# Fahad021/DER-VET

Measured on AMD Instinct MI355X. Metric: dispatch LP windows/sec (whole node, 8760h monthly windows); % HBM roofline, higher is better.
Workload: dtype f64

## Files before the change

der-vet_amd/csrc/dvh_band.hip:

```cpp
#include <stdio.h>
#include <stdlib.h>

#include <algorithm>
#include <type_traits>

#include "dvh_device.h"

namespace dvh {
namespace {

constexpr int kBandSteps = 768;
constexpr int kJMax = kBandJMax;
constexpr int kNeedsEll = -2;

__host__ __device__ constexpr size_t band_lds_doubles(int B, int S, bool ice, bool lc) {
  const int NW = B / kWave, NC = ice ? 5 : 3, NR = ice ? 4 : 2;
  const size_t SB = (size_t)S * B;
  return 2 * (size_t)(B + 1) + kJMax + (size_t)kNRed * (NW + 1) + 4 + (size_t)kJMax * B + (NC + NR) * SB +
         (lc ? 5 * SB : 0) + (ice ? 6 * SB : 0);
}
__host__ __device__ constexpr size_t band_ints_bytes(int B, int S) { return sizeof(int32_t) * (4 * (size_t)S * B + 4); }
__host__ __device__ constexpr size_t band_drow_bytes(int B, int S) { return align16(sizeof(int32_t) * (size_t)S * B); }
__host__ __device__ constexpr size_t band_lds_bytes(int B, int S, bool ice, bool lc) {
  const size_t d = align16(sizeof(double) * band_lds_doubles(B, S, ice, lc));
// ... 1152 lines not shown
    acc[2] = mv2;
    acc[3] = mv3;
#pragma unroll
    for (int u = 4; u < NRED; ++u) acc[u] = 0.0;
    double r = 0.0;
    if constexpr (GATE) {
      double acc4[4] = {acc[0], acc[1], acc[2], acc[3]};
      block_sum1<B, 4, true>(acc4, red);
#pragma unroll
      for (int u = 0; u < 4; ++u) acc[u] = acc4[u];
      r = usc<USC>(sqrt(pw * acc[0] + acc[2] / pw));
      if (kkt && !last && kkt_gate_skip(o, gate, r)) {
        kkt = false;
        ++gate.skip;
      }
    }
    if (kkt) {
      float fcl[S][NC], frl[S][NR], fspl = 1.0f;
      if constexpr (Tune::kkt_prefetch) {
        const int to = S * opaque(tid);
        const float* fcw = w.fc + W.wn;
        const float* frw = w.fr + W.wm;
#pragma unroll
        for (int s = 0; s < S; ++s) {
          const bool vs = to + s < T;
#pragma unroll
          for (int v = 0; v < NC; ++v) {
            const int j = v < 3 ? v * T + to + s : (v == 3 ? CE : CO) + to + s;
            const float f = fcw[vs ? j : 0];
            fcl[s][v] = vs ? f : 1.0f;
          }
#pragma unroll
          for (int r = 0; r < NR; ++r) {
            const int i = r == 0 ? (vs ? to + s + 1 : -1) : r == 1 ? DRL[s * B + tid] : (vs ? (r == 2 ? ra[s] : rb[s]) : -1);
            const float f = frw[i >= 0 ? i : 0];
            frl[s][r] = i >= 0 ? f : 1.0f;
          }
        }
        const int lo_ = (to / S) & (kWave - 1);
        const float ft = fcw[tlane ? 3 * T + lo_ : 0], fi = frw[0];
        fspl = tlane ? ft : ilane ? fi : 1.0f;
      }
      double xp[S][NC], yp[S][NR];
      load_images(xp, yp);
      XE[tid] = xp[0][2];
      YS[tid + 1] = yp[S - 1][0];
      if (ilane) YS[0] = sp[2];
      if (tlane) XT[lane] = sp[5];
      if (J > 0) tau_parts_of(yp);
      lds_barrier();
      auto col_kkt = [&](int j, double kt, double cj, double loj, double hij, double xj, float fpre) {
        const float fd = Tune::kkt_prefetch ? fpre : w.fc[W.wn + opaque(j)];
        static_assert(Tune::gate_rdx == Tune::kkt_inline, "col_kkt_x_i is inlined only, col_kkt_o out of line only");
        if constexpr (Tune::gate_rdx) {
          const ColKktX r = col_kkt_x_i(kt, cj, loj, hij, xj, fd);
          acc[5] += r.rd2;
          acc[6] += r.cx;
          acc[8] += r.bt;
          acc[kRdx] += r.rdx;
        } else {
          const ColKkt r = col_kkt_o(kt, cj, loj, hij, xj, fd);
          acc[5] += r.rd2;
          acc[6] += r.cx;
          acc[8] += r.bt;
        }
      };
      auto row_kkt = [&](int i, double kv, double qi, double yi, bool ge, float fpre) {
        const float fd = Tune::kkt_prefetch ? fpre : w.fr[W.wm + opaque(i)];
        const RowKkt r = row_kkt_fn<Tune::kkt_inline>(kv, qi, yi, fd, ge);
        acc[4] += r.rp2;
        acc[7] += qi * yi;
        acc[9] += r.y2;
      };
      const double ysp = YS[tid];
#pragma unroll
      for (int s = 0; s < S; ++s) {
        double kt[NC];
        ktr(s, yp[s], s == 0 ? ysp : yp[s > 0 ? s - 1 : 0][0], kt);
        if (val[s]) {
#pragma unroll
          for (int v = 0; v < NC; ++v) {
            if constexpr (BOX)
              col_kkt(col(s, v), kt[v], cof(s, v), 0.0, 1.0, xp[s][v], fcl[s][v]);
            else
              col_kkt(col(s, v), kt[v], cof(s, v), v == 2 ? loe[s] : 0.0, hib(s, v), xp[s][v], fcl[s][v]);
          }
        }
      }
      if (wid == 0 && J > 0) {
        const double ktt = tau_kt();
        if (tlane) col_kkt(3 * T + lane, ktt, sp[2], sp[3], sp[4], sp[5], fspl);
      }
      const double xen = XE[tid + 1];
#pragma unroll
      for (int s = 0; s < S; ++s) {
        double kv[NR];
        kown(s, xp[s], kv);
        kfin_next(s, kv, s == S - 1 ? xen : xp[s < S - 1 ? s + 1 : s][2]);
        kfin_tau(s, kv);
        const int t = t0 + s;
        if (val[s]) row_kkt(t + 1, kv[0], qv(s, 0), yp[s][0], false, frl[s][0]);
        const int dr_ = DRL[s * B + tid];
        if (dr_ >= 0) row_kkt(dr_, kv[1], qv(s, 1), yp[s][1], true, frl[s][1]);
        if (ICE && val[s]) {
          row_kkt(ra[s], kv[2], rhs(s, 2), yp[s][2], true, frl[s][NR > 2 ? 2 : 0]);
          row_kkt(rb[s], kv[3], rhs(s, 3), yp[s][3], true, frl[s][NR > 3 ? 3 : 0]);
        }
      }
      if (ilane) row_kkt(0, sp[4] * XE[0], sp[3], sp[2], false, fspl);
    }
    if constexpr (GATE) {
      if (kkt) {
        double acc6[NRED - 4];
#pragma unroll
        for (int u = 4; u < NRED; ++u) acc6[u - 4] = acc[u];
        block_sum1<B, NRED - 4, true>(acc6, red + 4 * NW);
#pragma unroll
        for (int u = 4; u < NRED; ++u) acc[u] = acc6[u - 4];
      }
    } else if (kkt) {
      block_sum1<B, NRED, true>(acc, red);
    } else {
      double acc4[4] = {acc[0], acc[1], acc[2], acc[3]};
      block_sum1<B, 4, true>(acc4, red);
#pragma unroll
      for (int u = 0; u < 4; ++u) acc[u] = acc4[u];
    }
    if constexpr (!GATE) r = usc<USC>(sqrt(pw * acc[0] + acc[2] / pw));
    if (kkt) {
      const double pobj = usc<USC>(acc[6] + c0), dobj = usc<USC>(acc[7] + acc[8] + c0);
      const double pres = usc<USC>(sqrt(acc[4]) / (1.0 + sgpr_fresh<USC>(qnorm)));
      const double dres = usc<USC>(sqrt(acc[5]) / (1.0 + sgpr_fresh<USC>(cnorm)));
      const double gap = usc<USC>(fabs(pobj - dobj) / (1.0 + fabs(pobj) + fabs(dobj)));
      if (tid == 0) {
        fin[0] = pobj;
        fin[1] = pres;
        fin[2] = dres;
        fin[3] = gap;
      }
      if (kkt_done(o, pres, dres, gap, pobj, dobj, acc[4], acc[9], Tune::gate_rdx ? acc[kRdx] : 0.0)) {
        status = kOptimal;
        break;
      }
      if constexpr (GATE) {
        gate.note(pres, dres, gap, o.eps, r);
        gate.q = usc<USC>(gate.q);
      }
      if (!(isfinite(pobj) && isfinite(dobj))) {
        status = kNumerical;
        break;
      }
    }
    if (r0 < 0.0) r0 = r;
    const bool restart = (r <= o.b_suff * r0) || (r <= o.b_nec * r0 && rprev >= 0.0 && r > rprev) ||
                         ((double)kin >= o.b_art * (double)it);
    if (restart) {
      const double ddx = sqrt(acc[1]), ddy = sqrt(acc[3]);
      if (ddx > 1e-10 && ddy > 1e-10) pw = uniform(pw_update<!ICE>(ddy / ddx, pw, o.theta));
      tau = uniform(eta / pw);
      sigma = uniform(eta * pw);
      sigma2n = uniform(-2.0 * sigma);
      box_steps_rescale();
      double xp[S][NC], yp[S][NR];
      load_images(xp, yp);
#pragma unroll
      for (int s = 0; s < S; ++s) {
#pragma unroll
        for (int v = 0; v < NC; ++v) {
          x[s][v] = xa[s][v] = xp[s][v];
        }
#pragma unroll
        for (int rr = 0; rr < NR; ++rr) {
          y[s][rr] = ya[s][rr] = yp[s][rr];
        }
      }
      if (ilane) sp[0] = sp[1] = sp[2];
      if (tlane) sp[0] = sp[1] = sp[5];
      kin = 0;
      kbase = 0;
      hw = hload(0);
      r0 = r;
      rprev = -1.0;
    } else {
      rprev = r;
    }
    if (restart || kkt) {
      YS[tid + 1] = y[S - 1][0];
      if (ilane) YS[0] = sp[0];
      if (J > 0) tau_parts_of(y);
      lds_barrier();
    }
  }
#pragma unroll
  for (int s = 0; s < S; ++s) {
    if (!val[s]) continue;
    const int t = t0 + s;
#pragma unroll
    for (int v = 0; v < NC; ++v) {
      const int j = col(s, v);
      if constexpr (BOX) {
        const double d = dcf(j), lo = lraw[j] / d, hv = uraw[j] / d;
        double wv = hv - (v == 2 ? lo : 0.0);
        if (!(wv >= 0x1p-500)) wv = 0.0;
        xo_g[j] = unscale_x(fmin(fmax(fma(wv, xpi(v, s), lo), lo), hv), d, lraw[j], uraw[j]);
      } else {
        xo_g[j] = unscale_x(xpi(v, s), dcf(j), lraw[j], uraw[j]);
      }
    }
    yo_g[t + 1] = ypi(0, s) * drf(t + 1);
    const int dr_ = DRL[s * B + tid];
    if (dr_ >= 0) yo_g[dr_] = ypi(1, s) * drf(dr_);
    if (ICE) {
      yo_g[ra[s]] = ypi(2, s) * drf(ra[s]);
      yo_g[rb[s]] = ypi(3, s) * drf(rb[s]);
    }
  }
  if (tlane) xo_g[3 * T + lane] = unscale_x(sp[5], dcf(3 * T + lane), lraw[3 * T + lane], uraw[3 * T + lane]);
  if (ilane) yo_g[0] = sp[2] * drf(0);
  if constexpr (DVH_BAND_PROBE) {
    pstamp(kProbeSegs - 1);
    pacc[kProbeSegs - 1] += (unsigned)(pt1 - pt2);
    unsigned hw = 0;
    asm volatile("s_getreg_b32 %0, hwreg(HW_REG_HW_ID)" : "=s"(hw));
    __syncthreads();
    if (lane == 0) {
      for (int u = 0; u < kProbeSegs; ++u) xo_g[(kProbeSegs + 1) * wid + u] = (double)pacc[u];
      xo_g[(kProbeSegs + 1) * wid + kProbeSegs] = (double)hw;
    }
  }
  if (tid == 0) {
    b.istats[2 * k] = status;
    b.istats[2 * k + 1] = it;
    for (int u = 0; u < 4; ++u) b.stats[4 * k + u] = fin[u];
  }
}

struct BandArgs {
  Batch b;
  Work w;
  Chunk ch;
  Opts o;
  const int32_t* list;
  int count;
  int32_t* queue;
};
template <int B, int S, bool ICE, bool LC, int WPS, bool GATE, bool BOX, bool PERSIST>
__global__ __launch_bounds__(B, WPS) void pdhg_band_kernel(const BandArgs args) {
  if constexpr (!PERSIST) {
    const int i = blockIdx.x;
    band_window<B, S, ICE, LC, WPS, GATE, BOX>(args.b, args.w, args.ch, args.o,
                                               args.list ? args.list[i] : args.ch.first + i, threadIdx.x);
  } else {
    __shared__ int32_t next;
    for (;;) {
#if defined(__HIP_DEVICE_COMPILE__)
      using KArgs = const __attribute__((address_space(4))) BandArgs*;
      KArgs kp = (KArgs)__builtin_amdgcn_kernarg_segment_ptr();
      asm volatile("" : "+s"(kp));
      const BandArgs& args = *(const BandArgs*)kp;
#endif
      if (__builtin_amdgcn_readfirstlane(threadIdx.x) < kWave)
        next = __builtin_amdgcn_readfirstlane(atomicAdd(args.queue, (threadIdx.x & (kWave - 1)) == 0 ? 1 : 0));
      __syncthreads();
      const int i = __builtin_amdgcn_readfirstlane(next);
      __syncthreads();
      if (i >= args.count) return;
      int tid = threadIdx.x;
#if defined(__HIP_DEVICE_COMPILE__)
      asm volatile("" : "+v"(tid));
#endif
      band_window<B, S, ICE, LC, WPS, GATE, BOX>(args.b, args.w, args.ch, args.o,
                                                 args.list ? args.list[i] : args.ch.first + i, tid);
    }
  }
}

template <int B, int S, bool ICE, bool LC, int WPS, bool GATE, bool BOX>
__global__ __launch_bounds__(B, WPS) void pdhg_band_kernel_j1(const BandArgs args) {
  __shared__ int32_t next;
  for (;;) {
#if defined(__HIP_DEVICE_COMPILE__)
    using KArgs = const __attribute__((address_space(4))) BandArgs*;
    KArgs kp = (KArgs)__builtin_amdgcn_kernarg_segment_ptr();
    asm volatile("" : "+s"(kp));
    const BandArgs& args = *(const BandArgs*)kp;
#endif
    if (__builtin_amdgcn_readfirstlane(threadIdx.x) < kWave)
      next = __builtin_amdgcn_readfirstlane(atomicAdd(args.queue, (threadIdx.x & (kWave - 1)) == 0 ? 1 : 0));
    __syncthreads();
    const int i = __builtin_amdgcn_readfirstlane(next);
    __syncthreads();
    if (i >= args.count) return;
    int tid = threadIdx.x;
#if defined(__HIP_DEVICE_COMPILE__)
    asm volatile("" : "+v"(tid));
#endif
    band_window<B, S, ICE, LC, WPS, GATE, BOX, true>(args.b, args.w, args.ch, args.o,
                                                     args.list ? args.list[i] : args.ch.first + i, tid);
  }
}

template <int B, int S, bool ICE, bool LC, int WPS, bool GATE, bool BOX, bool PERSIST>
hipError_t launch_band_one_q(const Batch& b, const Work& w, const Chunk& ch, const Opts& o, hipStream_t s,
                             const int32_t* list, int nlist, int* variant_out) {
  static_assert(B * S == kBandSteps, "every form covers T <= kBandSteps");
  const size_t lds = band_lds_bytes(B, S, ICE, LC);
  auto kern = pdhg_band_kernel<B, S, ICE, LC, WPS, GATE, BOX, PERSIST>;
  hipError_t e = hipFuncSetAttribute((const void*)kern, hipFuncAttributeMaxDynamicSharedMemorySize, (int)lds);
  if (e != hipSuccess) return e;
  if (getenv("DVH_BAND_OCC")) {
    int nb = -1, dev = 0;
    hipGetDevice(&dev);
    hipDeviceProp_t pr;
    hipGetDeviceProperties(&pr, dev);
    hipOccupancyMaxActiveBlocksPerMultiprocessor(&nb, (const void*)kern, B, lds);
    hipFuncAttributes fa;
    hipFuncGetAttributes(&fa, (const void*)kern);
    fprintf(stderr, "band<%d,%d,%d,%d,gate %d,box %d,persist %d>: lds %zu B, blocks/CU %d, lds/CU %zu, regs %d, local %zu\n",
            B, S, (int)ICE, (int)LC, (int)GATE, (int)BOX, (int)PERSIST, lds, nb, (size_t)pr.maxSharedMemoryPerMultiProcessor,
            fa.numRegs, (size_t)fa.localSizeBytes);
  }
  const int count = list ? nlist : ch.count;
  if (count <= 0) return hipSuccess;
  int grid = count;
  if (PERSIST) {
    int& slots = w.slots[(ICE ? 4 : 0) + (GATE ? 2 : 0) + (BOX ? 1 : 0)];
    if (slots <= 0) {
      int nb = 0, cus = 0, dev = 0;
      if ((e = hipGetDevice(&dev)) != hipSuccess) return e;
      if ((e = hipOccupancyMaxActiveBlocksPerMultiprocessor(&nb, (const void*)kern, B, lds)) != hipSuccess) return e;
      if ((e = hipDeviceGetAttribute(&cus, hipDeviceAttributeMultiprocessorCount, dev)) != hipSuccess) return e;
      slots = std::max(1, nb) * std::max(1, cus);
    }
    static const int reserve = [] { const char* e = getenv("DVH_BAND_RESERVE"); return e ? std::max(0, atoi(e)) : 0; }();
    grid = std::min(count, std::max(1, slots - 2 * reserve));
    if ((e = hipMemsetAsync(w.queue, 0, sizeof(int32_t), s)) != hipSuccess) return e;
  }
  const BandArgs args{b, w, ch, o, list, count, w.queue};
  hipLaunchKernelGGL(kern, dim3(grid), dim3(B), lds, s, args);
  if (variant_out) *variant_out = 9000000 + 1000 * (S - 1) + (ICE ? 100 : 0) + B / kWave;
  return hipGetLastError();
}
template <int B, int S, bool ICE, bool LC, int WPS, bool GATE, bool BOX>
hipError_t launch_band_one_g(const Batch& b, const Work& w, const Chunk& ch, const Opts& o, hipStream_t s,
                             const int32_t* list, int nlist, bool j1, int* variant_out) {
  if constexpr (S == 3 && !ICE) {
    static_assert(B == kBandSteps / 3 && LC && WPS == 2, "dvh_band_persist.hip instantiates this form");
    const char* q = getenv("DVH_BAND_QUEUE");
    if (!(q && atoi(q) == 0)) return launch_band_persist(GATE, BOX, j1, b, w, ch, o, s, list, nlist, variant_out);
  }
  if constexpr (ICE) {
    static_assert(B == kBandSteps && S == 1 && !LC && WPS == 3, "dvh_band_persist_ice.hip instantiates this form");
    const char* q = getenv("DVH_BAND_QUEUE");
    const char* qi = getenv("DVH_BAND_QUEUE_ICE");
    if (!(q && atoi(q) == 0) && !(qi && atoi(qi) == 0))
      return launch_band_persist_ice(GATE, BOX, b, w, ch, o, s, list, nlist, variant_out);
  }
  return launch_band_one_q<B, S, ICE, LC, WPS, GATE, BOX, false>(b, w, ch, o, s, list, nlist, variant_out);
}
template <int B, int S, bool ICE, bool LC, int WPS, bool BOX = false>
hipError_t launch_band_one(const Batch& b, const Work& w, const Chunk& ch, const Opts& o, hipStream_t s,
                           const int32_t* list, int nlist, bool j1, int* variant_out) {
  if (o.kkt_predict > 0)
    return launch_band_one_g<B, S, ICE, LC, WPS, true, BOX>(b, w, ch, o, s, list, nlist, j1, variant_out);
  return launch_band_one_g<B, S, ICE, LC, WPS, false, BOX>(b, w, ch, o, s, list, nlist, j1, variant_out);
}

}

#if DVH_BAND_PERSIST_TU == 1
namespace {
template <bool GATE, bool BOX>
hipError_t launch_band_persist_j1(const Batch& b, const Work& w, const Chunk& ch, const Opts& o, hipStream_t s,
                                  const int32_t* list, int nlist, int* variant_out) {
  constexpr int B = kBandSteps / 3, S = 3;
  const size_t lds = band_lds_bytes(B, S, false, true);
  auto kern = pdhg_band_kernel_j1<B, S, false, true, 2, GATE, BOX>;
  hipError_t e = hipFuncSetAttribute((const void*)kern, hipFuncAttributeMaxDynamicSharedMemorySize, (int)lds);
  if (e != hipSuccess) return e;
  const int count = list ? nlist : ch.count;
  if (count <= 0) return hipSuccess;
  int& slots = w.slots[8 + (GATE ? 2 : 0) + (BOX ? 1 : 0)];
  if (slots <= 0) {
    int nb = 0, cus = 0, dev = 0;
    if ((e = hipGetDevice(&dev)) != hipSuccess) return e;
    if ((e = hipOccupancyMaxActiveBlocksPerMultiprocessor(&nb, (const void*)kern, B, lds)) != hipSuccess) return e;
    if ((e = hipDeviceGetAttribute(&cus, hipDeviceAttributeMultiprocessorCount, dev)) != hipSuccess) return e;
    slots = std::max(1, nb) * std::max(1, cus);
  }
  static const int reserve = [] { const char* e = getenv("DVH_BAND_RESERVE"); return e ? std::max(0, atoi(e)) : 0; }();
  const int grid = std::min(count, std::max(1, slots - 2 * reserve));
  if ((e = hipMemsetAsync(w.queue, 0, sizeof(int32_t), s)) != hipSuccess) return e;
  const BandArgs args{b, w, ch, o, list, count, w.queue};
  hipLaunchKernelGGL(kern, dim3(grid), dim3(B), lds, s, args);
  if (variant_out) *variant_out = 9000000 + 1000 * (S - 1) + kBandJ1 + B / kWave;
  return hipGetLastError();
}
}
hipError_t launch_band_persist(bool gate, bool box, bool j1, const Batch& b, const Work& w, const Chunk& ch,
                               const Opts& o, hipStream_t s, const int32_t* list, int nlist, int* variant_out) {
  constexpr int B = kBandSteps / 3;
  if (j1) {
    const char* e = getenv("DVH_BAND_J1");
    if (e && atoi(e) == 0) j1 = false;
  }
  if (j1) {
    if (gate) {
      if (box) return launch_band_persist_j1<true, true>(b, w, ch, o, s, list, nlist, variant_out);
      return launch_band_persist_j1<true, false>(b, w, ch, o, s, list, nlist, variant_out);
    }
    if (box) return launch_band_persist_j1<false, true>(b, w, ch, o, s, list, nlist, variant_out);
    return launch_band_persist_j1<false, false>(b, w, ch, o, s, list, nlist, variant_out);
  }
  if (gate) {
    if (box) return launch_band_one_q<B, 3, false, true, 2, true, true, true>(b, w, ch, o, s, list, nlist, variant_out);
    return launch_band_one_q<B, 3, false, true, 2, true, false, true>(b, w, ch, o, s, list, nlist, variant_out);
  }
  if (box) return launch_band_one_q<B, 3, false, true, 2, false, true, true>(b, w, ch, o, s, list, nlist, variant_out);
  return launch_band_one_q<B, 3, false, true, 2, false, false, true>(b, w, ch, o, s, list, nlist, variant_out);
}
#elif DVH_BAND_PERSIST_TU == 2
hipError_t launch_band_persist_ice(bool gate, bool box, const Batch& b, const Work& w, const Chunk& ch, const Opts& o,
                                   hipStream_t s, const int32_t* list, int nlist, int* variant_out) {
  constexpr int B = kBandSteps;
  if (gate) {
    if (box) return launch_band_one_q<B, 1, true, false, 3, true, true, true>(b, w, ch, o, s, list, nlist, variant_out);
    return launch_band_one_q<B, 1, true, false, 3, true, false, true>(b, w, ch, o, s, list, nlist, variant_out);
  }
  if (box) return launch_band_one_q<B, 1, true, false, 3, false, true, true>(b, w, ch, o, s, list, nlist, variant_out);
  return launch_band_one_q<B, 1, true, false, 3, false, false, true>(b, w, ch, o, s, list, nlist, variant_out);
}
#else
hipError_t launch_pdhg_band(const Batch& b, const Work& w, const Chunk& ch, const Opts& o, hipStream_t s, bool ice,
                            int form, bool box, const int32_t* list, int nlist, bool j1, int* variant_out) {
  if (ice) {
    if (box) return launch_band_one<kBandSteps, 1, true, false, 3, true>(b, w, ch, o, s, list, nlist, false, variant_out);
    return launch_band_one<kBandSteps, 1, true, false, 3>(b, w, ch, o, s, list, nlist, false, variant_out);
  }
  if (form == 1) {
    if (box) return launch_band_one<kBandSteps, 1, false, false, 3, true>(b, w, ch, o, s, list, nlist, false, variant_out);
    return launch_band_one<kBandSteps, 1, false, false, 3>(b, w, ch, o, s, list, nlist, false, variant_out);
  }
  if (box) return launch_band_one<kBandSteps / 3, 3, false, true, 2, true>(b, w, ch, o, s, list, nlist, j1, variant_out);
  return launch_band_one<kBandSteps / 3, 3, false, true, 2>(b, w, ch, o, s, list, nlist, j1, variant_out);
}
#endif

}
```

der-vet_amd/csrc/dvh_cascade.cpp:

```cpp
#include <cstdio>
#include <cstdlib>

#include "dvh_handle.h"

namespace dvh {

int chain_pass(dvh_handle* h, const dvh::Batch& b, const dvh::Work& w, const dvh::Chunk& ch, const dvh::Opts& o,
               const std::vector<int32_t>& med, int max_T, const std::vector<int64_t>& desc,
               std::vector<char>& med_done, hipStream_t s) {
  const int nm = (int)med.size();
  if (nm == 0) return DVH_OK;
  const size_t I = sizeof(int32_t);
  DVH_HIP(h, h->m_list.ensure(I * (size_t)nm));
  DVH_HIP(h, hipMemcpyAsync(h->m_list.p, med.data(), I * nm, hipMemcpyHostToDevice, s));
  DVH_HIP(h, h->m_plan.ensure(I * (size_t)nm * dvh::kPlanInts));
  hipError_t e = dvh::launch_chain_plan(b, w, ch, h->m_list.as<int32_t>(), nm, max_T, h->m_plan.as<int32_t>(), s);
  if (e != hipSuccess) return hip_fail(h, e, "launch_chain_plan");
  std::vector<int32_t> head((size_t)nm * 4);
  DVH_HIP(h, hipMemcpy2DAsync(head.data(), 4 * I, h->m_plan.p, I * dvh::kPlanInts, 4 * I, nm, hipMemcpyDeviceToHost, s));
  DVH_HIP(h, sync_stream(h, s));
  std::vector<int32_t> small_setup, accepted;
  for (int i = 0; i < nm; ++i) {
    const int P = head[4 * (size_t)i];
    if (P < 0) med_done[med[i]] = 1;
    if (P <= 0) continue;
    accepted.push_back(i);
    if (desc[8 * (size_t)med[i]] < dvh::kMedSetupNMax) small_setup.push_back(med[i]);
  }
  if (accepted.empty()) return DVH_OK;
  if (!small_setup.empty()) {
    int mn = 0;
    for (int k : small_setup) mn = std::max<int>(mn, (int)desc[8 * (size_t)k]);
    DVH_HIP(h, h->m_pos.ensure(I * small_setup.size()));
    DVH_HIP(h, hipMemcpyAsync(h->m_pos.p, small_setup.data(), I * small_setup.size(), hipMemcpyHostToDevice, s));
    e = dvh::launch_setup_medium(b, w, ch, o, mn, h->m_pos.as<int32_t>(), (int)small_setup.size(), s);
    if (e != hipSuccess) return hip_fail(h, e, "launch_setup_medium");
  }
  for (int i : accepted) {
    const int k = med[i];
    if (desc[8 * (size_t)k] < dvh::kMedSetupNMax) continue;
    e = dvh::launch_setup_long(b, w, ch, o, k, &desc[8 * (size_t)k], s);
    if (e != hipSuccess) return hip_fail(h, e, "launch_setup_long");
  }
  std::vector<double> flag6(accepted.size(), 0.0);
  for (size_t a = 0; a < accepted.size(); ++a)
    DVH_HIP(h, hipMemcpyAsync(&flag6[a], w.scal + (int64_t)(med[accepted[a]] - ch.first) * dvh::kScal + 6,
                              sizeof(double), hipMemcpyDeviceToHost, s));
  DVH_HIP(h, sync_stream(h, s));
  std::vector<int32_t> groups[2];
  int PTg[2] = {0, 0};
  for (size_t a = 0; a < accepted.size(); ++a) {
    if (flag6[a] != 0.0) continue;
    const int i = accepted[a], P = head[4 * (size_t)i];
    const int g = P > dvh::kChainMedMax ? 1 : 0;
    groups[g].push_back(i);
    PTg[g] = std::max(PTg[g], P);
  }
  if (h->chain_cap < 0) {
    int cap = 0;
    if (dvh::chain_capacity(h->device, &cap) != hipSuccess) cap = 0;
    (void)hipGetLastError();
    h->chain_cap = cap;
  }
  if (h->spin_ticks <= 0) {
    int khz = 0;
    if (hipDeviceGetAttribute(&khz, hipDeviceAttributeWallClockRate, h->device) != hipSuccess || khz <= 0) khz = 100000;
    h->spin_ticks = (long long)khz * 1000 * 2;
    if (const char* v = getenv("DVH_CHAIN_SPIN_TICKS")) {
      const long long t = atoll(v);
      if (t != 0) h->spin_ticks = t;
    }
  }
  const int S = h->chain_cap / 8;
  for (int g = 0; g < 2; ++g) {
    const int PT = PTg[g];
    if (groups[g].empty()) continue;
    const int NT = S >= 1 && PT <= 8 * S ? dvh::chain_team_count(S, PT) : 0;
    if (NT < 1) continue;
    constexpr int kMaxPerLaunch = 0x3FFF - 2;
    for (size_t a0 = 0; a0 < groups[g].size(); a0 += kMaxPerLaunch) {
      const int np = (int)std::min<size_t>(kMaxPerLaunch, groups[g].size() - a0);
      const int32_t* pos = groups[g].data() + a0;
      std::vector<int32_t> ks(np);
      for (int q = 0; q < np; ++q) ks[q] = med[pos[q]];
      DVH_HIP(h, h->m_pos.ensure(I * 2 * (size_t)np));
      int32_t* dpos = h->m_pos.as<int32_t>();
      DVH_HIP(h, hipMemcpyAsync(dpos, pos, I * np, hipMemcpyHostToDevice, s));
      DVH_HIP(h, hipMemcpyAsync(dpos + np, ks.data(), I * np, hipMemcpyHostToDevice, s));
      e = dvh::launch_chain_mark(b, dpos + np, np, s);
      if (e != hipSuccess) return hip_fail(h, e, "launch_chain_mark");
      DVH_HIP(h, h->m_xbuf.ensure(dvh::chain_xbuf_bytes(NT, PT)));
      DVH_HIP(h, h->m_abort.ensure(dvh::chain_abort_bytes(S)));
      e = dvh::launch_chain(b, w, ch, o, dpos, np, h->m_plan.as<int32_t>(), PT, S, h->m_xbuf.p,
                            h->m_abort.as<int32_t>(), h->spin_ticks, s);
      if (e == hipErrorCooperativeLaunchTooLarge) {
        (void)hipGetLastError();
        h->chain_cap = 0;
        return DVH_OK;
      }
      if (e != hipSuccess) return hip_fail(h, e, "launch_chain");
      std::vector<int32_t> ab(dvh::chain_abort_bytes(S) / I);
      DVH_HIP(h, hipMemcpyAsync(ab.data(), h->m_abort.p, I * ab.size(), hipMemcpyDeviceToHost, s));
      DVH_HIP(h, sync_stream(h, s));
      if (getenv("DVH_CHAIN_PROBE_DUMP")) {
        for (int gb = 0; gb < 8 * S; ++gb)
          if (ab[16 + 8 * (size_t)gb + 6] || ab[16 + 8 * (size_t)gb + 7])
            fprintf(stderr, "PROBE block %d tauwait %d hopwait %d\n", gb, ab[16 + 8 * (size_t)gb + 6],
                    ab[16 + 8 * (size_t)gb + 7]);
      }
      if (ab[0] != 0) {
        std::string msg = "medium tier: a segment exchange timed out (PT " + std::to_string(PT) + ", NT " +
                          std::to_string(NT) + "); unfinished windows moved to the grid-wide path; workgroups "
                          "{block: state list round entry tag seen}:";
        for (int gb = 0; gb < 8 * S; ++gb) {
          const int32_t* d = &ab[16 + 8 * (size_t)gb];
          if (d[0] == 0) continue;
          char buf[128];
          snprintf(buf, sizeof buf, " %d: %d %d %d 0x%x 0x%x 0x%x;", gb, d[0], d[1], d[2], d[3], d[4], d[5]);
          msg += buf;
        }
        h->st.warn += msg;
        ++h->st.n_chain_aborts;
        std::vector<int32_t> st(2);
        for (int q = 0; q < np; ++q) {
          DVH_HIP(h, hipMemcpy(st.data(), b.istats + 2 * (int64_t)ks[q], 2 * I, hipMemcpyDeviceToHost));
          if (st[0] != dvh::kChainPending) {
            med_done[ks[q]] = 1;
            ++h->st.n_chain;
          }
        }
        continue;
      }
      for (int q = 0; q < np; ++q) med_done[ks[q]] = 1;
      h->st.n_chain += np;
    }
  }
  return DVH_OK;
}

int device_cascade(dvh_handle* h, const dvh::Batch& b, const dvh::Work& w, const dvh::Chunk& ch, const dvh::Opts& o,
                   int nsmall, int nj, int wc, int mn, int mm, hipStream_t s, const int32_t* order) {
  const size_t I = sizeof(int32_t);
  int32_t* L[5];
  for (int r = 0; r < 5; ++r) L[r] = h->d_list.as<int32_t>() + (size_t)r * wc;
  int32_t* info = h->d_route.as<int32_t>();
  int32_t* rh = h->route_host.as<int32_t>();
  if (h->cus <= 0 && hipDeviceGetAttribute(&h->cus, hipDeviceAttributeMultiprocessorCount, h->device) != hipSuccess)
    h->cus = 256;
  const int forced_form = h->kernel_path == 3 ? 1 : h->kernel_path == 4 ? 3 : 0;
  auto form_for = [&](int nl) { return forced_form ? forced_form : (nl <= h->cus ? 1 : 3); };
  auto route = [&](int slot, const int32_t* in, int n_in, int want, int cls, int out) -> hipError_t {
    return dvh::launch_route(b.desc, b.istats, w.scal, ch.first, n_in, in, want, dvh::kSmallMax, cls, 512, 768,
                             L[out], info + 8 * slot, s);
  };
  auto readback = [&](int slot0, int nslots) -> hipError_t {
    hipError_t e = hipMemcpyAsync(rh + 8 * slot0, info + 8 * slot0, 8 * I * nslots, hipMemcpyDeviceToHost, s);
    return e != hipSuccess ? e : sync_stream(h, s);
  };
  const bool j1 = nj == 0;
  int variant = -1, bvar = -1;
  h->last_band_variant = -1;
  auto form_code = [](int v) { return v >= 0 && v % 100 >= dvh::kBandJ1 ? v - dvh::kBandJ1 : v; };
  const char* box_env = getenv("DVH_BAND_BOX");
  const int box_mode = box_env ? atoi(box_env) : 1;
  const bool box = box_mode >= 1, box_ice = box_mode >= 2;
  DVH_HIP(h, dvh::launch_pdhg_band(b, w, ch, o, s, false, form_for(ch.count), box, order, order ? ch.count : 0, j1, &bvar));
  DVH_HIP(h, route(0, nullptr, ch.count, -2, 0, 0));
  if (box) DVH_HIP(h, route(1, nullptr, ch.count, -3, 0, 1));
  DVH_HIP(h, readback(0, box ? 2 : 1));
  if (box && rh[8] > 0) {
    DVH_HIP(h, dvh::launch_pdhg_band(b, w, ch, o, s, false, form_for(rh[8]), false, L[1], rh[8], j1, nullptr));
    DVH_HIP(h, route(0, nullptr, ch.count, -2, 0, 0));
    DVH_HIP(h, readback(0, 1));
  }
  int cur = rh[0];
  h->st.n_band += nsmall - cur;
  if (nsmall - cur > 0) {
    variant = form_code(bvar);
    h->last_band_variant = bvar;
  }
  if (cur > 0) {
    DVH_HIP(h, dvh::launch_pdhg_band(b, w, ch, o, s, true, form_for(cur), box_ice, L[0], cur, false, &bvar));
    if (h->kernel_path == 5) DVH_HIP(h, dvh::launch_pdhg_band_grid(b, w, ch, o, s, L[0], cur, &bvar));
    DVH_HIP(h, route(1, L[0], cur, -2, 0, 4));
    if (box_ice) DVH_HIP(h, route(2, L[0], cur, -3, 0, 1));
    DVH_HIP(h, readback(1, box_ice ? 2 : 1));
    if (box_ice && rh[16] > 0) {
      DVH_HIP(h, dvh::launch_pdhg_band(b, w, ch, o, s, true, form_for(rh[16]), false, L[1], rh[16], false, nullptr));
      DVH_HIP(h, route(1, L[0], cur, -2, 0, 4));
      DVH_HIP(h, readback(1, 1));
    }
    const int left = rh[8];
    h->st.n_band += cur - left;
    if (cur - left > 0 && variant < 0) variant = bvar;
    cur = left;
    if (cur > 0) {
      DVH_HIP(h, dvh::launch_setup(b, w, ch, o, mn, mm, s, L[4], cur));
      DVH_HIP(h, route(1, L[4], cur, -2, 1, 2));
      DVH_HIP(h, route(2, L[4], cur, -2, 2, 3));
      DVH_HIP(h, readback(1, 2));
    }
  }
  if (cur == 0) {
    h->last_variant = variant;
    return DVH_OK;
  }
  int ran[2] = {0, 0};
  for (int c = 0; c < 2; ++c) {
    const int32_t* in = rh + 8 * (1 + c);
    if (in[0] == 0) continue;
    int ev = -1;
    hipError_t e = dvh::launch_pdhg_ell(b, w, ch, o, in[3], in[4], in[1], in[2], s, &ev, L[2 + c], in[0],
                                        in[0] <= 2 * h->cus);
    if (e == hipSuccess) {
      if (variant < 0) variant = ev;
      DVH_HIP(h, route(3 + c, L[2 + c], in[0], -1, 0, c));
      ran[c] = 1;
    } else if (e == hipErrorInvalidValue) {
      (void)hipGetLastError();
    } else {
      return hip_fail(h, e, "launch_pdhg_ell");
    }
  }
  if (ran[0] || ran[1]) DVH_HIP(h, readback(3, 2));
  int gn = 0, gm[3] = {0, 0, 0};
  int32_t* gl = nullptr;
  for (int c = 0; c < 2; ++c) {
    const int32_t* in = rh + 8 * (1 + c);
    if (in[0] == 0) continue;
    const int32_t* g = ran[c] ? rh + 8 * (3 + c) : in;
    int32_t* l = ran[c] ? L[c] : L[2 + c];
    if (ran[c]) h->st.n_ell += in[0] - g[0];
    if (g[0] == 0) continue;
    if (!gl) {
      gl = l;
    } else {
      DVH_HIP(h, hipMemcpyAsync(gl + gn, l, I * g[0], hipMemcpyDeviceToDevice, s));
    }
    gn += g[0];
    for (int u = 0; u < 3; ++u) gm[u] = std::max(gm[u], (int)g[3 + u]);
  }
  if (gn > 0) {
    DVH_HIP(h, dvh::launch_power(b, w, ch, o, gl, gn, s));
    int gv = -1;
    hipError_t e = dvh::launch_pdhg(b, w, ch, o, gm[0], gm[1], gm[2], s, &gv, gl, gn);
    if (e == hipErrorInvalidValue)
      return fail(h, DVH_ERR_UNSUPPORTED, "window too large for the on-chip PDHG kernels (n or m > 4096)");
    if (e != hipSuccess) return hip_fail(h, e, "launch_pdhg");
    h->st.n_generic += gn;
    if (variant < 0) variant = gv;
  }
  h->last_variant = variant;
  return DVH_OK;
}

}
```

der-vet_amd/csrc/dvh_handle.h:

```cpp
#pragma once
#include <array>
#include <string>

#include "dvh_host.h"

struct SolveStats {
  int n_ell = 0, n_generic = 0, n_large = 0, n_band = 0, n_chain = 0;
  int n_chain_aborts = 0;
  std::string warn;
  float large_ms[2] = {0, 0};
  size_t chunk_used = 0;
  int32_t cert[5] = {0, 0, 0, 0, 0};
  double cert_ms = 0.0;
  double timing[3] = {0, 0, 0};
  void reset() {
    n_ell = n_generic = n_large = n_band = n_chain = 0;
    n_chain_aborts = 0;
    warn.clear();
    large_ms[0] = large_ms[1] = 0.0f;
    chunk_used = 0;
  }
  void add(const SolveStats& p) {
    n_ell += p.n_ell;
    n_generic += p.n_generic;
    n_large += p.n_large;
    n_band += p.n_band;
    n_chain += p.n_chain;
    n_chain_aborts += p.n_chain_aborts;
    warn += p.warn;
    for (int u = 0; u < 4; ++u) cert[u] += p.cert[u];
    cert[4] = std::max(cert[4], p.cert[4]);
    cert_ms = std::max(cert_ms, p.cert_ms);
    for (int u = 1; u < 3; ++u) timing[u] = std::max(timing[u], p.timing[u]);
  }
};

struct dvh_handle_core {
  int device = 0;
  hipStream_t stream = nullptr;
  ~dvh_handle_core() {
    if (stream) (void)hipStreamDestroy(stream);
  }
};

struct SizingSlot {
  dvh::SizingState* p = nullptr;
  SizingSlot() = default;
  SizingSlot(const SizingSlot&) = delete;
  SizingSlot& operator=(const SizingSlot&) = delete;
  ~SizingSlot() {
    if (p) dvh::sizing_destroy(p);
  }
};

struct dvh_handle : dvh_handle_core {
  SizingSlot sizing;
  dvh::CommOwner comm;
  dvh::LargeOwner large;
  DevEvent ev[4];
  DevEvent cert_ev[2];
  std::vector<std::array<DevEvent, 3>> chunk_events;
  DevEvent val_ev[2][2];
  bool val_ran[2] = {false, false};
  dvh_options opts{};
  std::string err;
  DevBuf d_desc, d_indptr, d_indices, d_data, d_c, d_c0, d_q, d_l, d_u, d_x, d_y, d_stats, d_istats;
  DevBuf w_queue;
  int band_slots[dvh::kPersistForms] = {};
  DevBuf w_tptr, w_tind, w_tval, w_kval, w_rowof, w_perm, w_dr, w_dc, w_cs, w_ls, w_us, w_qs, w_vbuf, w_wbuf,
      w_tmpc, w_tmpr, w_longk, w_longt, w_scal, w_fc, w_fr;
  DevBuf d_list, d_hinv;
  DevBuf m_list, m_plan, m_pos, m_xbuf, m_abort;
  int chain_cap = -1;
  long long spin_ticks = 0;
  SolveStats st;
  DevBuf o_data, o_cases, o_len, o_hist, o_soe;
  DevBuf s_pairs, s_wts, s_bad;
  DevBuf g_seeds, g_word;
  DevBuf d_route;
  DevBuf c_tptr, c_tind, c_tval, c_tau, c_gx, c_sig, c_gy, c_counts;
  bool cert_pending = false;
  DevBuf v_zwork;
  int n_syncs = 0;
  double outage_ms = 0.0;
  int last_variant = -1;
  int last_band_variant = -1;
  int kernel_path = 0;
  int cus = 0;
  std::vector<int32_t> order;
  std::vector<int32_t> order_used;
  DevBuf d_order;
  std::vector<dvh_handle*> peers;
  PinnedBuf route_host, cert_host;
};

inline hipError_t sync_stream(dvh_handle* h, hipStream_t s) {
  ++h->n_syncs;
  return hipStreamSynchronize(s);
}

inline int fail(dvh_handle* h, int code, const std::string& msg) {
  if (h) h->err = msg;
  return code;
}

inline int hip_fail(dvh_handle* h, hipError_t e, const char* where) {
  return fail(h, DVH_ERR_HIP, std::string(where) + ": " + hipGetErrorString(e));
}

#define DVH_HIP(h, call)                                 \
  do {                                                   \
    hipError_t e_ = (call);                              \
    if (e_ != hipSuccess) return hip_fail(h, e_, #call); \
  } while (0)

namespace dvh {

int device_cascade(dvh_handle* h, const Batch& b, const Work& w, const Chunk& ch, const Opts& o, int nsmall, int nj, int wc,
                   int mn, int mm, hipStream_t s, const int32_t* order);
int chain_pass(dvh_handle* h, const Batch& b, const Work& w, const Chunk& ch, const Opts& o,
               const std::vector<int32_t>& med, int max_T, const std::vector<int64_t>& desc,
               std::vector<char>& med_done, hipStream_t s);

}
```

der-vet_amd/csrc/dvh_internal.h:

```cpp
#pragma once
#include <hip/hip_runtime.h>
#include <stdint.h>

#include <memory>
#include <string>

struct dvh_window_series;
struct dvh_battery_group;
struct dvh_packed;
struct dvh_options;
struct dvh_handle;

namespace dvh {

constexpr int kWave = 64;
constexpr int kLongRow = 32;
constexpr int kLMax = 64;
constexpr int kScal = 16;
constexpr int kHalpernTab = 65536;
constexpr int kSmallMax = 4096;
constexpr int kChainB = 768;
constexpr int kPMax = 192;
constexpr int kChainMedMax = 16;
constexpr int kChainJMax = 256;
constexpr int kChainJSeg = 4;
constexpr int kPlanStart = 4;
constexpr int kPlanSlot = kPlanStart + kPMax + 4;
constexpr int kPlanLo = kPlanSlot + kChainJSeg * kPMax;
constexpr int kPlanHi = kPlanLo + kChainJSeg * kPMax;
constexpr int kPlanInts = kPlanHi + kChainJSeg * kPMax;
constexpr int kMedSetupNMax = 40000;

__host__ __device__ inline double unscale_x(double xs, double d, double l, double u) {
  const double v = xs * d;
  return v != v ? v : fmin(fmax(v, l), u);
}

struct Opts {
  double eps, step_safety, rho, b_suff, b_nec, b_art, theta;
  double eps_obj;
  int max_iters, check_every, kkt_every, ruiz_iters, power_iters;
  int setup_segments;
  int small_max;
  int warm;
  int kkt_predict;
};

struct Batch {
  const int64_t* desc;
  const int32_t* indptr;
  const int32_t* indices;
  const double* data;
  const double* c;
  const double* c0;
  const double* q;
  const double* l;
  const double* u;
  double* x;
  double* y;
  double* stats;
  int32_t* istats;
};

struct Work {
  int32_t* tptr;
  int32_t* tind;
  double* tval;
  double* kval;
  int32_t* rowof;
  int32_t* perm;
  double* dr;
  double* dc;
  double* cs;
  double* ls;
  double* us;
  double* qs;
  double* vbuf;
  double* wbuf;
  double* tmpc;
  double* tmpr;
  int32_t* longk;
  int32_t* longt;
  const double* hinv;
  double* scal;
  float* fc;
  float* fr;
  int32_t* queue;
  int* slots;
};
constexpr int kPersistForms = 12;

struct Chunk {
  int first;
  int count;
  int64_t base_n, base_m, base_nz;
};

hipError_t launch_setup(const Batch& b, const Work& w, const Chunk& ch, const Opts& o, int max_n, int max_m,
                        hipStream_t s, const int32_t* list = nullptr, int nlist = 0);
hipError_t launch_pdhg(const Batch& b, const Work& w, const Chunk& ch, const Opts& o, int max_n, int max_m,
                       int64_t max_nnz, hipStream_t s, int* variant_out, const int32_t* list, int nlist);
hipError_t launch_pdhg_ell(const Batch& b, const Work& w, const Chunk& ch, const Opts& o, int max_n, int max_m,
                           int wx, int wy, hipStream_t s, int* variant_out, const int32_t* list, int nlist,
                           bool latency = false);
hipError_t launch_pdhg_band(const Batch& b, const Work& w, const Chunk& ch, const Opts& o, hipStream_t s, bool ice,
                            int form, bool box, const int32_t* list, int nlist, bool j1, int* variant_out);
constexpr int kBandJ1 = 50;
constexpr int kBandJMax = 4;
hipError_t launch_band_persist(bool gate, bool box, bool j1, const Batch& b, const Work& w, const Chunk& ch,
                               const Opts& o, hipStream_t s, const int32_t* list, int nlist, int* variant_out);
hipError_t launch_band_persist_ice(bool gate, bool box, const Batch& b, const Work& w, const Chunk& ch, const Opts& o,
                                   hipStream_t s, const int32_t* list, int nlist, int* variant_out);
size_t setup_lds_bytes(int max_n, int max_m);
hipError_t launch_setup_medium(const Batch& b, const Work& w, const Chunk& ch, const Opts& o, int max_n,
                               const int32_t* list, int nlist, hipStream_t s);
hipError_t launch_chain_plan(const Batch& b, const Work& w, const Chunk& ch, const int32_t* list, int nlist,
                             int max_T, int32_t* plan, hipStream_t s);
hipError_t launch_setup_long(const Batch& b, const Work& w, const Chunk& ch, const Opts& o, int k, const int64_t* d,
                             hipStream_t s);
constexpr int kChainPending = -7;
hipError_t launch_chain_mark(const Batch& b, const int32_t* list, int nlist, hipStream_t s);
hipError_t chain_capacity(int device, int* blocks);
size_t chain_xbuf_bytes(int NT, int PT);
size_t chain_abort_bytes(int S);
int chain_team_count(int S, int PT);
hipError_t launch_chain(const Batch& b, const Work& w, const Chunk& ch, const Opts& o, const int32_t* pos, int npos,
                        const int32_t* plan, int PT, int S, void* xbuf, int32_t* abort_word, long long spin_ticks,
                        hipStream_t s);
constexpr int kMaxBlend = 8;
hipError_t launch_warm_transfer(const int64_t* desc, const double* c, const double* u, double* x, double* y,
                                const int32_t* rows, const double* wts, int q, int count, int32_t* bad, hipStream_t s);
hipError_t launch_series_draws(const uint64_t* seeds, int count, int steps, int n_unif, double a1, double innov,
                               double* z0, double* ar, double* unif, int32_t* ambiguous, int32_t* amb_rows,
                               hipStream_t s);
hipError_t launch_series_windows(const ::dvh_window_series& w, int32_t* bad, hipStream_t s);
hipError_t launch_build_battery(const ::dvh_battery_group& g, const ::dvh_packed& b, int first, hipStream_t s);
hipError_t launch_route(const int64_t* desc, const int32_t* istats, const double* scal, int first, int count,
                        const int32_t* in_list, int want, int small_max, int cls, int lim_n, int lim_m,
                        int32_t* out_list, int32_t* out_info, hipStream_t s);
hipError_t launch_power(const Batch& b, const Work& w, const Chunk& ch, const Opts& o, const int32_t* list, int nlist,
                        hipStream_t s);

struct OutageCase {
  int n_steps, max_steps, outage_len, pad;
  int64_t len_off, hist_off;
  double dt, soe0, dg_gen, gamma, soe_min, soe_max, charge_max, discharge_max, rte;
  const double *critical_load, *pv_max, *pv_vari, *init_soe, *load_shed;
};
hipError_t launch_outage(const OutageCase* d_cases, int ncase, int max_steps_n, int max_bins, int32_t* d_lengths,
                         int32_t* d_hist, hipStream_t s);
hipError_t launch_outage_min_soe(const OutageCase* d_cases, int ncase, int max_steps_n, double* d_soe_used,
                                 hipStream_t s);

hipError_t launch_outage_first_uncovered(const OutageCase* d_cases, int ncase, int max_steps_n, int32_t* d_first,
                                         int32_t* d_count, hipStream_t s);

struct SizingLP {
  const double *cl, *pv_vari, *shed;
  int32_t* starts;
  int n_steps, K, L, new_start;
  double dt, dg_gen, rte, llsoc, ulsoc, a0;
  double lE, uE, lP, uP, cE, cP, c0;
};
hipError_t launch_build_sizing(const SizingLP* d_lps, int nlp, const int64_t* desc, int32_t* indptr, int32_t* indices,
                               double* data, double* c, double* c0, double* q, double* l, double* u, hipStream_t s);
hipError_t launch_gather_sizes(const int64_t* desc, const double* x, const int32_t* istats, int nlp, double* sizes,
                               hipStream_t s);

struct SizingState;
void sizing_destroy(SizingState* s);
struct LargeSolver;
LargeSolver* large_create();
void large_destroy(LargeSolver* ls);
struct Comm;
void comm_destroy(Comm* c);
template <auto Destroy>
struct DestroyWith {
  template <class T>
  void operator()(T* p) const { Destroy(p); }
};
using LargeOwner = std::unique_ptr<LargeSolver, DestroyWith<large_destroy>>;
using CommOwner = std::unique_ptr<Comm, DestroyWith<comm_destroy>>;

struct HandleView {
  int device;
  hipStream_t stream;
  dvh_options* opts;
  std::string* err;
  SizingState** sizing;
};
HandleView handle_view(dvh_handle* h);
inline int fail(const HandleView& v, int code, const std::string& msg) {
  *v.err = msg;
  return code;
}
#define DVH_VIEW_HIP(v, call)                                                                                  \
  do {                                                                                                         \
    hipError_t e_ = (call);                                                                                    \
    if (e_ != hipSuccess) return dvh::fail(v, DVH_ERR_HIP, std::string(#call) + ": " + hipGetErrorString(e_)); \
  } while (0)


constexpr int kCommIdBytes = 128;
int comm_unique_id(unsigned char* id, std::string* err);
int comm_init(int device, int rank, int world, const unsigned char* id, CommOwner* out, std::string* err);
int comm_all_gather(Comm* c, const void* send, void* recv, size_t bytes, hipStream_t s, std::string* err);
void comm_info(const Comm* c, int* rank, int* world);
hipError_t large_solve(LargeSolver* ls, const Batch& b, int k, const int64_t* d, const Opts& o, const double* hinv,
                       hipStream_t s, std::string* err, float* setup_ms, float* pdhg_ms);

hipError_t launch_pdhg_band_grid(const Batch& b, const Work& w, const Chunk& ch, const Opts& o, hipStream_t s,
                                 const int32_t* list, int nlist, int* variant_out);

constexpr int kCertifyDefaultCap = 65536;
struct CertWork {
  int32_t* tptr;
  int32_t* tind;
  double* tval;
  double* tau;
  double* gx;
  double* sig;
  double* gy;
  int32_t* counts;
  int64_t base_n, base_m, base_nz;
};
size_t certify_lds_bytes(int max_n, int max_m);
hipError_t launch_certify(const Batch& b, const CertWork& cw, int count, int max_n, int max_m, int cap, int gate,
                          hipStream_t s);

}
```

der-vet_amd/csrc/dvh_solve.cpp:

```cpp
#include <chrono>
#include <thread>

#include "dvh_handle.h"
#include "dvh_validate.h"

namespace {

constexpr int kChunkWindows = 262144;

dvh::Opts make_opts(const dvh_options& p) {
  dvh::Opts o;
  o.eps = p.eps;
  o.eps_obj = p.eps_obj;
  o.step_safety = p.step_safety;
  o.rho = p.reflection;
  o.b_suff = p.restart_sufficient;
  o.b_nec = p.restart_necessary;
  o.b_art = p.restart_artificial;
  o.theta = p.primal_weight_theta;
  o.max_iters = p.max_iters;
  o.check_every = std::max(1, std::min(p.check_every, p.max_iters));
  o.kkt_every = p.kkt_every;
  o.ruiz_iters = p.ruiz_iters;
  o.power_iters = p.power_iters;
  o.warm = p.warm_start != 0;
  o.kkt_predict = p.kkt_predict;
  o.small_max = dvh::kSmallMax;
  return o;
}

dvh::Batch make_batch(const dvh_packed& bt) {
  return dvh::Batch{bt.desc, bt.indptr, bt.indices, bt.data, bt.c, bt.c0, bt.q, bt.l, bt.u,
                    bt.x, bt.y, bt.stats, bt.istats};
}

int certify_pass(dvh_handle* h, const dvh_packed* bt, const std::vector<int64_t>& desc, int gate, hipStream_t s) {
  const int count = bt->count;
  const int64_t bn = desc[6], bm = desc[7], bz = desc[5];
  int64_t sn = 0, sm = 0, snz = 0;
  int mn = 1, mm = 1;
  for (int k = 0; k < count; ++k) {
    const int64_t* d = &desc[8 * (size_t)k];
    sn = std::max(sn, d[6] + d[0] - bn);
    sm = std::max(sm, d[7] + d[1] - bm);
    snz = std::max(snz, d[5] + d[3] - bz);
    if (d[0] > dvh::kSmallMax || d[1] > dvh::kSmallMax) continue;
    mn = std::max<int>(mn, (int)d[0]);
    mm = std::max<int>(mm, (int)d[1]);
  }
  const size_t D = sizeof(double), I = sizeof(int32_t);
  DVH_HIP(h, h->c_tptr.ensure(I * (size_t)(sn + count)));
  DVH_HIP(h, h->c_tind.ensure(I * (size_t)snz));
  DVH_HIP(h, h->c_tval.ensure(D * (size_t)snz));
  DVH_HIP(h, h->c_tau.ensure(D * (size_t)sn));
  DVH_HIP(h, h->c_gx.ensure(D * (size_t)sn));
  DVH_HIP(h, h->c_sig.ensure(D * (size_t)sm));
  DVH_HIP(h, h->c_gy.ensure(D * (size_t)sm));
  DVH_HIP(h, h->c_counts.ensure(I * 5));
  DVH_HIP(h, h->cert_host.ensure(I * 5));
  for (DevEvent& e : h->cert_ev) DVH_HIP(h, e.ensure());
  dvh::CertWork cw{h->c_tptr.as<int32_t>(), h->c_tind.as<int32_t>(), h->c_tval.as<double>(), h->c_tau.as<double>(),
                   h->c_gx.as<double>(), h->c_sig.as<double>(), h->c_gy.as<double>(), h->c_counts.as<int32_t>(),
                   bn, bm, bz};
  const int cap = h->opts.certify_iters > 0 ? h->opts.certify_iters : dvh::kCertifyDefaultCap;
  DVH_HIP(h, hipMemsetAsync(h->c_counts.p, 0, I * 5, s));
  DVH_HIP(h, hipEventRecord(h->cert_ev[0], s));
  DVH_HIP(h, dvh::launch_certify(make_batch(*bt), cw, count, mn, mm, cap, gate, s));
  DVH_HIP(h, hipEventRecord(h->cert_ev[1], s));
  DVH_HIP(h, hipMemcpyAsync(h->cert_host.p, h->c_counts.p, I * 5, hipMemcpyDeviceToHost, s));
  h->cert_pending = true;
  return DVH_OK;
}

void certify_reset(dvh_handle* h) {
  for (int32_t& v : h->st.cert) v = 0;
  h->st.cert_ms = 0.0;
  h->cert_pending = false;
}

bool is_large(const int64_t* d) { return d[0] > dvh::kSmallMax || d[1] > dvh::kSmallMax; }

struct ChunkPlan {
  dvh::Chunk ch;
  int64_t sn, sm, snz;
  int mn, mm;
  int64_t mnz;
  int nsmall;
  int nj;
  std::vector<int32_t> med;
  int med_T = 0;
};
struct BatchPlan {
  std::vector<ChunkPlan> chunks;
  std::vector<int> large;
  int64_t wn = 0, wm = 0, wnz = 0;
  int wc = 0;
};

BatchPlan scan_chunks(const std::vector<int64_t>& desc, int count, bool chain_on) {
  auto is_medium = [&](const int64_t* d) {
    const int64_t T = d[2] - 1;
    return chain_on && T > dvh::kChainB && T <= (int64_t)dvh::kPMax * dvh::kChainB && d[0] >= 3 * T &&
           d[0] <= 3 * T + dvh::kChainJMax && d[1] <= 2 * T + 1;
  };
  BatchPlan p;
  for (int first = 0; first < count; first += kChunkWindows) {
    ChunkPlan c{};
    c.ch.first = first;
    c.ch.count = std::min(kChunkWindows, count - first);
    const int64_t* d0 = &desc[8 * (size_t)first];
    c.ch.base_n = d0[6];
    c.ch.base_m = d0[7];
    c.ch.base_nz = d0[5];
    for (int k = first; k < first + c.ch.count; ++k) {
      const int64_t* d = &desc[8 * (size_t)k];
      c.sn = std::max(c.sn, d[6] + d[0] - c.ch.base_n);
      c.sm = std::max(c.sm, d[7] + d[1] - c.ch.base_m);
      c.snz = std::max(c.snz, d[5] + d[3] - c.ch.base_nz);
      if (is_large(d)) {
        p.large.push_back(k);
        if (is_medium(d)) {
          c.med.push_back(k);
          c.med_T = std::max<int>(c.med_T, (int)d[2] - 1);
        }
        continue;
      }
      ++c.nsmall;
      const int64_t J = d[0] - 3 * (d[2] - 1);
      if (J == 0 || (J >= 2 && J <= dvh::kBandJMax)) ++c.nj;
      c.mn = std::max<int>(c.mn, (int)d[0]);
      c.mm = std::max<int>(c.mm, (int)d[1]);
      c.mnz = std::max(c.mnz, d[3]);
    }
    p.wn = std::max(p.wn, c.sn);
    p.wm = std::max(p.wm, c.sm);
    p.wnz = std::max(p.wnz, c.snz);
    p.wc = std::max(p.wc, c.ch.count);
    p.chunks.push_back(c);
  }
  return p;
}

int make_work(dvh_handle* h, const BatchPlan& p, dvh::Work& w) {
  const int64_t wn = p.wn, wm = p.wm, wnz = p.wnz;
  const int wc = p.wc;
  const size_t D = sizeof(double), I = sizeof(int32_t);
  DVH_HIP(h, h->w_tptr.ensure(I * (wn + wc)));
  DVH_HIP(h, h->w_tind.ensure(I * wnz));
  DVH_HIP(h, h->w_tval.ensure(D * wnz));
  DVH_HIP(h, h->w_kval.ensure(D * wnz));
  DVH_HIP(h, h->w_rowof.ensure(I * wnz));
  DVH_HIP(h, h->w_perm.ensure(I * wnz));
  DVH_HIP(h, h->w_dr.ensure(D * wm));
  DVH_HIP(h, h->w_dc.ensure(D * wn));
  DVH_HIP(h, h->w_cs.ensure(D * wn));
  DVH_HIP(h, h->w_ls.ensure(D * wn));
  DVH_HIP(h, h->w_us.ensure(D * wn));
  DVH_HIP(h, h->w_qs.ensure(D * wm));
  DVH_HIP(h, h->w_vbuf.ensure(D * wn));
  DVH_HIP(h, h->w_wbuf.ensure(D * wm));
  DVH_HIP(h, h->w_tmpc.ensure(D * wn));
  DVH_HIP(h, h->w_tmpr.ensure(D * wm));
  DVH_HIP(h, h->w_longk.ensure(I * (size_t)wc * dvh::kLMax));
  DVH_HIP(h, h->w_longt.ensure(I * (size_t)wc * dvh::kLMax));
  DVH_HIP(h, h->w_scal.ensure(D * (size_t)wc * dvh::kScal));
  DVH_HIP(h, h->w_fc.ensure(sizeof(float) * wn));
  DVH_HIP(h, h->w_fr.ensure(sizeof(float) * wm));
  DVH_HIP(h, h->w_queue.ensure(sizeof(int32_t)));
  w = dvh::Work{h->w_tptr.as<int32_t>(), h->w_tind.as<int32_t>(), h->w_tval.as<double>(), h->w_kval.as<double>(),
                h->w_rowof.as<int32_t>(), h->w_perm.as<int32_t>(), h->w_dr.as<double>(), h->w_dc.as<double>(),
                h->w_cs.as<double>(), h->w_ls.as<double>(), h->w_us.as<double>(), h->w_qs.as<double>(),
                h->w_vbuf.as<double>(), h->w_wbuf.as<double>(), h->w_tmpc.as<double>(), h->w_tmpr.as<double>(),
                h->w_longk.as<int32_t>(), h->w_longt.as<int32_t>(), h->d_hinv.as<double>(), h->w_scal.as<double>(),
                h->w_fc.as<float>(), h->w_fr.as<float>(), h->w_queue.as<int32_t>(), h->band_slots};
  DVH_HIP(h, h->d_list.ensure(I * 5 * (size_t)wc));
  DVH_HIP(h, h->d_route.ensure(I * 8 * 5));
  DVH_HIP(h, h->route_host.ensure(I * 8 * 5));
  return DVH_OK;
}

int next_chunk_events(dvh_handle* h, const DevEvent*& out) {
  if (h->st.chunk_used == h->chunk_events.size()) h->chunk_events.emplace_back();
  std::array<DevEvent, 3>& ce = h->chunk_events[h->st.chunk_used];
  for (DevEvent& e : ce) DVH_HIP(h, e.ensure());
  ++h->st.chunk_used;
  out = ce.data();
  return DVH_OK;
}

int host_list_tiers(dvh_handle* h, const dvh::Batch& b, const dvh::Work& w, const ChunkPlan& c, const dvh::Opts& o,
                    bool fast, const std::vector<int64_t>& desc, hipStream_t s) {
  const size_t I = sizeof(int32_t);
  auto large_at = [&](int k) { return is_large(&desc[8 * (size_t)k]); };
  std::vector<double> scal((size_t)c.ch.count * dvh::kScal);
  DVH_HIP(h, hipMemcpyAsync(scal.data(), w.scal, sizeof(double) * scal.size(), hipMemcpyDeviceToHost, s));
  DVH_HIP(h, sync_stream(h, s));
  int wx = 0, wy = 0;
  for (int k = 0; k < c.ch.count; ++k) {
    const double* sc = &scal[(size_t)k * dvh::kScal];
    if (sc[6] != 0.0) continue;
    wy = std::max(wy, (int)sc[8]);
    wx = std::max(wx, (int)sc[9]);
  }
  int variant = -1;
  hipError_t e = hipErrorInvalidValue;
  if (fast) {
    int ev = -1;
    e = dvh::launch_pdhg_ell(b, w, c.ch, o, c.mn, c.mm, wx, wy, s, &ev, nullptr, 0);
    if (e == hipSuccess) variant = ev;
  }
  std::vector<int32_t> generic;
  if (e == hipSuccess) {
    std::vector<int32_t> ist(2 * (size_t)c.ch.count);
    DVH_HIP(h, hipMemcpyAsync(ist.data(), b.istats + 2 * (size_t)c.ch.first, I * ist.size(),
                              hipMemcpyDeviceToHost, s));
    DVH_HIP(h, sync_stream(h, s));
    int nl = 0;
    for (int k = 0; k < c.ch.count; ++k) {
      if (large_at(c.ch.first + k)) {
        ++nl;
        continue;
      }
      if (ist[2 * (size_t)k] == -1) generic.push_back(c.ch.first + k);
    }
    h->st.n_ell += c.ch.count - (int)generic.size() - nl;
  } else if (e == hipErrorInvalidValue) {
    (void)hipGetLastError();
    for (int k = 0; k < c.ch.count; ++k)
      if (!large_at(c.ch.first + k)) generic.push_back(c.ch.first + k);
  } else {
    return hip_fail(h, e, "launch_pdhg_ell");
  }
  if (!generic.empty()) {
    DVH_HIP(h, hipMemcpyAsync(h->d_list.p, generic.data(), I * generic.size(), hipMemcpyHostToDevice, s));
    DVH_HIP(h, dvh::launch_power(b, w, c.ch, o, h->d_list.as<int32_t>(), (int)generic.size(), s));
    int gv = -1;
    e = dvh::launch_pdhg(b, w, c.ch, o, c.mn, c.mm, c.mnz, s, &gv, h->d_list.as<int32_t>(), (int)generic.size());
    if (e == hipErrorInvalidValue)
      return fail(h, DVH_ERR_UNSUPPORTED, "window too large for the on-chip PDHG kernels (n or m > 4096)");
    if (e != hipSuccess) return hip_fail(h, e, "launch_pdhg");
    h->st.n_generic += (int)generic.size();
    if (variant < 0) variant = gv;
    DVH_HIP(h, sync_stream(h, s));
  }
  h->last_variant = variant;
  return DVH_OK;
}

int solve_packed(dvh_handle* h, const dvh_packed* bt, const std::vector<int64_t>& desc, hipStream_t s) {
  const int count = bt->count;
  certify_reset(h);
  const dvh::Opts o = make_opts(h->opts);
  const dvh::Batch b = make_batch(*bt);
  const bool fast = h->kernel_path != 1 && o.rho == 1.0;
  const bool cascade = fast && (h->kernel_path == 0 || h->kernel_path >= 3);
  const bool chain_on = (h->kernel_path == 0 || h->kernel_path >= 3) && o.rho == 1.0 && o.max_iters + o.power_iters < (1 << 17);
  const BatchPlan plan = scan_chunks(desc, count, chain_on);
  dvh::Work w;
  if (int rc = make_work(h, plan, w)) return rc;
  h->st.reset();
  DVH_HIP(h, hipEventRecord(h->ev[0], s));
  const size_t I = sizeof(int32_t);
  const int32_t* order = nullptr;
  h->order_used.swap(h->order);
  h->order.clear();
  if (!h->order_used.empty() && (int)h->order_used.size() == count && plan.chunks.size() == 1 &&
      plan.chunks[0].nsmall == count) {
    DVH_HIP(h, h->d_order.ensure(I * count));
    DVH_HIP(h, hipMemcpyAsync(h->d_order.as<int32_t>(), h->order_used.data(), I * count, hipMemcpyHostToDevice, s));
    order = h->d_order.as<int32_t>();
  }
  std::vector<char> med_done(count, 0);
  for (const ChunkPlan& c : plan.chunks) {
    if (c.nsmall == 0 && c.med.empty()) continue;
    const DevEvent* ce = nullptr;
    if (int rc = next_chunk_events(h, ce)) return rc;
    DVH_HIP(h, hipEventRecord(ce[0], s));
    if (c.nsmall > 0 && !cascade) DVH_HIP(h, dvh::launch_setup(b, w, c.ch, o, c.mn, c.mm, s));
    DVH_HIP(h, hipEventRecord(ce[1], s));
    if (c.nsmall > 0)
      if (int rc = cascade ? dvh::device_cascade(h, b, w, c.ch, o, c.nsmall, c.nj, plan.wc, c.mn, c.mm, s, order)
                           : host_list_tiers(h, b, w, c, o, fast, desc, s))
        return rc;
    if (int rc = dvh::chain_pass(h, b, w, c.ch, o, c.med, c.med_T, desc, med_done, s)) return rc;
    DVH_HIP(h, hipEventRecord(ce[2], s));
  }
  for (int k : plan.large) {
    if (med_done[k]) continue;
    if (!h->large) h->large.reset(dvh::large_create());
    std::string msg;
    hipError_t e = dvh::large_solve(h->large.get(), b, k, &desc[8 * (size_t)k], o, h->d_hinv.as<double>(), s, &msg,
                                    &h->st.large_ms[0], &h->st.large_ms[1]);
    if (e != hipSuccess) return fail(h, DVH_ERR_HIP, "window " + std::to_string(k) + ": " + msg);
    ++h->st.n_large;
  }
  if (h->opts.certify != 0)
    if (int rc = certify_pass(h, bt, desc, 1, s)) return rc;
  DVH_HIP(h, hipEventRecord(h->ev[3], s));
  return DVH_OK;
}

int certify_packed(dvh_handle* h, const dvh_packed* bt, const std::vector<int64_t>& desc, hipStream_t s) {
  certify_reset(h);
  h->st.reset();
  DVH_HIP(h, hipEventRecord(h->ev[0], s));
  if (int rc = certify_pass(h, bt, desc, 0, s)) return rc;
  DVH_HIP(h, hipEventRecord(h->ev[3], s));
  return DVH_OK;
}

int finish_timing(dvh_handle* h, hipStream_t s) {
  DVH_HIP(h, sync_stream(h, s));
  SolveStats& st = h->st;
  float t = 0;
  st.timing[0] = st.timing[1] = st.timing[2] = 0;
  if (hipEventElapsedTime(&t, h->ev[0], h->ev[3]) == hipSuccess) st.timing[0] = t;
  if (h->cert_pending) {
    for (int i = 0; i < 5; ++i) st.cert[i] = h->cert_host.as<int32_t>()[i];
    if (hipEventElapsedTime(&t, h->cert_ev[0], h->cert_ev[1]) == hipSuccess) st.cert_ms = t;
    h->cert_pending = false;
  }
  for (size_t i = 0; i < st.chunk_used; ++i) {
    const auto& ce = h->chunk_events[i];
    if (hipEventElapsedTime(&t, ce[0], ce[1]) == hipSuccess) st.timing[1] += t;
    if (hipEventElapsedTime(&t, ce[1], ce[2]) == hipSuccess) st.timing[2] += t;
  }
  st.timing[1] += st.large_ms[0];
  st.timing[2] += st.large_ms[1];
  return DVH_OK;
}

std::vector<int> split_batch(const dvh_lp* lps, int32_t count, int parts) {
  std::vector<double> cum(count + 1, 0.0);
  for (int k = 0; k < count; ++k) {
    const dvh_lp& lp = lps[k];
    const bool big = lp.n > dvh::kSmallMax || lp.m_eq + lp.m_ineq > dvh::kSmallMax;
    cum[k + 1] = cum[k] + (big ? std::max(1.0, lp.nnz / 5208.0) : 1.0);
  }
  std::vector<int> b(parts + 1, count);
  b[0] = 0;
  for (int r = 1; r < parts; ++r) {
    const double target = cum[count] * r / parts;
    int k = b[r - 1];
    while (k < count && cum[k] + 0.5 * (cum[k + 1] - cum[k]) < target) ++k;
    b[r] = k;
  }
  return b;
}

int solve_batch_one(dvh_handle* h, const dvh_lp* lps, int32_t count, dvh_result* out, bool screen = false) {
  DVH_HIP(h, hipSetDevice(h->device));
  std::vector<int64_t> desc(8 * (size_t)count);
  int64_t tn = 0, tm = 0, tz = 0, tr = 0;
  for (int k = 0; k < count; ++k) {
    std::string msg = dvh::validate_lp(lps[k], k);
    if (!msg.empty()) return fail(h, DVH_ERR_ARG, msg);
    const dvh_lp& lp = lps[k];
    const int m = lp.m_eq + lp.m_ineq;
    int64_t* d = &desc[8 * (size_t)k];
    d[0] = lp.n;
    d[1] = m;
    d[2] = lp.m_eq;
    d[3] = lp.nnz;
    d[4] = tr;
    d[5] = tz;
    d[6] = tn;
    d[7] = tm;
    tr += m + 1;
    tz += lp.nnz;
    tn += lp.n;
    tm += m;
  }
  std::vector<int32_t> indptr(tr), indices(tz);
  std::vector<double> data(tz), c(tn), l(tn), u(tn), q(tm), c0(count);
  for (int k = 0; k < count; ++k) {
    const dvh_lp& lp = lps[k];
    const int64_t* d = &desc[8 * (size_t)k];
    const int m = (int)d[1];
    std::memcpy(&indptr[d[4]], lp.indptr, sizeof(int32_t) * (m + 1));
    if (lp.nnz) {
      std::memcpy(&indices[d[5]], lp.indices, sizeof(int32_t) * lp.nnz);
      std::memcpy(&data[d[5]], lp.data, sizeof(double) * lp.nnz);
    }
    std::memcpy(&c[d[6]], lp.c, sizeof(double) * lp.n);
    std::memcpy(&l[d[6]], lp.l, sizeof(double) * lp.n);
    std::memcpy(&u[d[6]], lp.u, sizeof(double) * lp.n);
    if (m) std::memcpy(&q[d[7]], lp.q, sizeof(double) * m);
    c0[k] = lp.c0;
  }
  const size_t D = sizeof(double), I = sizeof(int32_t);
  DVH_HIP(h, h->d_desc.ensure(desc.size() * sizeof(int64_t)));
  DVH_HIP(h, h->d_indptr.ensure(I * tr));
  DVH_HIP(h, h->d_indices.ensure(I * std::max<int64_t>(tz, 1)));
  DVH_HIP(h, h->d_data.ensure(D * std::max<int64_t>(tz, 1)));
  DVH_HIP(h, h->d_c.ensure(D * tn));
  DVH_HIP(h, h->d_l.ensure(D * tn));
  DVH_HIP(h, h->d_u.ensure(D * tn));
  DVH_HIP(h, h->d_x.ensure(D * tn));
  DVH_HIP(h, h->d_q.ensure(D * std::max<int64_t>(tm, 1)));
  DVH_HIP(h, h->d_y.ensure(D * std::max<int64_t>(tm, 1)));
  DVH_HIP(h, h->d_c0.ensure(D * count));
  DVH_HIP(h, h->d_stats.ensure(D * 4 * count));
  DVH_HIP(h, h->d_istats.ensure(I * 2 * count));
  hipStream_t s = h->stream;
  DVH_HIP(h, hipMemcpyAsync(h->d_desc.p, desc.data(), desc.size() * sizeof(int64_t), hipMemcpyHostToDevice, s));
  DVH_HIP(h, hipMemcpyAsync(h->d_indptr.p, indptr.data(), I * tr, hipMemcpyHostToDevice, s));
  if (tz) {
    DVH_HIP(h, hipMemcpyAsync(h->d_indices.p, indices.data(), I * tz, hipMemcpyHostToDevice, s));
    DVH_HIP(h, hipMemcpyAsync(h->d_data.p, data.data(), D * tz, hipMemcpyHostToDevice, s));
  }
  DVH_HIP(h, hipMemcpyAsync(h->d_c.p, c.data(), D * tn, hipMemcpyHostToDevice, s));
  DVH_HIP(h, hipMemcpyAsync(h->d_l.p, l.data(), D * tn, hipMemcpyHostToDevice, s));
  DVH_HIP(h, hipMemcpyAsync(h->d_u.p, u.data(), D * tn, hipMemcpyHostToDevice, s));
  if (tm) DVH_HIP(h, hipMemcpyAsync(h->d_q.p, q.data(), D * tm, hipMemcpyHostToDevice, s));
  DVH_HIP(h, hipMemcpyAsync(h->d_c0.p, c0.data(), D * count, hipMemcpyHostToDevice, s));
  std::vector<double> x0, y0;
  if (h->opts.warm_start || screen) {
    x0.assign(tn, 0.0);
    y0.assign(std::max<int64_t>(tm, 1), 0.0);
    for (int k = 0; k < count; ++k) {
      const int64_t* d = &desc[8 * (size_t)k];
      if (out[k].x) std::memcpy(&x0[d[6]], out[k].x, D * d[0]);
      if (out[k].y && d[1]) std::memcpy(&y0[d[7]], out[k].y, D * d[1]);
    }
    DVH_HIP(h, hipMemcpyAsync(h->d_x.p, x0.data(), D * tn, hipMemcpyHostToDevice, s));
    DVH_HIP(h, hipMemcpyAsync(h->d_y.p, y0.data(), D * y0.size(), hipMemcpyHostToDevice, s));
  }
  const dvh_packed bt{count, 0, tn, tm, tz, tr, h->d_desc.as<int64_t>(), h->d_indptr.as<int32_t>(),
                      h->d_indices.as<int32_t>(), h->d_data.as<double>(), h->d_c.as<double>(), h->d_c0.as<double>(),
                      h->d_q.as<double>(), h->d_l.as<double>(), h->d_u.as<double>(), h->d_x.as<double>(),
                      h->d_y.as<double>(), h->d_stats.as<double>(), h->d_istats.as<int32_t>()};
  h->n_syncs = 0;
  int rc = screen ? certify_packed(h, &bt, desc, s) : solve_packed(h, &bt, desc, s);
  if (rc != DVH_OK) return rc;
  std::vector<double> x(tn), y(tm), stats(4 * (size_t)count);
  std::vector<int32_t> ist(2 * (size_t)count);
  DVH_HIP(h, hipMemcpyAsync(x.data(), h->d_x.p, D * tn, hipMemcpyDeviceToHost, s));
  if (tm) DVH_HIP(h, hipMemcpyAsync(y.data(), h->d_y.p, D * tm, hipMemcpyDeviceToHost, s));
  DVH_HIP(h, hipMemcpyAsync(stats.data(), h->d_stats.p, D * 4 * count, hipMemcpyDeviceToHost, s));
  DVH_HIP(h, hipMemcpyAsync(ist.data(), h->d_istats.p, I * 2 * count, hipMemcpyDeviceToHost, s));
  rc = finish_timing(h, s);
  if (rc != DVH_OK) return rc;
  for (int k = 0; k < count; ++k) {
    const int64_t* d = &desc[8 * (size_t)k];
    dvh_result& r = out[k];
    if (r.x) std::memcpy(r.x, &x[d[6]], D * d[0]);
    if (r.y && d[1]) std::memcpy(r.y, &y[d[7]], D * d[1]);
    r.obj = stats[4 * k];
    r.primal_res_rel = stats[4 * k + 1];
    r.dual_res_rel = stats[4 * k + 2];
    r.gap_rel = stats[4 * k + 3];
    r.status = ist[2 * k];
    r.iters = ist[2 * k + 1];
  }
  return DVH_OK;
}

}

extern "C" {

int dvh_solve_batch(dvh_handle* h, const dvh_lp* lps, int32_t count, dvh_result* out) {
  if (!h) return DVH_ERR_ARG;
  if (count < 0 || (count > 0 && (!lps || !out))) return fail(h, DVH_ERR_ARG, "null lps/out or negative count");
  if (count == 0) return DVH_OK;
  if (h->peers.empty()) return solve_batch_one(h, lps, count, out);
  const auto t0 = std::chrono::steady_clock::now();
  std::vector<dvh_handle*> hs = {h};
  hs.insert(hs.end(), h->peers.begin(), h->peers.end());
  const int P = (int)hs.size();
  const std::vector<int> b = split_batch(lps, count, P);
  std::vector<int> rc(P, DVH_OK);
  std::vector<std::thread> th;
  for (int i = 1; i < P; ++i)
    if (b[i + 1] > b[i]) th.emplace_back([&, i] { rc[i] = solve_batch_one(hs[i], lps + b[i], b[i + 1] - b[i], out + b[i]); });
  if (b[1] > b[0]) rc[0] = solve_batch_one(h, lps, b[1], out);
  for (auto& t : th) t.join();
  SolveStats total;
  for (int i = 0; i < P; ++i) {
    if (rc[i] != DVH_OK) {
      const std::string msg = hs[i]->err;
      return fail(h, rc[i], "device " + std::to_string(hs[i]->device) + " (part " + std::to_string(i) + "): " + msg);
    }
    if (b[i + 1] > b[i]) total.add(hs[i]->st);
  }
  total.timing[0] = std::chrono::duration<double, std::milli>(std::chrono::steady_clock::now() - t0).count();
  h->st = total;
  return DVH_OK;
}

int dvh_certify_batch(dvh_handle* h, const dvh_lp* lps, int32_t count, dvh_result* out) {
  if (!h) return DVH_ERR_ARG;
  if (count < 0 || (count > 0 && (!lps || !out))) return fail(h, DVH_ERR_ARG, "null lps/out or negative count");
  if (count == 0) {
    certify_reset(h);
    return DVH_OK;
  }
  return solve_batch_one(h, lps, count, out, true);
}

int dvh_solve_packed_device(dvh_handle* h, const dvh_packed* bt, void* stream) {
  if (!h) return DVH_ERR_ARG;
  if (!bt || bt->count < 0) return fail(h, DVH_ERR_ARG, "null or negative batch");
  if (bt->count == 0) return DVH_OK;
  if (!bt->desc || !bt->indptr || !bt->c || !bt->c0 || !bt->l || !bt->u || !bt->x || !bt->stats || !bt->istats)
    return fail(h, DVH_ERR_ARG, "null device array in packed batch");
  DVH_HIP(h, hipSetDevice(h->device));
  hipStream_t s = stream ? static_cast<hipStream_t>(stream) : h->stream;
  h->n_syncs = 0;
  std::vector<int64_t> desc(8 * (size_t)bt->count);
  DVH_HIP(h, hipMemcpyAsync(desc.data(), bt->desc, desc.size() * sizeof(int64_t), hipMemcpyDeviceToHost, s));
  DVH_HIP(h, sync_stream(h, s));
  for (int k = 0; k < bt->count; ++k) {
    const int64_t* d = &desc[8 * (size_t)k];
    if (d[0] <= 0 || d[1] < 0 || d[2] < 0 || d[2] > d[1] || d[3] < 0 || d[4] < 0 || d[5] < 0 || d[6] < 0 || d[7] < 0 ||
        d[4] + d[1] + 1 > bt->total_rows || d[5] + d[3] > bt->total_nnz || d[6] + d[0] > bt->total_n ||
        d[7] + d[1] > bt->total_m)
      return fail(h, DVH_ERR_ARG, "packed descriptor " + std::to_string(k) + " out of range");
    if (k > 0) {
      const int64_t* p = &desc[8 * (size_t)(k - 1)];
      if (d[5] < p[5] || d[6] < p[6] || d[7] < p[7])
        return fail(h, DVH_ERR_ARG, "packed descriptors must have non-decreasing offsets");
    }
  }
  int rc = solve_packed(h, bt, desc, s);
  if (rc != DVH_OK) return rc;
  return finish_timing(h, s);
}

}
```

der-vet_amd/csrc/dvh_sweep.hip:

```cpp
#include "dvh_internal.h"

namespace dvh {
namespace {

constexpr int kSwB = 256;

__global__ __launch_bounds__(kSwB) void warm_transfer_kernel(const int64_t* desc, const double* c, const double* u,
                                                             double* x, double* y, const int32_t* rows,
                                                             const double* wts, int Q, int32_t* bad) {
  __shared__ double red[(kMaxBlend + 1) * (kSwB / kWave)];
  __shared__ double cps[kMaxBlend], cds[kMaxBlend];
  const int32_t* row = rows + (int64_t)(Q + 2) * blockIdx.x;
  const int w = row[0], T = row[Q + 1];
  const int64_t* dw = desc + 8 * (int64_t)w;
  const int64_t n = dw[0], m = dw[1];
  bool ok_shape = !(T > 0 && (3 * (int64_t)T + 1 != n || T + 1 > m));
  for (int i = 0; i < Q; ++i) {
    const int64_t* dp = desc + 8 * (int64_t)row[1 + i];
    ok_shape &= n == dp[0] && m == dp[1];
  }
  if (!ok_shape) {
    if (threadIdx.x == 0) atomicAdd(bad, 1);
    return;
  }
  const double* wq = wts + (int64_t)Q * blockIdx.x;
  const int64_t onw = dw[6], omw = dw[7];
  const int tid = threadIdx.x;
  int64_t onp[kMaxBlend], omp[kMaxBlend];
  double wqv[kMaxBlend];
#pragma unroll
  for (int q = 0; q < kMaxBlend; ++q) {
    const int64_t* dp = desc + 8 * (int64_t)row[1 + (q < Q ? q : 0)];
    onp[q] = dp[6];
    omp[q] = dp[7];
    wqv[q] = q < Q ? wq[q] : 0.0;
  }
  constexpr int kU = 2;
  for (int64_t j0 = tid; j0 < n; j0 += kU * kSwB) {
    double ur[kU], uv[kMaxBlend][kU], xv[kMaxBlend][kU];
#pragma unroll
    for (int e = 0; e < kU; ++e) {
      const int64_t j = j0 + e * kSwB;
      ur[e] = j < n ? u[onw + j] : 0.0;
#pragma unroll
      for (int q = 0; q < kMaxBlend; ++q) {
        uv[q][e] = (q < Q && j < n) ? u[onp[q] + j] : 1.0;
        xv[q][e] = (q < Q && j < n) ? x[onp[q] + j] : 0.0;
      }
    }
#pragma unroll
    for (int e = 0; e < kU; ++e) {
      const int64_t j = j0 + e * kSwB;
      if (j >= n) break;
      double acc = 0.0;
#pragma unroll
      for (int q = 0; q < kMaxBlend; ++q) {
        if (q >= Q) break;
        const double us = uv[q][e];
        const bool ok = isfinite(ur[e]) && isfinite(us) && us > 0.0;
        acc += wqv[q] * (xv[q][e] * (ok ? ur[e] / us : 1.0));
      }
      x[onw + j] = acc;
    }
  }
  if (T <= 0) {
    for (int64_t i = tid; i < m; i += kSwB) {
      double acc = 0.0;
#pragma unroll
      for (int q = 0; q < kMaxBlend; ++q) {
        if (q >= Q) break;
        acc += wqv[q] * y[omp[q] + i];
      }
      y[omw + i] = acc;
    }
    return;
  }
  const int lane = tid & 63, wid = tid >> 6;
  double a = 0.0;
  double bq[kMaxBlend];
#pragma unroll
  for (int q = 0; q < kMaxBlend; ++q) bq[q] = 0.0;
  for (int j = tid; j < T; j += kSwB) {
    a += fabs(c[onw + j]);
#pragma unroll
    for (int q = 0; q < kMaxBlend; ++q)
      if (q < Q) bq[q] += fabs(c[onp[q] + j]);
  }
#pragma unroll
  for (int o = 32; o > 0; o >>= 1) {
    a += __shfl_xor(a, o, kWave);
#pragma unroll
    for (int q = 0; q < kMaxBlend; ++q)
      if (q < Q) bq[q] += __shfl_xor(bq[q], o, kWave);
  }
  if (lane == 0) {
    red[(kMaxBlend + 1) * wid] = a;
#pragma unroll
    for (int q = 0; q < kMaxBlend; ++q)
      if (q < Q) red[(kMaxBlend + 1) * wid + 1 + q] = bq[q];
  }
  __syncthreads();
  if (tid < Q) {
    double sa = 0.0, sb = 0.0;
    for (int v = 0; v < kSwB / kWave; ++v) {
      sa += red[(kMaxBlend + 1) * v];
      sb += red[(kMaxBlend + 1) * v + 1 + tid];
    }
    const int64_t onq = desc[8 * (int64_t)row[1 + tid] + 6];
    cps[tid] = (sa / T) / fmax(sb / T, 1e-12);
    cds[tid] = c[onw + 3 * (int64_t)T] / fmax(c[onq + 3 * (int64_t)T], 1e-12);
  }
  __syncthreads();
  double cp[kMaxBlend], cd[kMaxBlend];
#pragma unroll
  for (int q = 0; q < kMaxBlend; ++q) {
    cp[q] = q < Q ? cps[q] : 0.0;
    cd[q] = q < Q ? cds[q] : 0.0;
  }
  for (int64_t i0 = tid; i0 < m; i0 += kU * kSwB) {
    double yv[kMaxBlend][kU];
#pragma unroll
    for (int e = 0; e < kU; ++e) {
      const int64_t i = i0 + e * kSwB;
#pragma unroll
      for (int q = 0; q < kMaxBlend; ++q) yv[q][e] = (q < Q && i < m) ? y[omp[q] + i] : 0.0;
    }
#pragma unroll
    for (int e = 0; e < kU; ++e) {
      const int64_t i = i0 + e * kSwB;
      if (i >= m) break;
      double acc = 0.0;
#pragma unroll
      for (int q = 0; q < kMaxBlend; ++q) {
        if (q >= Q) break;
        acc += wqv[q] * (yv[q][e] * (i <= T ? cp[q] : cd[q]));
      }
      y[omw + i] = acc;
    }
  }
}

}

hipError_t launch_warm_transfer(const int64_t* desc, const double* c, const double* u, double* x, double* y,
                                const int32_t* rows, const double* wts, int q, int count, int32_t* bad, hipStream_t s) {
  if (count <= 0) return hipSuccess;
  if (q < 1 || q > kMaxBlend) return hipErrorInvalidValue;
  hipLaunchKernelGGL(warm_transfer_kernel, dim3(count), dim3(kSwB), 0, s, desc, c, u, x, y, rows, wts, q, bad);
  return hipGetLastError();
}

}
```

der-vet_amd/dervet_hip/_lib.py:

```python
import ctypes
import os

HERE = os.path.dirname(os.path.abspath(__file__))
LIB_PATH = os.environ.get("DVH_LIB") or os.path.join(HERE, "libdervet_hip.so")

DVH_OK, DVH_ERR_ARG, DVH_ERR_HIP, DVH_ERR_UNSUPPORTED = 0, -1, -2, -3
OPTIMAL, PRIMAL_INFEASIBLE, DUAL_INFEASIBLE, ITER_LIMIT, NUMERICAL, UNDECIDED = 0, 1, 2, 3, 4, 5
STATUS_NAMES = {OPTIMAL: "optimal", PRIMAL_INFEASIBLE: "infeasible", DUAL_INFEASIBLE: "unbounded",
                ITER_LIMIT: "optimal_inaccurate", NUMERICAL: "solver_error",
                UNDECIDED: "undecided"}

c_int32_p = ctypes.POINTER(ctypes.c_int32)
c_double_p = ctypes.POINTER(ctypes.c_double)
c_int64_p = ctypes.POINTER(ctypes.c_int64)


class Options(ctypes.Structure):
    _fields_ = [("eps", ctypes.c_double), ("max_iters", ctypes.c_int32), ("check_every", ctypes.c_int32),
                ("ruiz_iters", ctypes.c_int32), ("power_iters", ctypes.c_int32), ("step_safety", ctypes.c_double),
                ("reflection", ctypes.c_double), ("restart_sufficient", ctypes.c_double),
                ("restart_necessary", ctypes.c_double), ("restart_artificial", ctypes.c_double),
                ("primal_weight_theta", ctypes.c_double), ("verbose", ctypes.c_int32),
                ("kkt_every", ctypes.c_int32), ("warm_start", ctypes.c_int32), ("certify_iters", ctypes.c_int32),
                ("eps_obj", ctypes.c_double), ("kkt_predict", ctypes.c_int32),
                ("certify", ctypes.c_int32)]


class LP(ctypes.Structure):
    _fields_ = [("n", ctypes.c_int32), ("m_eq", ctypes.c_int32), ("m_ineq", ctypes.c_int32), ("nnz", ctypes.c_int32),
                ("indptr", c_int32_p), ("indices", c_int32_p), ("data", c_double_p), ("c", c_double_p),
                ("c0", ctypes.c_double), ("q", c_double_p), ("l", c_double_p), ("u", c_double_p),
                ("structure", ctypes.c_int32), ("reserved", ctypes.c_int32)]


class Result(ctypes.Structure):
    _fields_ = [("x", c_double_p), ("y", c_double_p), ("obj", ctypes.c_double), ("primal_res_rel", ctypes.c_double),
                ("dual_res_rel", ctypes.c_double), ("gap_rel", ctypes.c_double), ("status", ctypes.c_int32),
                ("iters", ctypes.c_int32)]


class Packed(ctypes.Structure):
    _fields_ = [("count", ctypes.c_int32), ("reserved", ctypes.c_int32), ("total_n", ctypes.c_int64),
                ("total_m", ctypes.c_int64), ("total_nnz", ctypes.c_int64), ("total_rows", ctypes.c_int64),
                ("desc", ctypes.c_void_p), ("indptr", ctypes.c_void_p), ("indices", ctypes.c_void_p),
                ("data", ctypes.c_void_p), ("c", ctypes.c_void_p), ("c0", ctypes.c_void_p), ("q", ctypes.c_void_p),
                ("l", ctypes.c_void_p), ("u", ctypes.c_void_p), ("x", ctypes.c_void_p), ("y", ctypes.c_void_p),
                ("stats", ctypes.c_void_p), ("istats", ctypes.c_void_p)]


class OutageCase(ctypes.Structure):
    _fields_ = [("n_steps", ctypes.c_int32), ("max_outage", ctypes.c_int32), ("dt", ctypes.c_double),
                ("critical_load", c_double_p), ("pv_max", c_double_p), ("pv_vari", c_double_p),
                ("init_soe", c_double_p), ("load_shed_pct", c_double_p), ("soe0", ctypes.c_double),
                ("dg_gen", ctypes.c_double), ("gamma", ctypes.c_double), ("soe_min", ctypes.c_double),
                ("soe_max", ctypes.c_double), ("charge_max", ctypes.c_double), ("discharge_max", ctypes.c_double),
                ("rte", ctypes.c_double)]


class SizingSpec(ctypes.Structure):
    _fields_ = [("target_hours", ctypes.c_double), ("size_energy", ctypes.c_int32), ("size_power", ctypes.c_int32),
                ("ccost", ctypes.c_double), ("ccost_kw", ctypes.c_double), ("ccost_kwh", ctypes.c_double),
                ("energy_min", ctypes.c_double), ("energy_max", ctypes.c_double), ("power_min", ctypes.c_double),
                ("power_max", ctypes.c_double), ("energy", ctypes.c_double), ("power", ctypes.c_double),
                ("llsoc", ctypes.c_double), ("ulsoc", ctypes.c_double), ("soc_init", ctypes.c_double),
                ("n_seed", ctypes.c_int32), ("max_rounds", ctypes.c_int32)]


class SizingResult(ctypes.Structure):
    _fields_ = [("energy", ctypes.c_double), ("power", ctypes.c_double), ("capex", ctypes.c_double),
                ("status", ctypes.c_int32), ("lp_status", ctypes.c_int32), ("rounds", ctypes.c_int32),
                ("n_starts", ctypes.c_int32), ("lp_iters", ctypes.c_int32), ("reserved", ctypes.c_int32),
                ("starts", c_int32_p)]


SIZING_STATUS_NAMES = {0: "SIZED", 1: "ROUND_LIMIT", 2: "STALLED", 3: "LP_FAILED"}


class BatteryGroup(ctypes.Structure):
    _fields_ = [("T", ctypes.c_int32), ("J", ctypes.c_int32), ("G", ctypes.c_int32), ("mI", ctypes.c_int32),
                ("dt", ctypes.c_double), ("has_retail", ctypes.c_int32), ("has_da", ctypes.c_int32),
                ("has_emin", ctypes.c_int32), ("has_emax", ctypes.c_int32)] + \
               [(f, ctypes.c_void_p) for f in ("dcm_t", "dcm_j", "base", "retail", "da", "demand", "emin", "emax", "E",
                                               "pch", "pdis", "rte", "sdr", "soc_target", "ulsoc", "llsoc", "om",
                                               "c0")] + \
               [("has_ice", ctypes.c_int32), ("pad_ice", ctypes.c_int32)] + \
               [(f, ctypes.c_void_p) for f in ("ice_cap", "ice_pmin", "ice_cost")]



class SweepDraws(ctypes.Structure):
    _fields_ = [("count", ctypes.c_int32), ("steps", ctypes.c_int32), ("n_uniform", ctypes.c_int32),
                ("seeds", ctypes.c_void_p), ("a1", ctypes.c_double), ("innov", ctypes.c_double),
                ("z0", ctypes.c_void_p), ("ar", ctypes.c_void_p), ("uniform", ctypes.c_void_p),
                ("ambiguous", ctypes.c_void_p)]


class WindowSeries(ctypes.Structure):
    _fields_ = [(f, ctypes.c_int32) for f in ("G", "T", "t0", "rep", "J", "count", "hours")] + \
               [("dt", ctypes.c_double)] + \
               [(f, ctypes.c_void_p) for f in ("rows", "ar", "site_load", "pv_profile", "price", "load_scale",
                                               "price_scale", "pv_rated", "hp", "c0_add", "base", "retail", "c0")]

class DegradationState(ctypes.Structure):
    _fields_ = [("incl_cycle_degrade", ctypes.c_int32), ("reserved", ctypes.c_int32)] + \
               [(f, ctypes.c_void_p) for f in ("e_rated", "yearly", "soh", "replaceable", "degrade_perc",
                                               "replacements", "skipped", "capacity", "degradation", "reached")]


RAINFLOW_MAX_T, RAINFLOW_MAX_TABLE = 20351, 64


class BillGroup(ctypes.Structure):
    _fields_ = [("T", ctypes.c_int32), ("J", ctypes.c_int32), ("G", ctypes.c_int32), ("mI", ctypes.c_int32),
                ("dt", ctypes.c_double), ("has_pv", ctypes.c_int32), ("has_ice", ctypes.c_int32)] + \
               [(f, ctypes.c_void_p) for f in ("dcm_t", "dcm_j", "base", "orig", "retail", "da", "demand", "om",
                                               "ice_cost")]


class ValuationArgs(ctypes.Structure):
    _fields_ = [("S", ctypes.c_int32), ("Y", ctypes.c_int32), ("n_opt", ctypes.c_int32), ("n_extra", ctypes.c_int32),
                ("n_win", ctypes.c_int64), ("n_bills", ctypes.c_int64), ("opt_years", c_int32_p),
                ("win_ptr_host", c_int64_p)] + \
               [(f, ctypes.c_void_p) for f in ("win_ptr", "win_idx", "win_year", "bills", "bad")] + \
               [("rate", ctypes.c_double), ("growth", ctypes.c_double * 5)] + \
               [(f, ctypes.c_void_p) for f in ("capex", "fixed_om", "extra")]


BILL_ROWS, BILL_MAX_J, CBA_MAX_YEARS, CBA_MAX_EXTRA, CBA_FIXED_COLS, VALUE_COLS = 8, 16, 64, 16, 7, 7

class ValueSpec(ctypes.Structure):
    _fields_ = [("size_energy", ctypes.c_int32), ("size_power", ctypes.c_int32), ("c_energy", ctypes.c_double),
                ("c_power", ctypes.c_double), ("c_fixed", ctypes.c_double), ("alpha", ctypes.c_double),
                ("energy_min", ctypes.c_double), ("energy_max", ctypes.c_double), ("power_min", ctypes.c_double),
                ("power_max", ctypes.c_double), ("gap_tol", ctypes.c_double), ("max_rounds", ctypes.c_int32),
                ("reserved", ctypes.c_int32)]


class ValueMasterArgs(ctypes.Structure):
    _fields_ = [(f, ctypes.c_int32) for f in ("count", "n_cases", "W", "n_cand", "n_next", "cut_cap")] + \
               [("spec_host", ctypes.POINTER(ValueSpec))] + \
               [(f, ctypes.c_void_p) for f in ("spec", "case_ids", "window_cuts", "E_in", "P_in", "cuts", "state",
                                               "flags", "E_out", "pch_out", "pdis_out")]


VALUE_CUT_COLS, VALUE_MAX_J, VALUE_MAX_CUTS, VALUE_MAX_CAND, VALUE_STATE_COLS, VALUE_FLAG_COLS = 10, 64, 256, 8, 8, 8
VALUE_STATUS_NAMES = {0: "SIZED", 1: "ROUND_LIMIT", 2: "LP_FAILED", 3: "MASTER_FAILED"}

SYMBOLS = {
    "dvh_version": (ctypes.c_char_p, []),
    "dvh_default_options": (None, [ctypes.POINTER(Options)]),
    "dvh_create": (ctypes.c_int, [ctypes.c_int, ctypes.POINTER(Options), ctypes.POINTER(ctypes.c_void_p)]),
    "dvh_create_devices": (ctypes.c_int, [c_int32_p, ctypes.c_int32, ctypes.POINTER(Options),
                                          ctypes.POINTER(ctypes.c_void_p)]),
    "dvh_device_count": (ctypes.c_int, [ctypes.c_void_p]),
    "dvh_destroy": (ctypes.c_int, [ctypes.c_void_p]),
    "dvh_last_error": (ctypes.c_char_p, [ctypes.c_void_p]),
    "dvh_set_options": (ctypes.c_int, [ctypes.c_void_p, ctypes.POINTER(Options)]),
    "dvh_solve_batch": (ctypes.c_int, [ctypes.c_void_p, ctypes.POINTER(LP), ctypes.c_int32, ctypes.POINTER(Result)]),
    "dvh_certify_batch": (ctypes.c_int, [ctypes.c_void_p, ctypes.POINTER(LP), ctypes.c_int32, ctypes.POINTER(Result)]),
    "dvh_last_certify": (ctypes.c_int, [ctypes.c_void_p, c_int32_p]),
    "dvh_last_certify_ms": (ctypes.c_int, [ctypes.c_void_p, c_double_p]),
    "dvh_solve_packed_device": (ctypes.c_int, [ctypes.c_void_p, ctypes.POINTER(Packed), ctypes.c_void_p]),
    "dvh_warm_transfer": (ctypes.c_int, [ctypes.c_void_p, ctypes.POINTER(Packed), ctypes.c_void_p, ctypes.c_int32]),
    "dvh_warm_transfer_blend": (ctypes.c_int, [ctypes.c_void_p, ctypes.POINTER(Packed), ctypes.c_void_p,
                                               ctypes.c_void_p, ctypes.c_int32, ctypes.c_int32]),
    "dvh_build_battery_group": (ctypes.c_int, [ctypes.c_void_p, ctypes.POINTER(BatteryGroup), ctypes.POINTER(Packed),
                                               ctypes.c_int32]),
    "dvh_synchronize": (ctypes.c_int, [ctypes.c_void_p]),
    "dvh_series_draws": (ctypes.c_int, [ctypes.c_void_p, ctypes.POINTER(SweepDraws)]),
    "dvh_series_windows": (ctypes.c_int, [ctypes.c_void_p, ctypes.POINTER(WindowSeries)]),
    "dvh_last_timing": (ctypes.c_int, [ctypes.c_void_p, c_double_p]),
    "dvh_last_stats": (ctypes.c_int, [ctypes.c_void_p, c_int32_p]),
    "dvh_last_host_syncs": (ctypes.c_int, [ctypes.c_void_p, c_int32_p]),
    "dvh_last_path_counts": (ctypes.c_int, [ctypes.c_void_p, c_int32_p]),
    "dvh_last_path_counts4": (ctypes.c_int, [ctypes.c_void_p, c_int32_p]),
    "dvh_last_path_counts5": (ctypes.c_int, [ctypes.c_void_p, c_int32_p]),
    "dvh_last_band_variant": (ctypes.c_int, [ctypes.c_void_p, c_int32_p]),
    "dvh_last_chain_aborts": (ctypes.c_int, [ctypes.c_void_p, c_int32_p]),
    "dvh_last_warning": (ctypes.c_char_p, [ctypes.c_void_p]),
    "dvh_set_kernel_path": (ctypes.c_int, [ctypes.c_void_p, ctypes.c_int]),
    "dvh_set_launch_order": (ctypes.c_int, [ctypes.c_void_p, ctypes.c_void_p, ctypes.c_int32]),
    "dvh_outage_coverage": (ctypes.c_int, [ctypes.c_void_p, ctypes.POINTER(OutageCase), ctypes.c_int32, c_int32_p,
                                           c_double_p]),
    "dvh_outage_min_soe": (ctypes.c_int, [ctypes.c_void_p, ctypes.POINTER(OutageCase), ctypes.c_int32, c_int32_p,
                                          c_double_p]),
    "dvh_last_outage_ms": (ctypes.c_int, [ctypes.c_void_p, c_double_p]),
    "dvh_outage_first_uncovered": (ctypes.c_int, [ctypes.c_void_p, ctypes.POINTER(OutageCase), ctypes.c_int32,
                                                  c_int32_p, c_int32_p, c_int32_p]),
    "dvh_sizing_windows": (ctypes.c_int, [ctypes.c_void_p, ctypes.POINTER(OutageCase), ctypes.POINTER(SizingSpec),
                                          ctypes.c_int32, c_int32_p, c_int32_p, ctypes.POINTER(Result)]),
    "dvh_size_reliability": (ctypes.c_int, [ctypes.c_void_p, ctypes.POINTER(OutageCase), ctypes.POINTER(SizingSpec),
                                            ctypes.c_int32, ctypes.POINTER(SizingResult)]),
    "dvh_last_sizing_ms": (ctypes.c_int, [ctypes.c_void_p, c_double_p, c_double_p]),
    "dvh_cycle_damage": (ctypes.c_int, [ctypes.c_void_p, ctypes.c_void_p, ctypes.c_int64, ctypes.c_int32, ctypes.c_int32,
                                        ctypes.c_void_p, ctypes.c_void_p, ctypes.c_void_p, ctypes.c_int32,
                                        ctypes.c_void_p, ctypes.c_void_p]),
    "dvh_degradation_update": (ctypes.c_int, [ctypes.c_void_p, ctypes.POINTER(Packed), ctypes.c_int32, ctypes.c_int32,
                                              ctypes.c_int32, ctypes.c_int32, ctypes.c_double, ctypes.c_double,
                                              ctypes.c_void_p, ctypes.c_void_p, ctypes.c_int32,
                                              ctypes.POINTER(DegradationState), ctypes.c_void_p]),
    "dvh_bill_windows": (ctypes.c_int, [ctypes.c_void_p, ctypes.POINTER(BillGroup), ctypes.POINTER(Packed), ctypes.c_int32,
                                        ctypes.c_void_p, ctypes.c_void_p, ctypes.c_void_p, ctypes.c_void_p]),
    "dvh_value_scenarios": (ctypes.c_int, [ctypes.c_void_p, ctypes.POINTER(ValuationArgs), ctypes.c_void_p,
                                           ctypes.c_void_p, ctypes.c_void_p, ctypes.c_void_p]),
    "dvh_last_valuation_ms": (ctypes.c_int, [ctypes.c_void_p, c_double_p]),
    "dvh_value_cuts": (ctypes.c_int, [ctypes.c_void_p, ctypes.POINTER(BatteryGroup), ctypes.POINTER(Packed),
                                      ctypes.c_int32, ctypes.c_void_p, ctypes.c_void_p]),
    "dvh_value_master": (ctypes.c_int, [ctypes.c_void_p, ctypes.POINTER(ValueMasterArgs), ctypes.c_void_p]),
    "dvh_comm_unique_id": (ctypes.c_int, [ctypes.c_void_p, ctypes.c_char_p]),
    "dvh_comm_init": (ctypes.c_int, [ctypes.c_void_p, ctypes.c_int32, ctypes.c_int32, ctypes.c_char_p]),
    "dvh_comm_info": (ctypes.c_int, [ctypes.c_void_p, c_int32_p]),
    "dvh_gather_results": (ctypes.c_int, [ctypes.c_void_p, ctypes.c_void_p, ctypes.c_uint64, ctypes.c_void_p,
                                          ctypes.c_void_p]),
}
COMM_ID_BYTES = 128

_lib = None


def load(path=None):
    global _lib
    if _lib is not None and path is None:
        return _lib
    p = path or LIB_PATH
    if not os.path.exists(p):
        raise RuntimeError(f"libdervet_hip.so not found at {p}: build it with `python -m dervet_hip.build` "
                           "(there is no CPU fallback)")
    lib = ctypes.CDLL(p)
    for name, (res, args) in SYMBOLS.items():
        if (path is not None or os.environ.get("DVH_LIB")) and not hasattr(lib, name):
            continue
        f = getattr(lib, name)
        f.restype = res
        f.argtypes = args
    if path is None:
        _lib = lib
    return lib


def default_options(**kw):
    o = Options()
    load().dvh_default_options(ctypes.byref(o))
    for k, v in kw.items():
        if not hasattr(o, k):
            raise KeyError(f"unknown option {k}")
        setattr(o, k, v)
    return o
```

der-vet_amd/dervet_hip/build.py:

```python
import json
import os
import subprocess
import sys
from concurrent.futures import ThreadPoolExecutor

HERE = os.path.dirname(os.path.abspath(__file__))
CSRC = os.path.join(HERE, "..", "csrc")
LIB = os.path.join(HERE, "libdervet_hip.so")
BUILDINFO = os.path.join(HERE, "libdervet_hip.buildinfo.json")
SOURCES = ["dvh_kernels.hip", "dvh_band.hip", "dvh_band_persist.hip", "dvh_band_persist_ice.hip", "dvh_band_grid.hip", "dvh_chain.hip", "dvh_build.hip", "dvh_sweep.hip", "dvh_series.hip", "dvh_route.hip", "dvh_large.hip", "dvh_outage.hip",
           "dvh_certify.hip", "dvh_sizing.hip", "dvh_degradation.hip", "dvh_valuation.hip", "dvh_value_sizing.hip", "dvh_api.cpp", "dvh_api_outage.cpp", "dvh_api_build.cpp",
           "dvh_api_valuation.cpp", "dvh_api_value_sizing.cpp", "dvh_solve.cpp",
           "dvh_cascade.cpp", "dvh_validate.cpp", "dvh_comm.cpp", "dvh_sizing.cpp", "dvh_sizing_validate.cpp"]
EXTRA_FLAGS = {"dvh_band_persist.hip": ["-mllvm", "-disable-machine-licm", "-mllvm", "-amdgpu-use-amdgpu-trackers=1"],
               "dvh_band_persist_ice.hip": ["-mllvm", "-disable-machine-licm"],
               "dvh_chain.hip": ["-mllvm", "-disable-machine-licm"],
               "dvh_kernels.hip": ["-mllvm", "-disable-machine-licm"],
               "dvh_valuation.hip": ["-ffp-contract=off"],
               "dvh_value_sizing.hip": ["-ffp-contract=off"]}
INCLUDES = {"dvh_band_persist.hip": "dvh_band.hip",
            "dvh_band_persist_ice.hip": "dvh_band.hip"}
FLAGS = ["--offload-arch=gfx950", "-O3", "-std=c++17", "-fPIC", "-Wall", "-Wno-unused-result", "-Wno-unused-value"]
HEADERS = ["dvh_internal.h", "dvh_handle.h", "dvh_host.h", "dvh_device.h", "dvh_validate.h", "dvh_sizing_validate.h", "dvh_rng.h", "dvh_ziggurat.h", "dvh_rainflow.h", "dvh_degradation_validate.h", "dvh_cba.h", "dvh_valuation.h", "dvh_valuation_validate.h", "dvh_value_cut.h", "dvh_value_sizing.h", "dvh_value_sizing_validate.h", os.path.join("..", "..", "include", "dervet_hip.h")]


def _stale():
    if not os.path.exists(LIB):
        return True
    t = os.path.getmtime(LIB)
    return os.path.getmtime(os.path.abspath(__file__)) > t or \
        any(os.path.getmtime(os.path.join(CSRC, f)) > t for f in SOURCES + HEADERS)


def build(force=False, verbose=False):
    if not force and not _stale():
        if not os.path.exists(BUILDINFO):
            _write_buildinfo()
        return LIB
    hipcc = os.environ.get("HIPCC", "/opt/rocm/bin/hipcc")
    flags = list(FLAGS)
    objdir = os.path.join(HERE, "build_obj")
    os.makedirs(objdir, exist_ok=True)
    order = sorted(SOURCES, key=lambda f: -os.path.getsize(os.path.join(CSRC, INCLUDES.get(f, f))))
    objs = {f: os.path.join(objdir, f + ".o") for f in SOURCES}

    def compile_one(f):
        cmd = [hipcc, *flags, *EXTRA_FLAGS.get(f, []), "-c", os.path.join(CSRC, f), "-o", objs[f]]
        if verbose:
            print(" ".join(cmd), flush=True)
        return f, subprocess.run(cmd, capture_output=True, text=True)

    jobs = int(os.environ.get("DVH_BUILD_JOBS", min(len(SOURCES), os.cpu_count() or 1, 16)))
    with ThreadPoolExecutor(max_workers=max(1, jobs)) as ex:
        results = list(ex.map(compile_one, order))
    failed = [(f, r) for f, r in results if r.returncode != 0]
    for f, r in failed:
        sys.stderr.write(f"--- {f}\n" + r.stdout + r.stderr)
    if failed:
        raise RuntimeError("hipcc failed building libdervet_hip.so: " + ", ".join(f for f, _ in failed))
    cmd = [hipcc, "--offload-arch=gfx950", "-fPIC", "-shared", "-o", LIB + ".tmp"] + [objs[f] for f in SOURCES]
    r = subprocess.run(cmd, capture_output=True, text=True)
    if r.returncode != 0:
        sys.stderr.write(r.stdout + r.stderr)
        raise RuntimeError("hipcc failed linking libdervet_hip.so")
    os.replace(LIB + ".tmp", LIB)
    _write_buildinfo()
    return LIB


def _write_buildinfo():
    cfg = _current_config(compiler_version())
    with open(BUILDINFO + ".tmp", "w") as f:
        json.dump(cfg, f, sort_keys=True)
    os.replace(BUILDINFO + ".tmp", BUILDINFO)


def build_variant(out, defines, recompile=("dvh_band.hip", "dvh_band_persist.hip", "dvh_band_persist_ice.hip"),
                  verbose=False):
    build()
    hipcc = os.environ.get("HIPCC", "/opt/rocm/bin/hipcc")
    flags = [*FLAGS, *defines]
    name = os.path.splitext(os.path.basename(out))[0]
    objdir = os.path.join(HERE, "build_obj", name)
    os.makedirs(objdir, exist_ok=True)
    objs = {f: os.path.join(HERE, "build_obj", f + ".o") for f in SOURCES}

    def compile_one(f):
        objs[f] = os.path.join(objdir, f + ".o")
        cmd = [hipcc, *flags, *EXTRA_FLAGS.get(f, []), "-c", os.path.join(CSRC, f), "-o", objs[f]]
        if verbose:
            print(" ".join(cmd), flush=True)
        return f, subprocess.run(cmd, capture_output=True, text=True)

    with ThreadPoolExecutor(max_workers=max(1, len(recompile))) as ex:
        results = list(ex.map(compile_one, recompile))
    failed = [(f, r) for f, r in results if r.returncode != 0]
    for f, r in failed:
        sys.stderr.write(f"--- {f}\n" + r.stdout + r.stderr)
    if failed:
        raise RuntimeError("hipcc failed building variant " + name)
    os.makedirs(os.path.dirname(os.path.abspath(out)), exist_ok=True)
    cmd = [hipcc, "--offload-arch=gfx950", "-fPIC", "-shared", "-o", out] + [objs[f] for f in SOURCES]
    r = subprocess.run(cmd, capture_output=True, text=True)
    if r.returncode != 0:
        sys.stderr.write(r.stdout + r.stderr)
        raise RuntimeError("hipcc failed linking variant " + name)
    return out


def compiler_version():
    hipcc = os.environ.get("HIPCC", "/opt/rocm/bin/hipcc")
    try:
        r = subprocess.run([hipcc, "--version"], capture_output=True, text=True, timeout=60)
        lines = [ln.strip() for ln in r.stdout.splitlines() if ln.strip()]
        return " | ".join(ln for ln in lines if not ln.startswith("InstalledDir")) or "unknown"
    except (OSError, subprocess.SubprocessError):
        return "unknown"


def _current_config(compiler):
    return {"flags": FLAGS, "extra_flags": {k: EXTRA_FLAGS[k] for k in sorted(EXTRA_FLAGS)}, "compiler": compiler}


def build_config():
    try:
        with open(BUILDINFO) as f:
            rec = json.load(f)
        if rec == _current_config(rec.get("compiler")) and rec.get("compiler"):
            return rec
    except (OSError, ValueError):
        pass
    return _current_config(compiler_version())


if __name__ == "__main__":
    print(build(force="--force" in sys.argv, verbose=True))
```

der-vet_amd/dervet_hip/solver.py:

```python
import ctypes
from dataclasses import dataclass, field

import numpy as np

from . import _lib


@dataclass
class WindowLP:
    indptr: np.ndarray
    indices: np.ndarray
    data: np.ndarray
    c: np.ndarray
    q: np.ndarray
    l: np.ndarray
    u: np.ndarray
    m_eq: int
    c0: float = 0.0
    structure: int = 0
    meta: dict = field(default_factory=dict)

    @property
    def n(self):
        return len(self.c)

    @property
    def m(self):
        return len(self.q)

    @classmethod
    def from_csr(cls, K, q, c, l, u, m_eq, c0=0.0, **kw):
        K = K.tocsr()
        K.sort_indices()
        return cls(np.ascontiguousarray(K.indptr, np.int32), np.ascontiguousarray(K.indices, np.int32),
                   np.ascontiguousarray(K.data, np.float64), np.ascontiguousarray(c, np.float64),
                   np.ascontiguousarray(q, np.float64), np.ascontiguousarray(l, np.float64),
                   np.ascontiguousarray(u, np.float64), int(m_eq), float(c0), **kw)


@dataclass
class WindowResult:
    x: np.ndarray
    y: np.ndarray
    obj: float
    status: int
    iters: int
    primal_res_rel: float
    dual_res_rel: float
    gap_rel: float

    @property
    def status_name(self):
        return _lib.STATUS_NAMES.get(self.status, "solver_error")


class SolverError(RuntimeError):
    pass


def _init_torch_first():
    try:
        import torch
    except ImportError:
        return
    if torch.cuda.is_available():
        torch.cuda.init()


class BatchSolver:

    def __init__(self, device=0, devices=None, **options):
        _init_torch_first()
        self._lib = _lib.load()
        self._opts = _lib.default_options(**options)
        h = ctypes.c_void_p()
        if devices is None:
            rc = self._lib.dvh_create(1 << int(device), ctypes.byref(self._opts), ctypes.byref(h))
        else:
            arr = (ctypes.c_int32 * len(devices))(*[int(d) for d in devices])
            rc = self._lib.dvh_create_devices(arr, len(devices), ctypes.byref(self._opts), ctypes.byref(h))
        if rc != 0:
            raise SolverError(f"dvh_create failed ({rc}): no usable GPU device {devices or device} or invalid options")
        self._h = h

    @property
    def device_count(self):
        return int(self._lib.dvh_device_count(self._h))

    def close(self):
        if getattr(self, "_h", None):
            self._lib.dvh_destroy(self._h)
            self._h = None

    def __del__(self):
        try:
            self.close()
        except Exception:
            pass

    def __enter__(self):
        return self

    def __exit__(self, *a):
        self.close()

    def _check(self, rc, what):
        if rc != 0:
            msg = self._lib.dvh_last_error(self._h)
            raise SolverError(f"{what} failed ({rc}): {msg.decode() if msg else ''}")

    def options(self):
        o = type(self._opts)()
        ctypes.pointer(o)[0] = self._opts
        return o

    def set_options(self, **options):
        for k, v in options.items():
            setattr(self._opts, k, v)
        self._check(self._lib.dvh_set_options(self._h, ctypes.byref(self._opts)), "dvh_set_options")

    def timing(self):
        t = (ctypes.c_double * 3)()
        self._check(self._lib.dvh_last_timing(self._h, t), "dvh_last_timing")
        return {"total_ms": t[0], "setup_ms": t[1], "pdhg_ms": t[2]}

    def kernel_stats(self):
        v = (ctypes.c_int32 * 4)()
        self._check(self._lib.dvh_last_stats(self._h, v), "dvh_last_stats")
        c = (ctypes.c_int32 * 5)()
        self._check(self._lib.dvh_last_path_counts5(self._h, c), "dvh_last_path_counts5")
        a = ctypes.c_int32()
        self._check(self._lib.dvh_last_chain_aborts(self._h, ctypes.byref(a)), "dvh_last_chain_aborts")
        out = {"band_windows": c[3], "ell_windows": v[0], "generic_windows": v[1], "variant": v[2],
               "generic_only": bool(v[3]), "large_windows": c[2], "chain_windows": c[4],
               "chain_aborts": int(a.value)}
        if hasattr(self._lib, "dvh_last_band_variant"):
            bv = ctypes.c_int32()
            self._check(self._lib.dvh_last_band_variant(self._h, ctypes.byref(bv)), "dvh_last_band_variant")
            out["band_variant"] = int(bv.value)
        return out

    def last_warning(self):
        return (self._lib.dvh_last_warning(self._h) or b"").decode()

    def host_syncs(self):
        v = ctypes.c_int32()
        self._check(self._lib.dvh_last_host_syncs(self._h, ctypes.byref(v)), "dvh_last_host_syncs")
        return int(v.value)

    _PATHS = {"default": 0, "generic": 1, "ell": 2, "band1": 3, "band3": 4, "interconnect": 5}

    def set_kernel_path(self, path):
        mode = (1 if path else 0) if isinstance(path, bool) else self._PATHS[path]
        self._check(self._lib.dvh_set_kernel_path(self._h, mode), "dvh_set_kernel_path")

    def set_launch_order(self, order):
        o = np.ascontiguousarray(np.zeros(0, np.int32) if order is None else order, np.int32)
        self._check(self._lib.dvh_set_launch_order(self._h, o.ctypes.data_as(ctypes.c_void_p), len(o)),
                    "dvh_set_launch_order")

    def solve(self, lps, start=None):
        return self._batch_call("dvh_solve_batch", lps, start)

    def certify(self, lps):
        return self._batch_call("dvh_certify_batch", lps, None)

    def certify_stats(self):
        v = (ctypes.c_int32 * 5)()
        self._check(self._lib.dvh_last_certify(self._h, v), "dvh_last_certify")
        ms = ctypes.c_double()
        self._check(self._lib.dvh_last_certify_ms(self._h, ctypes.byref(ms)), "dvh_last_certify_ms")
        return {"examined": v[0], "primal_infeasible": v[1], "dual_infeasible": v[2], "skipped": v[3],
                "max_iters": v[4], "ms": float(ms.value)}

    def _batch_call(self, entry, lps, start):
        count = len(lps)
        if count == 0:
            return []
        keep = []
        arr = (_lib.LP * count)()
        res = (_lib.Result * count)()
        outs = []

        def ptr(a, t, ct):
            a = np.ascontiguousarray(a, dtype=t)
            keep.append(a)
            return a.ctypes.data_as(ct)

        for k, lp in enumerate(lps):
            m = lp.m
            if len(lp.indptr) != m + 1:
                raise ValueError(f"window {k}: indptr has {len(lp.indptr)} entries, expected m+1={m + 1}")
            L = arr[k]
            L.n, L.m_eq, L.m_ineq, L.nnz = lp.n, lp.m_eq, m - lp.m_eq, len(lp.indices)
            L.indptr = ptr(lp.indptr, np.int32, _lib.c_int32_p)
            L.indices = ptr(lp.indices, np.int32, _lib.c_int32_p)
            L.data = ptr(lp.data, np.float64, _lib.c_double_p)
            L.c = ptr(lp.c, np.float64, _lib.c_double_p)
            L.q = ptr(lp.q, np.float64, _lib.c_double_p)
            L.l = ptr(lp.l, np.float64, _lib.c_double_p)
            L.u = ptr(lp.u, np.float64, _lib.c_double_p)
            L.c0 = lp.c0
            L.structure = lp.structure
            x = np.zeros(lp.n)
            y = np.zeros(m)
            if start is not None and start[k] is not None:
                x[:] = start[k][0]
                y[:] = start[k][1]
            outs.append((x, y))
            res[k].x = x.ctypes.data_as(_lib.c_double_p)
            res[k].y = y.ctypes.data_as(_lib.c_double_p) if m else None
        self._check(getattr(self._lib, entry)(self._h, arr, count, res), entry)
        return [WindowResult(outs[k][0], outs[k][1], res[k].obj, res[k].status, res[k].iters, res[k].primal_res_rel,
                             res[k].dual_res_rel, res[k].gap_rel) for k in range(count)]

    def comm_unique_id(self):
        buf = ctypes.create_string_buffer(_lib.COMM_ID_BYTES)
        self._check(self._lib.dvh_comm_unique_id(self._h, buf), "dvh_comm_unique_id")
        return buf.raw

    def comm_init(self, rank, world, uid):
        if len(uid) != _lib.COMM_ID_BYTES:
            raise ValueError(f"a communicator id has {_lib.COMM_ID_BYTES} bytes, got {len(uid)}")
        self._check(self._lib.dvh_comm_init(self._h, int(rank), int(world), bytes(uid)), "dvh_comm_init")

    def comm_info(self):
        v = (ctypes.c_int32 * 2)()
        self._check(self._lib.dvh_comm_info(self._h, v), "dvh_comm_info")
        return int(v[0]), int(v[1])

    def gather_results(self, rows, out, stream=None):
        if not rows.is_contiguous() or not out.is_contiguous():
            raise ValueError("gather_results needs contiguous tensors")
        nb = rows.numel() * rows.element_size()
        world = self.comm_info()[1]
        if world and out.numel() * out.element_size() != nb * world:
            raise ValueError("out must hold world x the rows' bytes")
        s = getattr(stream, "cuda_stream", stream)
        self._check(self._lib.dvh_gather_results(self._h, ctypes.c_void_p(rows.data_ptr()), nb,
                                                 ctypes.c_void_p(out.data_ptr()), ctypes.c_void_p(s or 0)),
                    "dvh_gather_results")

    def solve_packed(self, pb, stream=None, sync=True):
        p = pb.as_ctypes()
        s = ctypes.c_void_p(stream) if stream else None
        self._check(self._lib.dvh_solve_packed_device(self._h, ctypes.byref(p), s), "dvh_solve_packed_device")
        if sync and stream:
            self._check(self._lib.dvh_synchronize(self._h), "dvh_synchronize")


def version():
    return _lib.load().dvh_version().decode()
```

der-vet_amd/dervet_hip/sweep.py:

```python
import os
from dataclasses import dataclass

import numpy as np

from .packed import PackedBatch


def seed_split(keys, stride, features=None, cover=False):
    keys = np.asarray(keys, np.float64)
    S = len(keys)
    stride = max(int(stride), 1)
    if stride == 1 or S < 2:
        return np.arange(S), np.zeros(0, np.int64), np.zeros(0, np.int64)
    order = np.argsort(keys, kind="stable")
    pos = np.arange(S)
    seed_pos = np.arange(min(stride // 2, S - 1), S, stride)
    is_seed = np.zeros(S, bool)
    is_seed[seed_pos] = True
    rest_pos = pos[~is_seed]
    near = np.clip(np.searchsorted(seed_pos, rest_pos), 0, len(seed_pos) - 1)
    left = np.clip(near - 1, 0, len(seed_pos) - 1)
    pick = np.where(np.abs(seed_pos[left] - rest_pos) <= np.abs(seed_pos[near] - rest_pos), left, near)
    seeds, rest = order[seed_pos], order[rest_pos]
    if features is not None:
        f = standardise(features, S)
        if cover:
            ns = len(seeds)
            sel = [int(seeds[0])]
            dmin = ((f - f[sel[0]]) ** 2).sum(1)
            for _ in range(ns - 1):
                j = int(dmin.argmax())
                sel.append(j)
                dmin = np.minimum(dmin, ((f - f[j]) ** 2).sum(1))
            seeds = np.array(sel, np.int64)
            mask = np.ones(S, bool)
            mask[seeds] = False
            rest = np.nonzero(mask)[0]
        pick = _nearest(f[rest], f[seeds])
    return seeds, rest, pick


def standardise(features, S=None):
    f = np.asarray(features, np.float64)
    f = f.reshape(S if S is not None else f.shape[0], -1)
    return (f - f.mean(0)) / np.where(f.std(0) > 0, f.std(0), 1.0)


def affine_weights(fr, fs, idx, w0, lam):
    F = fs[idx]
    q = idx.shape[1]
    A = F @ np.swapaxes(F, 1, 2) + lam * np.eye(q)[None]
    rhs = (F @ fr[:, :, None])[:, :, 0] + lam * w0
    one = np.ones((len(idx), q))
    sol = np.linalg.solve(A, np.stack([rhs, one], axis=2))
    ai, a1 = sol[:, :, 0], sol[:, :, 1]
    mu = (ai.sum(1) - 1.0) / a1.sum(1)
    return ai - mu[:, None] * a1


def seed_partners(fr, fs, q, first=None, power=1.0, lam=None):
    fr = np.ascontiguousarray(fr, np.float64)
    fs = np.ascontiguousarray(fs, np.float64)
    q = max(1, min(int(q), len(fs)))
    R = len(fr)
    idx = np.zeros((R, q), np.int64)
    w = np.zeros((R, q), np.float64)
    bb = (fs * fs).sum(1)
    for a in range(0, R, 2048):
        fa = fr[a:a + 2048]
        g = fa @ fs.T
        g *= -2.0
        g += bb[None, :]
        qc = min(q + 2, len(fs))
        cand = np.argpartition(g, qc - 1, axis=1)[:, :qc] if qc < len(fs) else np.tile(np.arange(len(fs)), (len(fa), 1))
        cand.sort(axis=1)
        dc = ((fa[:, None, :] - fs[cand]) ** 2).sum(-1)
        o = np.argsort(dc, axis=1, kind="stable")[:, :q]
        part = np.take_along_axis(cand, o, 1)
        d = np.zeros((len(fa), len(fs)))
        np.put_along_axis(d, part, np.take_along_axis(dc, o, 1), 1)
        if first is not None:
            f0 = np.asarray(first[a:a + 2048], np.int64)
            has = (part == f0[:, None]).any(1)
            part[~has, -1] = f0[~has]
            rs = np.nonzero(~has)[0]
            d[rs, f0[rs]] = ((fa[rs] - fs[f0[rs]]) ** 2).sum(1)
            part = np.take_along_axis(part, np.argsort(part != f0[:, None], axis=1, kind="stable"), 1)
        dd = np.sqrt(np.take_along_axis(d, part, 1))
        inv = np.where(dd > 0, 1.0 / np.where(dd > 0, dd, 1.0) ** power, np.inf)
        ww = np.where(np.isinf(inv).any(1, keepdims=True), np.isinf(inv).astype(np.float64), inv)
        w[a:a + 2048] = ww / ww.sum(1, keepdims=True)
        idx[a:a + 2048] = part
    if lam is not None and q > 1:
        w = affine_weights(fr, fs, idx, w, float(lam))
    return idx, w


def _nearest(fr, fs):
    fr = np.ascontiguousarray(fr, np.float64)
    fs = np.ascontiguousarray(fs, np.float64)
    if len(fr) == 0:
        return np.zeros(0, np.int64)
    bb = (fs * fs).sum(1)
    g = fr @ fs.T
    g *= -2.0
    g += bb[None, :]
    j0 = g.argmin(1)
    rows = np.arange(len(fr))
    tol = 1e-9 * ((fr * fr).sum(1) + bb.max() + 1.0)
    close = ((g <= (g[rows, j0] + tol)[:, None]).sum(1) > 1).nonzero()[0]
    for a in range(0, len(close), 1024):
        i = close[a:a + 1024]
        j0[i] = ((fr[i, None, :] - fs[None, :, :]) ** 2).sum(-1).argmin(1)
    return j0


WARM_OPTIONS = {"check_every": 64, "kkt_every": 1, "kkt_predict": 4}
SEED_OPTIONS = {"kkt_predict": 4}


@dataclass
class _Transfer:
    on_rest: int
    om_rest: int
    on_seed: int
    om_seed: int
    n: int
    m: int
    g_rest: int
    g_seed: int
    local: object
    battery_dcm: bool
    T: int
    w_rest: int = 0
    w_seed: int = 0
    weights: object = None


def _scenarios_of(g):
    s = getattr(g, "scen", None)
    if s is not None:
        return np.asarray(s, np.int64)
    return np.fromiter((t[0] for t in g.tags), np.int64, len(g.tags))


def _window_id(tag):
    return tag[1] if isinstance(tag, tuple) and len(tag) > 1 else tag


def _same_pattern(a, b):
    if a.n != b.n or a.m != b.m:
        return False
    if hasattr(a, "indices"):
        return np.array_equal(a.indices, b.indices) and np.array_equal(a.indptr, b.indptr)
    return a.T == b.T and np.array_equal(a.dcm_t, b.dcm_t) and np.array_equal(a.dcm_j, b.dcm_j)


def plan(seed_groups, rest_groups, partner_of, blend=None):
    out = []
    on = om = wk = 0
    seed_at = {}
    for g in seed_groups:
        seed_at[_window_id(g.tags[0])] = (g, on, om, wk)
        on += g.G * g.n
        om += g.G * g.m
        wk += g.G
    pk = np.fromiter(partner_of.keys(), np.int64, len(partner_of))
    pv = np.fromiter(partner_of.values(), np.int64, len(partner_of))
    po = np.argsort(pk, kind="stable")
    pk, pv = pk[po], pv[po]
    cols = {}
    if blend is not None:
        b_ids = np.asarray(blend[0], np.int64)
        b_ord = np.argsort(b_ids, kind="stable")
        b_ids = b_ids[b_ord]
        b_seed = np.asarray(blend[1], np.int64)[b_ord]
        b_w = np.asarray(blend[2], np.float64)[b_ord]
    for g in rest_groups:
        wid = _window_id(g.tags[0])
        if wid not in seed_at:
            raise ValueError(f"no seed group for window {wid!r}")
        sg, son, som, swk = seed_at[wid]
        if not _same_pattern(sg, g):
            raise ValueError(f"seed and rest groups of window {wid!r} differ in pattern")
        rs = _scenarios_of(g)
        i = np.minimum(np.searchsorted(pk, rs), max(len(pk) - 1, 0))
        if len(rs) and (len(pk) == 0 or not np.array_equal(pk[i], rs)):
            raise KeyError("a rest scenario has no partner seed")
        key = id(sg)
        if key not in cols:
            ss = _scenarios_of(sg)
            so = np.argsort(ss, kind="stable")
            cols[key] = (ss[so], so)
        ss, so = cols[key]
        want = pv[i]
        j = np.minimum(np.searchsorted(ss, want), max(len(ss) - 1, 0))
        if len(want) and (len(ss) == 0 or not np.array_equal(ss[j], want)):
            raise KeyError(f"a partner seed is not in the seed group of window {wid!r}")
        local = so[j].astype(np.int64)
        weights = None
        if blend is not None:
            ib = np.minimum(np.searchsorted(b_ids, rs), max(len(b_ids) - 1, 0))
            if len(rs) and (len(b_ids) == 0 or not np.array_equal(b_ids[ib], rs)):
                raise KeyError("a rest scenario has no blend partners")
            want_q = b_seed[ib]
            jq = np.minimum(np.searchsorted(ss, want_q), max(len(ss) - 1, 0))
            if want_q.size and (len(ss) == 0 or not np.array_equal(ss[jq], want_q)):
                raise KeyError(f"a blend partner is not in the seed group of window {wid!r}")
            local = so[jq].astype(np.int64)
            weights = b_w[ib]
        out.append(_Transfer(on, om, son, som, g.n, g.m, g.G, sg.G, local,
                             g.n == 3 * g.T + 1 and g.J == 1, g.T, wk, swk, weights))
        on += g.G * g.n
        om += g.G * g.m
        wk += g.G
    return out


def transfer_rows(tr_list):
    rows, wts = [], []
    for t in tr_list:
        loc = np.asarray(t.local, np.int64).reshape(t.g_rest, -1)
        q = loc.shape[1]
        r = np.empty((t.g_rest, q + 2), np.int32)
        r[:, 0] = t.w_rest + np.arange(t.g_rest)
        r[:, 1:q + 1] = t.w_seed + loc
        r[:, q + 1] = t.T if t.battery_dcm else 0
        rows.append(r)
        wts.append(np.ones((t.g_rest, 1)) if t.weights is None else np.asarray(t.weights, np.float64))
    if not rows:
        return np.zeros((0, 3), np.int32), np.zeros((0, 1))
    if len({r.shape[1] for r in rows}) != 1:
        raise ValueError("transfers with different partner counts")
    return np.ascontiguousarray(np.concatenate(rows)), np.ascontiguousarray(np.concatenate(wts))


def transfer_pairs(tr_list):
    parts = []
    for t in tr_list:
        if t.weights is not None:
            raise ValueError("blended transfers: use transfer_rows / dvh_warm_transfer_blend")
        p = np.empty((t.g_rest, 3), np.int32)
        p[:, 0] = t.w_rest + np.arange(t.g_rest)
        p[:, 1] = t.w_seed + np.asarray(t.local, np.int64)
        p[:, 2] = t.T if t.battery_dcm else 0
        parts.append(p)
    return np.ascontiguousarray(np.concatenate(parts)) if parts else np.zeros((0, 3), np.int32)


def transfer_device(solver, tr_list, pb, pairs=None, rows=None):
    import ctypes
    if pairs is None and any(t.weights is not None for t in tr_list):
        rows, wts = transfer_rows(tr_list) if rows is None else rows
        p = pb.as_ctypes()
        solver._check(solver._lib.dvh_warm_transfer_blend(
            solver._h, ctypes.byref(p), rows.ctypes.data_as(ctypes.c_void_p), wts.ctypes.data_as(ctypes.c_void_p),
            len(rows), rows.shape[1] - 2), "dvh_warm_transfer_blend")
        return
    pairs = transfer_pairs(tr_list) if pairs is None else np.ascontiguousarray(pairs, np.int32)
    if pairs.ndim != 2 or pairs.shape[1] != 3:
        raise ValueError(f"pairs must be [count, 3] {{window, partner, T}}, got shape {pairs.shape}")
    p = pb.as_ctypes()
    solver._check(solver._lib.dvh_warm_transfer(solver._h, ctypes.byref(p), pairs.ctypes.data_as(ctypes.c_void_p),
                                                len(pairs)), "dvh_warm_transfer")


def transfer(tr_list, x, y, c, u):
    import torch
    for t in tr_list:
        locs = np.asarray(t.local, np.int64).reshape(t.g_rest, -1)
        wts = None if t.weights is None else torch.as_tensor(np.asarray(t.weights, np.float64), device=x.device)
        Ur = u[t.on_rest:t.on_rest + t.g_rest * t.n].view(t.g_rest, t.n)
        Xb = Yb = None
        for k in range(locs.shape[1]):
            loc = torch.as_tensor(locs[:, k], device=x.device)
            Xs = x[t.on_seed:t.on_seed + t.g_seed * t.n].view(t.g_seed, t.n)[loc]
            Us = u[t.on_seed:t.on_seed + t.g_seed * t.n].view(t.g_seed, t.n)[loc]
            ok = torch.isfinite(Ur) & torch.isfinite(Us) & (Us > 0)
            ratio = torch.where(ok, Ur / torch.where(ok, Us, torch.ones_like(Us)), torch.ones_like(Us))
            Xk = Xs * ratio
            Ys = y[t.om_seed:t.om_seed + t.g_seed * t.m].view(t.g_seed, t.m)[loc]
            if t.battery_dcm:
                T = t.T
                Cs = c[t.on_seed:t.on_seed + t.g_seed * t.n].view(t.g_seed, t.n)[loc]
                Cr = c[t.on_rest:t.on_rest + t.g_rest * t.n].view(t.g_rest, t.n)
                cd = Cr[:, 3 * T:3 * T + 1] / Cs[:, 3 * T:3 * T + 1].clamp(min=1e-12)
                cp = Cr[:, :T].abs().mean(1, keepdim=True) / Cs[:, :T].abs().mean(1, keepdim=True).clamp(min=1e-12)
                Ys = torch.cat([Ys[:, :T + 1] * cp, Ys[:, T + 1:] * cd], dim=1)
            if wts is None:
                Xb, Yb = Xk, Ys
            else:
                wk = wts[:, k:k + 1]
                Xb = wk * Xk if Xb is None else Xb + wk * Xk
                Yb = wk * Ys if Yb is None else Yb + wk * Ys
        x[t.on_rest:t.on_rest + t.g_rest * t.n].view(t.g_rest, t.n).copy_(Xb)
        y[t.om_rest:t.om_rest + t.g_rest * t.m].view(t.g_rest, t.m).copy_(Yb)


def sub_batch(pb, a, b):
    return PackedBatch(desc=pb.desc[a:b], indptr=pb.indptr, indices=pb.indices, data=pb.data, c=pb.c,
                       c0=pb.c0[a:b], q=pb.q, l=pb.l, u=pb.u, x=pb.x, y=pb.y, stats=pb.stats[a:b],
                       istats=pb.istats[a:b])


class SeededSweep:

    def __init__(self, make_groups, scenario_ids, keys, stride=8, features=None, cover=False, blend=1,
                 blend_power=1.0, blend_lam=None):
        from .lp import builder
        ids = np.asarray(list(scenario_ids), np.int64)
        seed_i, rest_i, pick = seed_split(keys, stride, features, cover)
        self.seed_ids, self.rest_ids = ids[seed_i], ids[rest_i]
        partner_of = {int(r): int(self.seed_ids[p]) for r, p in zip(self.rest_ids, pick)}
        bl = None
        self.blend = 1
        if blend > 1 and features is not None and len(seed_i) > 1 and len(rest_i):
            f = standardise(features, len(ids))
            idx, w = seed_partners(f[rest_i], f[seed_i], blend, first=pick, power=blend_power, lam=blend_lam)
            self.blend = idx.shape[1]
            bl = (self.rest_ids, self.seed_ids[idx], w)
        sg = make_groups(self.seed_ids)
        rg = make_groups(self.rest_ids) if len(self.rest_ids) else []
        self.transfers = plan(sg, rg, partner_of, bl)
        self.pairs = transfer_pairs(self.transfers) if bl is None else None
        self.rows = transfer_rows(self.transfers) if bl is not None else None
        self._order_dev = None
        self.n_seed = sum(g.G for g in sg)
        self.tags = [t for g in sg + rg for t in g.tags]
        self.specs = None
        if sg and not hasattr(sg[0], "indices"):
            from .lp import gpu_builder
            self.specs, self.packed = sg + rg, None
            self.desc = gpu_builder.desc_of(self.specs)[0]
        else:
            self.packed = builder.pack_groups(sg + rg)
            self.desc = np.asarray(self.packed.desc)

    def to_device(self, solver, device):
        if self.specs is not None:
            from .lp import gpu_builder
            return gpu_builder.pack_specs_device(self.specs, solver, device)
        return self.packed.to_torch(device).alloc_outputs()

    def _order_warm(self, solver, dev):
        if self.rows is None or os.environ.get("DVH_SWEEP_ORDER", "1") == "0":
            return
        import torch
        rows, wts = self.rows
        n_rest = dev.count - self.n_seed
        if len(rows) != n_rest:
            return
        if self._order_dev is None or self._order_dev[0].device != dev.istats.device:
            self._order_dev = (torch.as_tensor(rows[:, 1:-1].astype(np.int64), device=dev.istats.device),
                               torch.as_tensor(wts, device=dev.istats.device),
                               torch.as_tensor(rows[:, 0].astype(np.int64) - self.n_seed, device=dev.istats.device))
        part, w, win = self._order_dev
        iters = dev.istats.view(-1, 2)[:, 1].to(torch.float64)
        if os.environ.get("DVH_SWEEP_ORDER") in ("prev", "prevasc"):
            pred = iters[win + self.n_seed] * (-1.0 if os.environ["DVH_SWEEP_ORDER"] == "prevasc" else 1.0)
        elif os.environ.get("DVH_SWEEP_ORDER") == "random":
            pred = torch.rand(len(win), generator=torch.Generator().manual_seed(7), dtype=torch.float64).to(win.device)
        else:
            pred = (w * iters[part]).sum(1)
        order = win[torch.argsort(pred, descending=True, stable=True)].to(torch.int32).cpu().numpy()
        solver.set_launch_order(order)

    def solve(self, solver, dev, warm_options=None, seed_options=None):
        cnt = dev.count
        o0 = solver.options()
        warm_options = dict(WARM_OPTIONS if warm_options is None else warm_options)
        seed_options = dict(SEED_OPTIONS if seed_options is None else seed_options)
        restore = {k: getattr(o0, k) for k in list(warm_options) + list(seed_options)}
        restore["warm_start"] = o0.warm_start
        tm = {"total_ms": 0.0, "setup_ms": 0.0, "pdhg_ms": 0.0}
        paths = {}

        def account():
            for k, v in solver.timing().items():
                tm[k] += v
            for k, v in solver.kernel_stats().items():
                if k.endswith("_windows"):
                    paths[k] = paths.get(k, 0) + v

        solver.set_options(warm_start=0, **seed_options)
        try:
            solver.solve_packed(sub_batch(dev, 0, self.n_seed))
        finally:
            solver.set_options(**restore)
        account()
        if cnt > self.n_seed:
            if dev.x.is_cuda and not os.environ.get("DVH_SWEEP_TORCH_TRANSFER"):
                transfer_device(solver, self.transfers, dev, self.pairs, self.rows)
                self._order_warm(solver, dev)
            else:
                transfer(self.transfers, dev.x, dev.y, dev.c, dev.u)
                if dev.x.is_cuda:
                    import torch
                    torch.cuda.synchronize(dev.x.device)
            solver.set_options(warm_start=1, **warm_options)
            try:
                solver.solve_packed(sub_batch(dev, self.n_seed, cnt))
            finally:
                solver.set_options(**restore)
            account()
        return tm, paths
```

include/dervet_hip.h:

```cpp
#ifndef DERVET_HIP_H
#define DERVET_HIP_H

#include <stdint.h>

#ifdef __cplusplus
extern "C" {
#endif

#define DVH_OK 0
#define DVH_ERR_ARG (-1)
#define DVH_ERR_HIP (-2)
#define DVH_ERR_UNSUPPORTED (-3)

#define DVH_OPTIMAL 0
#define DVH_PRIMAL_INFEASIBLE 1
#define DVH_DUAL_INFEASIBLE 2
#define DVH_ITER_LIMIT 3
#define DVH_NUMERICAL 4
#define DVH_UNDECIDED 5

#define DVH_STRUCT_GENERIC_CSR 0
#define DVH_STRUCT_BATTERY_BANDED 1

typedef struct dvh_options {
  double eps;
  int32_t max_iters;
  int32_t check_every;
  int32_t ruiz_iters;
  int32_t power_iters;
  double step_safety;
  double reflection;
  double restart_sufficient;
  double restart_necessary;
  double restart_artificial;
  double primal_weight_theta;
  int32_t verbose;
  int32_t kkt_every;
  int32_t warm_start;
  int32_t certify_iters;
  double eps_obj;
  int32_t kkt_predict;
  int32_t certify;
} dvh_options;

typedef struct dvh_lp {
  int32_t n;
  int32_t m_eq;
  int32_t m_ineq;
  int32_t nnz;
  const int32_t* indptr;
  const int32_t* indices;
  const double* data;
  const double* c;
  double c0;
  const double* q;
  const double* l;
  const double* u;
  int32_t structure;
  int32_t reserved;
} dvh_lp;

typedef struct dvh_result {
  double* x;
  double* y;
  double obj;
  double primal_res_rel;
  double dual_res_rel;
  double gap_rel;
  int32_t status;
  int32_t iters;
} dvh_result;

typedef struct dvh_packed {
  int32_t count;
  int32_t reserved;
  int64_t total_n, total_m, total_nnz, total_rows;
  const int64_t* desc;
  const int32_t* indptr;
  const int32_t* indices;
  const double* data;
  const double* c;
  const double* c0;
  const double* q;
  const double* l;
  const double* u;
  double* x;
  double* y;
  double* stats;
  int32_t* istats;
} dvh_packed;

typedef struct dvh_handle dvh_handle;

const char* dvh_version(void);
void dvh_default_options(dvh_options* opts);
int dvh_create(int device_mask, const dvh_options* opts, dvh_handle** out);
int dvh_create_devices(const int32_t* devices, int32_t n, const dvh_options* opts, dvh_handle** out);
int dvh_device_count(const dvh_handle* h);
int dvh_destroy(dvh_handle* h);
const char* dvh_last_error(const dvh_handle* h);
int dvh_set_options(dvh_handle* h, const dvh_options* opts);

#define DVH_COMM_ID_BYTES 128
int dvh_comm_unique_id(dvh_handle* h, uint8_t* id);
int dvh_comm_init(dvh_handle* h, int32_t rank, int32_t world, const uint8_t* id);
int dvh_comm_info(const dvh_handle* h, int32_t* rank_world);
int dvh_gather_results(dvh_handle* h, const void* rows, uint64_t bytes_per_rank, void* out, void* stream);

int dvh_solve_batch(dvh_handle* h, const dvh_lp* lps, int32_t count, dvh_result* out);

int dvh_solve_packed_device(dvh_handle* h, const dvh_packed* batch, void* stream);

typedef struct dvh_battery_group {
  int32_t T, J, G, mI;
  double dt;
  int32_t has_retail, has_da;
  int32_t has_emin, has_emax;
  const int32_t* dcm_t;
  const int32_t* dcm_j;
  const double* base;
  const double* retail;
  const double* da;
  const double* demand;
  const double* emin;
  const double* emax;
  const double* E;
  const double* pch;
  const double* pdis;
  const double* rte;
  const double* sdr;
  const double* soc_target;
  const double* ulsoc;
  const double* llsoc;
  const double* om;
  const double* c0;
  int32_t has_ice, pad_ice;
  const double* ice_cap;
  const double* ice_pmin;
  const double* ice_cost;
} dvh_battery_group;
int dvh_build_battery_group(dvh_handle* h, const dvh_battery_group* group, const dvh_packed* batch, int32_t first);
int dvh_synchronize(dvh_handle* h);

typedef struct dvh_sweep_draws {
  int32_t count, steps, n_uniform;
  const uint64_t* seeds;
  double a1;
  double innov;
  double* z0;
  double* ar;
  double* uniform;
  int32_t* ambiguous;
} dvh_sweep_draws;
int dvh_series_draws(dvh_handle* h, const dvh_sweep_draws* d);

typedef struct dvh_window_series {
  int32_t G, T, t0, rep, J, count, hours;
  double dt;
  const int32_t* rows;
  const double* ar;
  const double* site_load;
  const double* pv_profile;
  const double* price;
  const double* load_scale;
  const double* price_scale;
  const double* pv_rated;
  const double* hp;
  const double* c0_add;
  double* base;
  double* retail;
  double* c0;
} dvh_window_series;
int dvh_series_windows(dvh_handle* h, const dvh_window_series* w);

int dvh_warm_transfer(dvh_handle* h, const dvh_packed* batch, const int32_t* pairs, int32_t count);
int dvh_warm_transfer_blend(dvh_handle* h, const dvh_packed* batch, const int32_t* rows, const double* weights,
                            int32_t count, int32_t q);

int dvh_certify_batch(dvh_handle* h, const dvh_lp* lps, int32_t count, dvh_result* out);
int dvh_last_certify(const dvh_handle* h, int32_t* out5);
int dvh_last_certify_ms(const dvh_handle* h, double* ms);

int dvh_last_timing(const dvh_handle* h, double* ms3);

int dvh_last_host_syncs(const dvh_handle* h, int32_t* out);
int dvh_last_stats(const dvh_handle* h, int32_t* out4);
int dvh_last_path_counts(const dvh_handle* h, int32_t* out3);
int dvh_last_path_counts4(const dvh_handle* h, int32_t* out4);
int dvh_last_path_counts5(const dvh_handle* h, int32_t* out5);
int dvh_last_band_variant(const dvh_handle* h, int32_t* out);
int dvh_last_chain_aborts(const dvh_handle* h, int32_t* out);
const char* dvh_last_warning(const dvh_handle* h);
typedef struct dvh_outage_case {
  int32_t n_steps;
  int32_t max_outage;
  double dt;
  const double* critical_load;
  const double* pv_max;
  const double* pv_vari;
  const double* init_soe;
  const double* load_shed_pct;
  double soe0;
  double dg_gen;
  double gamma;
  double soe_min, soe_max;
  double charge_max, discharge_max;
  double rte;
} dvh_outage_case;

int dvh_outage_coverage(dvh_handle* h, const dvh_outage_case* cases, int32_t count, int32_t* lengths,
                        double* lcp);
int dvh_outage_min_soe(dvh_handle* h, const dvh_outage_case* cases, int32_t count, const int32_t* target_hours,
                       double* min_soe);
int dvh_last_outage_ms(const dvh_handle* h, double* ms);

int dvh_outage_first_uncovered(dvh_handle* h, const dvh_outage_case* cases, int32_t count, const int32_t* target_steps,
                               int32_t* first, int32_t* n_uncovered);

typedef struct dvh_sizing_spec {
  double target_hours;
  int32_t size_energy, size_power;
  double ccost, ccost_kw, ccost_kwh;
  double energy_min, energy_max;
  double power_min, power_max;
  double energy, power;
  double llsoc, ulsoc, soc_init;
  int32_t n_seed, max_rounds;
} dvh_sizing_spec;

int dvh_sizing_windows(dvh_handle* h, const dvh_outage_case* cases, const dvh_sizing_spec* specs, int32_t count,
                       const int32_t* starts, const int32_t* n_starts, dvh_result* out);

#define DVH_SIZING_SIZED 0
#define DVH_SIZING_ROUND_LIMIT 1
#define DVH_SIZING_STALLED 2
#define DVH_SIZING_LP_FAILED 3
typedef struct dvh_sizing_result {
  double energy, power;
  double capex;
  int32_t status;
  int32_t lp_status;
  int32_t rounds;
  int32_t n_starts;
  int32_t lp_iters;
  int32_t reserved;
  int32_t* starts;
} dvh_sizing_result;

int dvh_size_reliability(dvh_handle* h, const dvh_outage_case* cases, const dvh_sizing_spec* specs, int32_t count,
                         dvh_sizing_result* out);
int dvh_last_sizing_ms(const dvh_handle* h, double* ms, double* out3);

#define DVH_RAINFLOW_MAX_T 20351
#define DVH_RAINFLOW_MAX_TABLE 64
int dvh_cycle_damage(dvh_handle* h, const double* ene, int64_t row_stride, int32_t S, int32_t T, const double* e_rated,
                     const double* upper, const double* life, int32_t n_table, double* damage_out, void* stream);

typedef struct dvh_degradation_state {
  int32_t incl_cycle_degrade;
  int32_t reserved;
  const double* e_rated;
  const double* yearly;
  const double* soh;
  const int32_t* replaceable;
  double* degrade_perc;
  int64_t* replacements;
  int64_t* skipped;
  double* capacity;
  double* degradation;
  int32_t* reached;
} dvh_degradation_state;

int dvh_degradation_update(dvh_handle* h, const dvh_packed* batch, int32_t first, int32_t S, int32_t T,
                           int32_t ene_col, double days, double eol_condition, const double* upper, const double* life,
                           int32_t n_table, const dvh_degradation_state* state, void* stream);

#define DVH_BILL_ROWS 8
#define DVH_BILL_MAX_J 16
typedef struct dvh_bill_group {
  int32_t T, J, G, mI;
  double dt;
  int32_t has_pv, has_ice;
  const int32_t* dcm_t;
  const int32_t* dcm_j;
  const double* base;
  const double* orig;
  const double* retail;
  const double* da;
  const double* demand;
  const double* om;
  const double* ice_cost;
} dvh_bill_group;
int dvh_bill_windows(dvh_handle* h, const dvh_bill_group* group, const dvh_packed* batch, int32_t first,
                     double* bills, double* peaks, int32_t* bad, void* stream);

#define DVH_CBA_MAX_YEARS 64
#define DVH_CBA_MAX_EXTRA 16
#define DVH_CBA_FIXED_COLS 7
#define DVH_VALUE_COLS 7
typedef struct dvh_valuation {
  int32_t S, Y, n_opt, n_extra;
  int64_t n_win, n_bills;
  const int32_t* opt_years;
  const int64_t* win_ptr_host;
  const int64_t* win_ptr;
  const int32_t* win_idx;
  const int32_t* win_year;
  const double* bills;
  const int32_t* bad;
  double rate;
  double growth[5];
  const double* capex;
  const double* fixed_om;
  const double* extra;
} dvh_valuation;
int dvh_value_scenarios(dvh_handle* h, const dvh_valuation* v, double* values, int32_t* valid, double* proforma,
                        void* stream);
int dvh_last_valuation_ms(const dvh_handle* h, double* ms2);

#define DVH_VALUE_CUT_COLS 10
#define DVH_VALUE_MAX_J 64
#define DVH_VALUE_MAX_CUTS 256
#define DVH_VALUE_MAX_CAND 8
int dvh_value_cuts(dvh_handle* h, const dvh_battery_group* group, const dvh_packed* batch, int32_t first,
                   double* cuts_out, void* stream);

typedef struct dvh_value_spec {
  int32_t size_energy, size_power;
  double c_energy, c_power;
  double c_fixed;
  double alpha;
  double energy_min, energy_max;
  double power_min, power_max;
  double gap_tol;
  int32_t max_rounds, reserved;
} dvh_value_spec;

#define DVH_VALUE_SIZED 0
#define DVH_VALUE_ROUND_LIMIT 1
#define DVH_VALUE_LP_FAILED 2
#define DVH_VALUE_MASTER_FAILED 3
#define DVH_VALUE_STATE_COLS 8
#define DVH_VS_LOWER 0
#define DVH_VS_UPPER 1
#define DVH_VS_INC_E 2
#define DVH_VS_INC_P 3
#define DVH_VS_INC_V 4
#define DVH_VS_Z_E 5
#define DVH_VS_Z_P 6
#define DVH_VS_THETA 7
#define DVH_VALUE_FLAG_COLS 8
#define DVH_VF_DONE 0
#define DVH_VF_STATUS 1
#define DVH_VF_LP_STATUS 2
#define DVH_VF_NCUTS 3
#define DVH_VF_ROUNDS 4
#define DVH_VF_LP_ITERS 5
#define DVH_VF_MASTER 6

typedef struct dvh_value_master_args {
  int32_t count, n_cases, W, n_cand, n_next, cut_cap;
  const dvh_value_spec* spec_host;
  const dvh_value_spec* spec;
  const int32_t* case_ids;
  const double* window_cuts;
  const double* E_in;
  const double* P_in;
  double* cuts;
  double* state;
  int32_t* flags;
  double* E_out;
  double* pch_out;
  double* pdis_out;
} dvh_value_master_args;
int dvh_value_master(dvh_handle* h, const dvh_value_master_args* args, void* stream);

int dvh_set_kernel_path(dvh_handle* h, int mode);

int dvh_set_launch_order(dvh_handle* h, const int32_t* order, int32_t count);

#ifdef __cplusplus
}
#endif
#endif
```

Before: 353,500.

## Fuse seed and warm sweep solves into a single cached device-side seeded plan

Adds a seeded-plan API that precomputes chunk plans and warm-transfer rows once and runs the seed solve, the warm transfer and the warm solve in one native call. The cascade is split into front and finish stages, and the persistent-queue memset can be skipped when the caller has already reset the queue. The aim is to cut Python round trips, host syncs, per-call planning and redundant launches between the seed and warm phases. It adds plan lifetime management keyed by solver and handle, plus a fallback path that must stay consistent with the old flow.

```diff
diff --git a/der-vet_amd/csrc/dvh_band.hip b/der-vet_amd/csrc/dvh_band.hip
--- a/der-vet_amd/csrc/dvh_band.hip
+++ b/der-vet_amd/csrc/dvh_band.hip
@@ -1478,7 +1478,7 @@
 
 template <int B, int S, bool ICE, bool LC, int WPS, bool GATE, bool BOX, bool PERSIST>
 hipError_t launch_band_one_q(const Batch& b, const Work& w, const Chunk& ch, const Opts& o, hipStream_t s,
-                             const int32_t* list, int nlist, int* variant_out) {
+                             const int32_t* list, int nlist, int* variant_out, bool queue_set = false) {
   static_assert(B * S == kBandSteps, "every form covers T <= kBandSteps");
   const size_t lds = band_lds_bytes(B, S, ICE, LC);
   auto kern = pdhg_band_kernel<B, S, ICE, LC, WPS, GATE, BOX, PERSIST>;
@@ -1510,7 +1510,7 @@
     }
     static const int reserve = [] { const char* e = getenv("DVH_BAND_RESERVE"); return e ? std::max(0, atoi(e)) : 0; }();
     grid = std::min(count, std::max(1, slots - 2 * reserve));
-    if ((e = hipMemsetAsync(w.queue, 0, sizeof(int32_t), s)) != hipSuccess) return e;
+    if (!queue_set && (e = hipMemsetAsync(w.queue, 0, sizeof(int32_t), s)) != hipSuccess) return e;
   }
   const BandArgs args{b, w, ch, o, list, count, w.queue};
   hipLaunchKernelGGL(kern, dim3(grid), dim3(B), lds, s, args);
@@ -1519,27 +1519,27 @@
 }
 template <int B, int S, bool ICE, bool LC, int WPS, bool GATE, bool BOX>
 hipError_t launch_band_one_g(const Batch& b, const Work& w, const Chunk& ch, const Opts& o, hipStream_t s,
-                             const int32_t* list, int nlist, bool j1, int* variant_out) {
+                             const int32_t* list, int nlist, bool j1, int* variant_out, bool queue_set) {
   if constexpr (S == 3 && !ICE) {
     static_assert(B == kBandSteps / 3 && LC && WPS == 2, "dvh_band_persist.hip instantiates this form");
     const char* q = getenv("DVH_BAND_QUEUE");
-    if (!(q && atoi(q) == 0)) return launch_band_persist(GATE, BOX, j1, b, w, ch, o, s, list, nlist, variant_out);
+    if (!(q && atoi(q) == 0)) return launch_band_persist(GATE, BOX, j1, b, w, ch, o, s, list, nlist, variant_out, queue_set);
   }
   if constexpr (ICE) {
     static_assert(B == kBandSteps && S == 1 && !LC && WPS == 3, "dvh_band_persist_ice.hip instantiates this form");
     const char* q = getenv("DVH_BAND_QUEUE");
     const char* qi = getenv("DVH_BAND_QUEUE_ICE");
     if (!(q && atoi(q) == 0) && !(qi && atoi(qi) == 0))
-      return launch_band_persist_ice(GATE, BOX, b, w, ch, o, s, list, nlist, variant_out);
+      return launch_band_persist_ice(GATE, BOX, b, w, ch, o, s, list, nlist, variant_out, queue_set);
   }
   return launch_band_one_q<B, S, ICE, LC, WPS, GATE, BOX, false>(b, w, ch, o, s, list, nlist, variant_out);
 }
 template <int B, int S, bool ICE, bool LC, int WPS, bool BOX = false>
 hipError_t launch_band_one(const Batch& b, const Work& w, const Chunk& ch, const Opts& o, hipStream_t s,
-                           const int32_t* list, int nlist, bool j1, int* variant_out) {
+                           const int32_t* list, int nlist, bool j1, int* variant_out, bool queue_set) {
   if (o.kkt_predict > 0)
-    return launch_band_one_g<B, S, ICE, LC, WPS, true, BOX>(b, w, ch, o, s, list, nlist, j1, variant_out);
-  return launch_band_one_g<B, S, ICE, LC, WPS, false, BOX>(b, w, ch, o, s, list, nlist, j1, variant_out);
+    return launch_band_one_g<B, S, ICE, LC, WPS, true, BOX>(b, w, ch, o, s, list, nlist, j1, variant_out, queue_set);
+  return launch_band_one_g<B, S, ICE, LC, WPS, false, BOX>(b, w, ch, o, s, list, nlist, j1, variant_out, queue_set);
 }
 
 }
@@ -1548,7 +1548,7 @@
 namespace {
 template <bool GATE, bool BOX>
 hipError_t launch_band_persist_j1(const Batch& b, const Work& w, const Chunk& ch, const Opts& o, hipStream_t s,
-                                  const int32_t* list, int nlist, int* variant_out) {
+                                  const int32_t* list, int nlist, int* variant_out, bool queue_set) {
   constexpr int B = kBandSteps / 3, S = 3;
   const size_t lds = band_lds_bytes(B, S, false, true);
   auto kern = pdhg_band_kernel_j1<B, S, false, true, 2, GATE, BOX>;
@@ -1566,7 +1566,7 @@
   }
   static const int reserve = [] { const char* e = getenv("DVH_BAND_RESERVE"); return e ? std::max(0, atoi(e)) : 0; }();
   const int grid = std::min(count, std::max(1, slots - 2 * reserve));
-  if ((e = hipMemsetAsync(w.queue, 0, sizeof(int32_t), s)) != hipSuccess) return e;
+  if (!queue_set && (e = hipMemsetAsync(w.queue, 0, sizeof(int32_t), s)) != hipSuccess) return e;
   const BandArgs args{b, w, ch, o, list, count, w.queue};
   hipLaunchKernelGGL(kern, dim3(grid), dim3(B), lds, s, args);
   if (variant_out) *variant_out = 9000000 + 1000 * (S - 1) + kBandJ1 + B / kWave;
@@ -1574,7 +1574,8 @@
 }
 }
 hipError_t launch_band_persist(bool gate, bool box, bool j1, const Batch& b, const Work& w, const Chunk& ch,
-                               const Opts& o, hipStream_t s, const int32_t* list, int nlist, int* variant_out) {
+                               const Opts& o, hipStream_t s, const int32_t* list, int nlist, int* variant_out,
+                               bool queue_set) {
   constexpr int B = kBandSteps / 3;
   if (j1) {
     const char* e = getenv("DVH_BAND_J1");
@@ -1582,43 +1583,44 @@
   }
   if (j1) {
     if (gate) {
-      if (box) return launch_band_persist_j1<true, true>(b, w, ch, o, s, list, nlist, variant_out);
-      return launch_band_persist_j1<true, false>(b, w, ch, o, s, list, nlist, variant_out);
-    }
-    if (box) return launch_band_persist_j1<false, true>(b, w, ch, o, s, list, nlist, variant_out);
-    return launch_band_persist_j1<false, false>(b, w, ch, o, s, list, nlist, variant_out);
+      if (box) return launch_band_persist_j1<true, true>(b, w, ch, o, s, list, nlist, variant_out, queue_set);
+      return launch_band_persist_j1<true, false>(b, w, ch, o, s, list, nlist, variant_out, queue_set);
+    }
+    if (box) return launch_band_persist_j1<false, true>(b, w, ch, o, s, list, nlist, variant_out, queue_set);
+    return launch_band_persist_j1<false, false>(b, w, ch, o, s, list, nlist, variant_out, queue_set);
   }
   if (gate) {
-    if (box) return launch_band_one_q<B, 3, false, true, 2, true, true, true>(b, w, ch, o, s, list, nlist, variant_out);
-    return launch_band_one_q<B, 3, false, true, 2, true, false, true>(b, w, ch, o, s, list, nlist, variant_out);
-  }
-  if (box) return launch_band_one_q<B, 3, false, true, 2, false, true, true>(b, w, ch, o, s, list, nlist, variant_out);
-  return launch_band_one_q<B, 3, false, true, 2, false, false, true>(b, w, ch, o, s, list, nlist, variant_out);
+    if (box) return launch_band_one_q<B, 3, false, true, 2, true, true, true>(b, w, ch, o, s, list, nlist, variant_out, queue_set);
+    return launch_band_one_q<B, 3, false, true, 2, true, false, true>(b, w, ch, o, s, list, nlist, variant_out, queue_set);
+  }
+  if (box) return launch_band_one_q<B, 3, false, true, 2, false, true, true>(b, w, ch, o, s, list, nlist, variant_out, queue_set);
+  return launch_band_one_q<B, 3, false, true, 2, false, false, true>(b, w, ch, o, s, list, nlist, variant_out, queue_set);
 }
 #elif DVH_BAND_PERSIST_TU == 2
 hipError_t launch_band_persist_ice(bool gate, bool box, const Batch& b, const Work& w, const Chunk& ch, const Opts& o,
-                                   hipStream_t s, const int32_t* list, int nlist, int* variant_out) {
+                                   hipStream_t s, const int32_t* list, int nlist, int* variant_out, bool queue_set) {
   constexpr int B = kBandSteps;
   if (gate) {
-    if (box) return launch_band_one_q<B, 1, true, false, 3, true, true, true>(b, w, ch, o, s, list, nlist, variant_out);
-    return launch_band_one_q<B, 1, true, false, 3, true, false, true>(b, w, ch, o, s, list, nlist, variant_out);
-  }
-  if (box) return launch_band_one_q<B, 1, true, false, 3, false, true, true>(b, w, ch, o, s, list, nlist, variant_out);
-  return launch_band_one_q<B, 1, true, false, 3, false, false, true>(b, w, ch, o, s, list, nlist, variant_out);
+    if (box) return launch_band_one_q<B, 1, true, false, 3, true, true, true>(b, w, ch, o, s, list, nlist, variant_out, queue_set);
+    return launch_band_one_q<B, 1, true, false, 3, true, false, true>(b, w, ch, o, s, list, nlist, variant_out, queue_set);
+  }
+  if (box) return launch_band_one_q<B, 1, true, false, 3, false, true, true>(b, w, ch, o, s, list, nlist, variant_out, queue_set);
+  return launch_band_one_q<B, 1, true, false, 3, false, false, true>(b, w, ch, o, s, list, nlist, variant_out, queue_set);
 }
 #else
 hipError_t launch_pdhg_band(const Batch& b, const Work& w, const Chunk& ch, const Opts& o, hipStream_t s, bool ice,
-                            int form, bool box, const int32_t* list, int nlist, bool j1, int* variant_out) {
+                            int form, bool box, const int32_t* list, int nlist, bool j1, int* variant_out,
+                            bool queue_set) {
   if (ice) {
-    if (box) return launch_band_one<kBandSteps, 1, true, false, 3, true>(b, w, ch, o, s, list, nlist, false, variant_out);
-    return launch_band_one<kBandSteps, 1, true, false, 3>(b, w, ch, o, s, list, nlist, false, variant_out);
+    if (box) return launch_band_one<kBandSteps, 1, true, false, 3, true>(b, w, ch, o, s, list, nlist, false, variant_out, queue_set);
+    return launch_band_one<kBandSteps, 1, true, false, 3>(b, w, ch, o, s, list, nlist, false, variant_out, queue_set);
   }
   if (form == 1) {
-    if (box) return launch_band_one<kBandSteps, 1, false, false, 3, true>(b, w, ch, o, s, list, nlist, false, variant_out);
-    return launch_band_one<kBandSteps, 1, false, false, 3>(b, w, ch, o, s, list, nlist, false, variant_out);
-  }
-  if (box) return launch_band_one<kBandSteps / 3, 3, false, true, 2, true>(b, w, ch, o, s, list, nlist, j1, variant_out);
-  return launch_band_one<kBandSteps / 3, 3, false, true, 2>(b, w, ch, o, s, list, nlist, j1, variant_out);
+    if (box) return launch_band_one<kBandSteps, 1, false, false, 3, true>(b, w, ch, o, s, list, nlist, false, variant_out, queue_set);
+    return launch_band_one<kBandSteps, 1, false, false, 3>(b, w, ch, o, s, list, nlist, false, variant_out, queue_set);
+  }
+  if (box) return launch_band_one<kBandSteps / 3, 3, false, true, 2, true>(b, w, ch, o, s, list, nlist, j1, variant_out, queue_set);
+  return launch_band_one<kBandSteps / 3, 3, false, true, 2>(b, w, ch, o, s, list, nlist, j1, variant_out, queue_set);
 }
 #endif
 
diff --git a/der-vet_amd/csrc/dvh_cascade.cpp b/der-vet_amd/csrc/dvh_cascade.cpp
--- a/der-vet_amd/csrc/dvh_cascade.cpp
+++ b/der-vet_amd/csrc/dvh_cascade.cpp
@@ -138,36 +138,69 @@
   return DVH_OK;
 }
 
-int device_cascade(dvh_handle* h, const dvh::Batch& b, const dvh::Work& w, const dvh::Chunk& ch, const dvh::Opts& o,
-                   int nsmall, int nj, int wc, int mn, int mm, hipStream_t s, const int32_t* order) {
-  const size_t I = sizeof(int32_t);
-  int32_t* L[5];
-  for (int r = 0; r < 5; ++r) L[r] = h->d_list.as<int32_t>() + (size_t)r * wc;
-  int32_t* info = h->d_route.as<int32_t>();
-  int32_t* rh = h->route_host.as<int32_t>();
+namespace {
+
+struct CascadeEnv {
+  int forced_form, cus;
+  int form_for(int nl) const { return forced_form ? forced_form : (nl <= cus ? 1 : 3); }
+};
+CascadeEnv cascade_env(dvh_handle* h) {
   if (h->cus <= 0 && hipDeviceGetAttribute(&h->cus, hipDeviceAttributeMultiprocessorCount, h->device) != hipSuccess)
     h->cus = 256;
-  const int forced_form = h->kernel_path == 3 ? 1 : h->kernel_path == 4 ? 3 : 0;
-  auto form_for = [&](int nl) { return forced_form ? forced_form : (nl <= h->cus ? 1 : 3); };
-  auto route = [&](int slot, const int32_t* in, int n_in, int want, int cls, int out) -> hipError_t {
-    return dvh::launch_route(b.desc, b.istats, w.scal, ch.first, n_in, in, want, dvh::kSmallMax, cls, 512, 768,
-                             L[out], info + 8 * slot, s);
-  };
-  auto readback = [&](int slot0, int nslots) -> hipError_t {
-    hipError_t e = hipMemcpyAsync(rh + 8 * slot0, info + 8 * slot0, 8 * I * nslots, hipMemcpyDeviceToHost, s);
-    return e != hipSuccess ? e : sync_stream(h, s);
-  };
-  const bool j1 = nj == 0;
-  int variant = -1, bvar = -1;
+  return CascadeEnv{h->kernel_path == 3 ? 1 : h->kernel_path == 4 ? 3 : 0, h->cus};
+}
+hipError_t route(const CascadeRun& r, const dvh::Batch& b, const dvh::Work& w, const dvh::Chunk& ch, hipStream_t s,
+                 int slot, const int32_t* in, int n_in, int want, int cls, int out) {
+  return dvh::launch_route(b.desc, b.istats, w.scal, ch.first, n_in, in, want, dvh::kSmallMax, cls, 512, 768,
+                           r.L[out], r.info + 8 * slot, s);
+}
+hipError_t readback(dvh_handle* h, const CascadeRun& r, hipStream_t s, int slot0, int nslots) {
+  hipError_t e = hipMemcpyAsync(r.rh + 8 * slot0, r.info + 8 * slot0, 8 * sizeof(int32_t) * nslots,
+                                hipMemcpyDeviceToHost, s);
+  return e != hipSuccess ? e : sync_stream(h, s);
+}
+
+}
+
+CascadeRun cascade_run(dvh_handle* h, int wc) {
+  CascadeRun r;
+  for (int i = 0; i < 5; ++i) r.L[i] = h->d_list.as<int32_t>() + (size_t)i * wc;
+  r.info = h->d_route.as<int32_t>();
+  r.rh = h->route_host.as<int32_t>();
+  return r;
+}
+
+int cascade_front(dvh_handle* h, const dvh::Batch& b, const dvh::Work& w, const dvh::Chunk& ch, const dvh::Opts& o,
+                  int nj, hipStream_t s, const int32_t* order, bool queue_set, CascadeRun& r) {
+  const CascadeEnv env = cascade_env(h);
+  r.j1 = nj == 0;
+  r.bvar = -1;
   h->last_band_variant = -1;
-  auto form_code = [](int v) { return v >= 0 && v % 100 >= dvh::kBandJ1 ? v - dvh::kBandJ1 : v; };
   const char* box_env = getenv("DVH_BAND_BOX");
   const int box_mode = box_env ? atoi(box_env) : 1;
-  const bool box = box_mode >= 1, box_ice = box_mode >= 2;
-  DVH_HIP(h, dvh::launch_pdhg_band(b, w, ch, o, s, false, form_for(ch.count), box, order, order ? ch.count : 0, j1, &bvar));
-  DVH_HIP(h, route(0, nullptr, ch.count, -2, 0, 0));
-  if (box) DVH_HIP(h, route(1, nullptr, ch.count, -3, 0, 1));
-  DVH_HIP(h, readback(0, box ? 2 : 1));
+  r.box = box_mode >= 1;
+  r.box_ice = box_mode >= 2;
+  DVH_HIP(h, dvh::launch_pdhg_band(b, w, ch, o, s, false, env.form_for(ch.count), r.box, order, order ? ch.count : 0,
+                                   r.j1, &r.bvar, queue_set));
+  DVH_HIP(h, route(r, b, w, ch, s, 0, nullptr, ch.count, -2, 0, 0));
+  if (r.box) DVH_HIP(h, route(r, b, w, ch, s, 1, nullptr, ch.count, -3, 0, 1));
+  return DVH_OK;
+}
+
+int cascade_finish(dvh_handle* h, const dvh::Batch& b, const dvh::Work& w, const dvh::Chunk& ch, const dvh::Opts& o,
+                   int nsmall, int mn, int mm, hipStream_t s, CascadeRun& r) {
+  const size_t I = sizeof(int32_t);
+  const CascadeEnv env = cascade_env(h);
+  auto form_for = [&](int nl) { return env.form_for(nl); };
+  int32_t** L = r.L;
+  int32_t* rh = r.rh;
+  auto route = [&](int slot, const int32_t* in, int n_in, int want, int cls, int out) -> hipError_t {
+    return dvh::route(r, b, w, ch, s, slot, in, n_in, want, cls, out);
+  };
+  auto readback = [&](int slot0, int nslots) -> hipError_t { return dvh::readback(h, r, s, slot0, nslots); };
+  const bool j1 = r.j1, box = r.box, box_ice = r.box_ice;
+  int variant = -1, bvar = r.bvar;
+  auto form_code = [](int v) { return v >= 0 && v % 100 >= dvh::kBandJ1 ? v - dvh::kBandJ1 : v; };
   if (box && rh[8] > 0) {
     DVH_HIP(h, dvh::launch_pdhg_band(b, w, ch, o, s, false, form_for(rh[8]), false, L[1], rh[8], j1, nullptr));
     DVH_HIP(h, route(0, nullptr, ch.count, -2, 0, 0));
@@ -254,4 +287,12 @@
   return DVH_OK;
 }
 
-}
+int device_cascade(dvh_handle* h, const dvh::Batch& b, const dvh::Work& w, const dvh::Chunk& ch, const dvh::Opts& o,
+                   int nsmall, int nj, int wc, int mn, int mm, hipStream_t s, const int32_t* order) {
+  CascadeRun r = cascade_run(h, wc);
+  if (int rc = cascade_front(h, b, w, ch, o, nj, s, order, false, r)) return rc;
+  DVH_HIP(h, readback(h, r, s, 0, r.box ? 2 : 1));
+  return cascade_finish(h, b, w, ch, o, nsmall, mn, mm, s, r);
+}
+
+}
diff --git a/der-vet_amd/csrc/dvh_handle.h b/der-vet_amd/csrc/dvh_handle.h
--- a/der-vet_amd/csrc/dvh_handle.h
+++ b/der-vet_amd/csrc/dvh_handle.h
@@ -91,6 +91,7 @@
   std::vector<int32_t> order_used;
   DevBuf d_order;
   std::vector<dvh_handle*> peers;
+  std::vector<dvh::SeededPlanOwner> seeded_plans;
   PinnedBuf route_host, cert_host;
 };
 
@@ -116,6 +117,44 @@
 
 namespace dvh {
 
+struct ChunkPlan {
+  Chunk ch;
+  int64_t sn, sm, snz;
+  int mn, mm;
+  int64_t mnz;
+  int nsmall;
+  int nj;
+  std::vector<int32_t> med;
+  int med_T = 0;
+};
+struct BatchPlan {
+  std::vector<ChunkPlan> chunks;
+  std::vector<int> large;
+  int64_t wn = 0, wm = 0, wnz = 0;
+  int wc = 0;
+};
+Opts make_opts(const dvh_options& p);
+Batch make_batch(const dvh_packed& bt);
+std::string check_descriptors(const dvh_packed& bt, const std::vector<int64_t>& desc);
+BatchPlan scan_chunks(const std::vector<int64_t>& desc, int count, bool chain_on);
+int make_work(dvh_handle* h, const BatchPlan& p, Work& w);
+int next_chunk_events(dvh_handle* h, const DevEvent*& out);
+void certify_reset(dvh_handle* h);
+void collect_timing(dvh_handle* h);
+
+struct CascadeRun {
+  int32_t* L[5];
+  int32_t* info;
+  int32_t* rh;
+  bool j1 = false, box = false, box_ice = false;
+  int bvar = -1;
+};
+CascadeRun cascade_run(dvh_handle* h, int wc);
+int cascade_front(dvh_handle* h, const Batch& b, const Work& w, const Chunk& ch, const Opts& o, int nj, hipStream_t s,
+                  const int32_t* order, bool queue_set, CascadeRun& r);
+int cascade_finish(dvh_handle* h, const Batch& b, const Work& w, const Chunk& ch, const Opts& o, int nsmall, int mn,
+                   int mm, hipStream_t s, CascadeRun& r);
+
 int device_cascade(dvh_handle* h, const Batch& b, const Work& w, const Chunk& ch, const Opts& o, int nsmall, int nj, int wc,
                    int mn, int mm, hipStream_t s, const int32_t* order);
 int chain_pass(dvh_handle* h, const Batch& b, const Work& w, const Chunk& ch, const Opts& o,
diff --git a/der-vet_amd/csrc/dvh_internal.h b/der-vet_amd/csrc/dvh_internal.h
--- a/der-vet_amd/csrc/dvh_internal.h
+++ b/der-vet_amd/csrc/dvh_internal.h
@@ -104,13 +104,16 @@
                            int wx, int wy, hipStream_t s, int* variant_out, const int32_t* list, int nlist,
                            bool latency = false);
 hipError_t launch_pdhg_band(const Batch& b, const Work& w, const Chunk& ch, const Opts& o, hipStream_t s, bool ice,
-                            int form, bool box, const int32_t* list, int nlist, bool j1, int* variant_out);
+                            int form, bool box, const int32_t* list, int nlist, bool j1, int* variant_out,
+                            bool queue_set = false);
 constexpr int kBandJ1 = 50;
 constexpr int kBandJMax = 4;
 hipError_t launch_band_persist(bool gate, bool box, bool j1, const Batch& b, const Work& w, const Chunk& ch,
-                               const Opts& o, hipStream_t s, const int32_t* list, int nlist, int* variant_out);
+                               const Opts& o, hipStream_t s, const int32_t* list, int nlist, int* variant_out,
+                               bool queue_set = false);
 hipError_t launch_band_persist_ice(bool gate, bool box, const Batch& b, const Work& w, const Chunk& ch, const Opts& o,
-                                   hipStream_t s, const int32_t* list, int nlist, int* variant_out);
+                                   hipStream_t s, const int32_t* list, int nlist, int* variant_out,
+                                   bool queue_set = false);
 size_t setup_lds_bytes(int max_n, int max_m);
 hipError_t launch_setup_medium(const Batch& b, const Work& w, const Chunk& ch, const Opts& o, int max_n,
                                const int32_t* list, int nlist, hipStream_t s);
@@ -129,7 +132,13 @@
                         hipStream_t s);
 constexpr int kMaxBlend = 8;
 hipError_t launch_warm_transfer(const int64_t* desc, const double* c, const double* u, double* x, double* y,
-                                const int32_t* rows, const double* wts, int q, int count, int32_t* bad, hipStream_t s);
+                                const int32_t* rows, const double* wts, int q, int count, int32_t* bad, hipStream_t s,
+                                const int32_t* guard = nullptr);
+hipError_t launch_seeded_guard(const int32_t* info, int box, int32_t* queue, int32_t* guard, hipStream_t s);
+hipError_t seeded_order_temp_bytes(int count, size_t* bytes);
+hipError_t launch_seeded_order(const int32_t* rows, const double* wts, int q, int count, int first,
+                               const int32_t* istats, double* keys, double* keys_out, int32_t* vals, int32_t* order,
+                               void* temp, size_t temp_bytes, hipStream_t s);
 hipError_t launch_series_draws(const uint64_t* seeds, int count, int steps, int n_unif, double a1, double innov,
                                double* z0, double* ar, double* unif, int32_t* ambiguous, int32_t* amb_rows,
                                hipStream_t s);
@@ -179,7 +188,10 @@
   template <class T>
   void operator()(T* p) const { Destroy(p); }
 };
+struct SeededPlan;
+void seeded_plan_destroy(SeededPlan* p);
 using LargeOwner = std::unique_ptr<LargeSolver, DestroyWith<large_destroy>>;
+using SeededPlanOwner = std::unique_ptr<SeededPlan, DestroyWith<seeded_plan_destroy>>;
 using CommOwner = std::unique_ptr<Comm, DestroyWith<comm_destroy>>;
 
 struct HandleView {
diff --git a/der-vet_amd/csrc/dvh_seeded.cpp b/der-vet_amd/csrc/dvh_seeded.cpp
--- /dev/null
+++ b/der-vet_amd/csrc/dvh_seeded.cpp
@@ -0,0 +1,273 @@
+#include <cmath>
+#include <cstdlib>
+
+#include "dvh_handle.h"
+
+namespace dvh {
+
+struct SeededPlan {
+  dvh_packed bt{};
+  int n_seed = 0, n_rest = 0, q = 1;
+  BatchPlan seed, rest, both;
+  DevBuf rows, wts, bad, guard;
+  DevBuf keys, keys_out, vals, order, temp;
+  size_t temp_bytes = 0;
+  DevBuf lists, info;
+  PinnedBuf rh;
+  bool ordered = false;
+};
+void seeded_plan_destroy(SeededPlan* p) { delete p; }
+
+namespace {
+
+SeededPlan* find_plan(dvh_handle* h, const dvh_seeded_plan* p) {
+  for (const SeededPlanOwner& o : h->seeded_plans)
+    if ((const void*)o.get() == (const void*)p) return o.get();
+  return nullptr;
+}
+
+bool same_batch(const dvh_packed& a, const dvh_packed& b) {
+  return a.count == b.count && a.total_n == b.total_n && a.total_m == b.total_m && a.total_nnz == b.total_nnz &&
+         a.total_rows == b.total_rows && a.desc == b.desc && a.indptr == b.indptr && a.indices == b.indices &&
+         a.data == b.data && a.c == b.c && a.c0 == b.c0 && a.q == b.q && a.l == b.l && a.u == b.u && a.x == b.x &&
+         a.y == b.y && a.stats == b.stats && a.istats == b.istats;
+}
+
+dvh_packed sub_batch(const dvh_packed& bt, int first, int count) {
+  dvh_packed v = bt;
+  v.count = count;
+  v.desc = bt.desc + 8 * (int64_t)first;
+  v.c0 = bt.c0 + first;
+  v.stats = bt.stats + 4 * (int64_t)first;
+  v.istats = bt.istats + 2 * (int64_t)first;
+  return v;
+}
+
+bool one_small_chunk(const BatchPlan& p, int count) {
+  return p.chunks.size() == 1 && p.large.empty() && p.chunks[0].nsmall == count && p.chunks[0].med.empty();
+}
+
+CascadeRun plan_run(const SeededPlan& p, int pass) {
+  CascadeRun r;
+  const int n = pass == 0 ? p.n_seed : p.n_rest;
+  int32_t* base = p.lists.as<int32_t>() + (pass == 0 ? 0 : 5 * (size_t)p.n_seed);
+  for (int i = 0; i < 5; ++i) r.L[i] = base + (size_t)i * n;
+  r.info = p.info.as<int32_t>() + 40 * pass;
+  r.rh = p.rh.as<int32_t>() + 40 * pass;
+  return r;
+}
+
+bool refused(const CascadeRun& r) { return r.rh[0] > 0 || (r.box && r.rh[8] > 0); }
+
+}
+}
+
+extern "C" {
+
+int dvh_seeded_plan_create(dvh_handle* h, const dvh_packed* bt, int32_t n_seed, const int32_t* rows,
+                           const double* weights, int32_t count, int32_t q, dvh_seeded_plan** out) {
+  if (!h) return DVH_ERR_ARG;
+  if (!out) return fail(h, DVH_ERR_ARG, "seeded plan: null result pointer");
+  *out = nullptr;
+  if (q < 1 || q > dvh::kMaxBlend) return fail(h, DVH_ERR_ARG, "seeded plan: partners per window must be 1..8");
+  if (!bt || bt->count <= 0 || n_seed <= 0 || n_seed > bt->count || count < 0 || (count > 0 && (!rows || !weights)))
+    return fail(h, DVH_ERR_ARG, "seeded plan: bad arguments");
+  if (!bt->desc || !bt->indptr || !bt->c || !bt->c0 || !bt->l || !bt->u || !bt->x || !bt->y || !bt->stats || !bt->istats)
+    return fail(h, DVH_ERR_ARG, "null device array in packed batch");
+  DVH_HIP(h, hipSetDevice(h->device));
+  hipStream_t s = h->stream;
+  std::vector<int64_t> desc(8 * (size_t)bt->count);
+  DVH_HIP(h, hipMemcpyAsync(desc.data(), bt->desc, desc.size() * sizeof(int64_t), hipMemcpyDeviceToHost, s));
+  DVH_HIP(h, hipStreamSynchronize(s));
+  const std::string bad = dvh::check_descriptors(*bt, desc);
+  if (!bad.empty()) return fail(h, DVH_ERR_ARG, bad);
+  const size_t R = (size_t)q + 2;
+  const int n_rest = bt->count - n_seed;
+  std::vector<char> target((size_t)bt->count, 0);
+  for (int32_t i = 0; i < count; ++i) {
+    const std::string at = "seeded plan: row " + std::to_string(i);
+    const int32_t w = rows[R * i], T = rows[R * i + q + 1];
+    if (w < n_seed || w >= bt->count)
+      return fail(h, DVH_ERR_ARG, at + " lists window " + std::to_string(w) + ", which is not one of " +
+                                      std::to_string(n_seed) + " .. " + std::to_string(bt->count - 1));
+    if (target[w]) return fail(h, DVH_ERR_ARG, at + ": window " + std::to_string(w) + " listed twice");
+    target[w] = 1;
+    const int64_t n = desc[8 * (size_t)w], m = desc[8 * (size_t)w + 1];
+    if (T > 0 && (3 * (int64_t)T + 1 != n || (int64_t)T + 1 > m))
+      return fail(h, DVH_ERR_ARG, at + ": T = " + std::to_string(T) + " is not window " + std::to_string(w) + "'s shape");
+    for (int32_t k = 0; k < q; ++k) {
+      const int32_t p = rows[R * i + 1 + k];
+      if (p < 0 || p >= n_seed)
+        return fail(h, DVH_ERR_ARG, at + ": partner " + std::to_string(p) + " is not a seed (0 .. " +
+                                        std::to_string(n_seed - 1) + ")");
+      if (!std::isfinite(weights[(size_t)q * i + k])) return fail(h, DVH_ERR_ARG, at + ": weight is not finite");
+      if (desc[8 * (size_t)p] != n || desc[8 * (size_t)p + 1] != m)
+        return fail(h, DVH_ERR_ARG, at + ": partner " + std::to_string(p) + " is of another shape than window " +
+                                        std::to_string(w));
+    }
+  }
+  for (int w = n_seed; w < bt->count; ++w)
+    if (!target[w]) return fail(h, DVH_ERR_ARG, "seeded plan: window " + std::to_string(w) + " is listed by no row");
+  dvh::SeededPlanOwner po(new dvh::SeededPlan);
+  dvh::SeededPlan& p = *po;
+  p.bt = *bt;
+  p.n_seed = n_seed;
+  p.n_rest = n_rest;
+  p.q = q;
+  p.seed = dvh::scan_chunks(desc, n_seed, false);
+  if (!dvh::one_small_chunk(p.seed, n_seed))
+    return fail(h, DVH_ERR_UNSUPPORTED, "seeded plan: the seeds are not one chunk of on-chip windows");
+  p.both.wn = p.seed.wn;
+  p.both.wm = p.seed.wm;
+  p.both.wnz = p.seed.wnz;
+  p.both.wc = p.seed.wc;
+  if (n_rest > 0) {
+    const std::vector<int64_t> dr(desc.begin() + 8 * (size_t)n_seed, desc.end());
+    p.rest = dvh::scan_chunks(dr, n_rest, false);
+    if (!dvh::one_small_chunk(p.rest, n_rest))
+      return fail(h, DVH_ERR_UNSUPPORTED, "seeded plan: the warm windows are not one chunk of on-chip windows");
+    p.both.wn = std::max(p.both.wn, p.rest.wn);
+    p.both.wm = std::max(p.both.wm, p.rest.wm);
+    p.both.wnz = std::max(p.both.wnz, p.rest.wnz);
+    p.both.wc = std::max(p.both.wc, p.rest.wc);
+  }
+  const size_t I = sizeof(int32_t), D = sizeof(double);
+  DVH_HIP(h, p.lists.ensure(I * 5 * (size_t)bt->count));
+  DVH_HIP(h, p.info.ensure(I * 80));
+  DVH_HIP(h, p.rh.ensure(I * 80));
+  DVH_HIP(h, p.bad.ensure(I));
+  DVH_HIP(h, p.guard.ensure(I));
+  DVH_HIP(h, hipMemsetAsync(p.info.p, 0, I * 80, s));
+  DVH_HIP(h, hipMemsetAsync(p.bad.p, 0, I, s));
+  DVH_HIP(h, hipMemsetAsync(p.guard.p, 0, I, s));
+  if (n_rest > 0) {
+    DVH_HIP(h, p.rows.ensure(I * R * (size_t)n_rest));
+    DVH_HIP(h, p.wts.ensure(D * (size_t)q * (size_t)n_rest));
+    DVH_HIP(h, hipMemcpyAsync(p.rows.p, rows, I * R * (size_t)n_rest, hipMemcpyHostToDevice, s));
+    DVH_HIP(h, hipMemcpyAsync(p.wts.p, weights, D * (size_t)q * (size_t)n_rest, hipMemcpyHostToDevice, s));
+    DVH_HIP(h, p.keys.ensure(D * (size_t)n_rest));
+    DVH_HIP(h, p.keys_out.ensure(D * (size_t)n_rest));
+    DVH_HIP(h, p.vals.ensure(I * (size_t)n_rest));
+    DVH_HIP(h, p.order.ensure(I * (size_t)n_rest));
+    DVH_HIP(h, dvh::seeded_order_temp_bytes(n_rest, &p.temp_bytes));
+    DVH_HIP(h, p.temp.ensure(std::max<size_t>(p.temp_bytes, 1)));
+  }
+  DVH_HIP(h, hipStreamSynchronize(s));
+  *out = reinterpret_cast<dvh_seeded_plan*>(po.get());
+  h->seeded_plans.push_back(std::move(po));
+  return DVH_OK;
+}
+
+int dvh_seeded_plan_destroy(dvh_handle* h, dvh_seeded_plan* plan) {
+  if (!h) return DVH_ERR_ARG;
+  if (!plan) return DVH_OK;
+  for (size_t i = 0; i < h->seeded_plans.size(); ++i) {
+    if ((void*)h->seeded_plans[i].get() != (void*)plan) continue;
+    DVH_HIP(h, hipSetDevice(h->device));
+    DVH_HIP(h, hipStreamSynchronize(h->stream));
+    h->seeded_plans.erase(h->seeded_plans.begin() + i);
+    return DVH_OK;
+  }
+  return fail(h, DVH_ERR_ARG, "seeded plan: not a plan of this handle");
+}
+
+int dvh_seeded_plan_order(dvh_handle* h, const dvh_seeded_plan* plan, int32_t* out, int32_t count, int32_t* ordered) {
+  if (!h) return DVH_ERR_ARG;
+  const dvh::SeededPlan* p = plan ? dvh::find_plan(h, plan) : nullptr;
+  if (!p || !out || !ordered || count != p->n_rest) return fail(h, DVH_ERR_ARG, "seeded plan order: bad arguments");
+  *ordered = p->ordered ? 1 : 0;
+  if (!p->ordered) return DVH_OK;
+  DVH_HIP(h, hipSetDevice(h->device));
+  DVH_HIP(h, hipStreamSynchronize(h->stream));
+  DVH_HIP(h, hipMemcpy(out, p->order.p, sizeof(int32_t) * (size_t)count, hipMemcpyDeviceToHost));
+  return DVH_OK;
+}
+
+int dvh_solve_seeded_device(dvh_handle* h, dvh_seeded_plan* plan, const dvh_packed* bt, const dvh_options* seed_opts,
+                            const dvh_options* warm_opts, void* stream) {
+  if (!h) return DVH_ERR_ARG;
+  dvh::SeededPlan* pp = plan ? dvh::find_plan(h, plan) : nullptr;
+  if (!pp) return fail(h, DVH_ERR_ARG, "seeded step: not a plan of this handle");
+  if (!bt || !seed_opts || !warm_opts) return fail(h, DVH_ERR_ARG, "seeded step: null batch or options");
+  dvh::SeededPlan& p = *pp;
+  if (!dvh::same_batch(p.bt, *bt)) return fail(h, DVH_ERR_ARG, "seeded step: the batch is not the one the plan was made for");
+  if (h->kernel_path == 1 || h->kernel_path == 2 || seed_opts->reflection != 1.0 || warm_opts->reflection != 1.0 ||
+      seed_opts->certify != 0 || warm_opts->certify != 0)
+    return fail(h, DVH_ERR_UNSUPPORTED, "seeded step: the device cascade only (no A/B kernel path, reflection 1, no certify)");
+  DVH_HIP(h, hipSetDevice(h->device));
+  hipStream_t s = stream ? static_cast<hipStream_t>(stream) : h->stream;
+  h->n_syncs = 0;
+  dvh::certify_reset(h);
+  h->order.clear();
+  dvh::Opts os = dvh::make_opts(*seed_opts), ow = dvh::make_opts(*warm_opts);
+  os.warm = 0;
+  ow.warm = 1;
+  const dvh_packed vs = dvh::sub_batch(*bt, 0, p.n_seed), vr = dvh::sub_batch(*bt, p.n_seed, p.n_rest);
+  const dvh::Batch bs = dvh::make_batch(vs), br = dvh::make_batch(vr);
+  dvh::Work w;
+  if (int rc = dvh::make_work(h, p.both, w)) return rc;
+  h->st.reset();
+  const dvh::ChunkPlan& cs = p.seed.chunks[0];
+  const char* oe = getenv("DVH_SWEEP_ORDER");
+  p.ordered = p.n_rest > 0 && !(oe && std::string(oe) == "0");
+  const int32_t* order = p.ordered ? p.order.as<int32_t>() : nullptr;
+  auto enqueue_order = [&]() -> hipError_t {
+    if (!p.ordered) return hipSuccess;
+    return dvh::launch_seeded_order(p.rows.as<int32_t>(), p.wts.as<double>(), p.q, p.n_rest, p.n_seed, bt->istats,
+                                    p.keys.as<double>(), p.keys_out.as<double>(), p.vals.as<int32_t>(),
+                                    p.order.as<int32_t>(), p.temp.p, p.temp_bytes, s);
+  };
+  auto enqueue_transfer = [&](const int32_t* guard) -> hipError_t {
+    return dvh::launch_warm_transfer(bt->desc, bt->c, bt->u, bt->x, bt->y, p.rows.as<int32_t>(), p.wts.as<double>(),
+                                     p.q, p.n_rest, p.bad.as<int32_t>(), s, guard);
+  };
+  DVH_HIP(h, hipEventRecord(h->ev[0], s));
+  dvh::CascadeRun rs = dvh::plan_run(p, 0), rr = dvh::plan_run(p, 1);
+  const DevEvent* ce = nullptr;
+  if (int rc = dvh::next_chunk_events(h, ce)) return rc;
+  DVH_HIP(h, hipEventRecord(ce[0], s));
+  DVH_HIP(h, hipEventRecord(ce[1], s));
+  if (int rc = dvh::cascade_front(h, bs, w, cs.ch, os, cs.nj, s, nullptr, false, rs)) return rc;
+  DVH_HIP(h, hipEventRecord(ce[2], s));
+  if (p.n_rest > 0) {
+    const dvh::ChunkPlan& cr = p.rest.chunks[0];
+    DVH_HIP(h, dvh::launch_seeded_guard(rs.info, rs.box ? 1 : 0, w.queue, p.guard.as<int32_t>(), s));
+    DVH_HIP(h, enqueue_order());
+    DVH_HIP(h, enqueue_transfer(p.guard.as<int32_t>()));
+    if (int rc = dvh::next_chunk_events(h, ce)) return rc;
+    DVH_HIP(h, hipEventRecord(ce[0], s));
+    DVH_HIP(h, hipEventRecord(ce[1], s));
+    if (int rc = dvh::cascade_front(h, br, w, cr.ch, ow, cr.nj, s, order, true, rr)) return rc;
+    DVH_HIP(h, hipEventRecord(ce[2], s));
+  }
+  DVH_HIP(h, hipMemcpyAsync(p.rh.p, p.info.p, sizeof(int32_t) * 80, hipMemcpyDeviceToHost, s));
+  DVH_HIP(h, hipEventRecord(h->ev[3], s));
+  DVH_HIP(h, sync_stream(h, s));
+  const bool seed_refused = dvh::refused(rs);
+  const bool warm_refused = !seed_refused && p.n_rest > 0 && dvh::refused(rr);
+  if (seed_refused || warm_refused) {
+    if (int rc = dvh::next_chunk_events(h, ce)) return rc;
+    DVH_HIP(h, hipEventRecord(ce[0], s));
+    DVH_HIP(h, hipEventRecord(ce[1], s));
+  }
+  if (int rc = dvh::cascade_finish(h, bs, w, cs.ch, os, cs.nsmall, cs.mn, cs.mm, s, rs)) return rc;
+  if (p.n_rest > 0) {
+    const dvh::ChunkPlan& cr = p.rest.chunks[0];
+    if (seed_refused) {
+      DVH_HIP(h, enqueue_order());
+      DVH_HIP(h, enqueue_transfer(nullptr));
+      if (int rc = dvh::device_cascade(h, br, w, cr.ch, ow, cr.nsmall, cr.nj, p.both.wc, cr.mn, cr.mm, s, order)) return rc;
+    } else {
+      if (int rc = dvh::cascade_finish(h, br, w, cr.ch, ow, cr.nsmall, cr.mn, cr.mm, s, rr)) return rc;
+    }
+  }
+  if (seed_refused || warm_refused) {
+    DVH_HIP(h, hipEventRecord(ce[2], s));
+    DVH_HIP(h, hipEventRecord(h->ev[3], s));
+    DVH_HIP(h, sync_stream(h, s));
+  }
+  dvh::collect_timing(h);
+  return DVH_OK;
+}
+
+}
diff --git a/der-vet_amd/csrc/dvh_solve.cpp b/der-vet_amd/csrc/dvh_solve.cpp
--- a/der-vet_amd/csrc/dvh_solve.cpp
+++ b/der-vet_amd/csrc/dvh_solve.cpp
@@ -5,10 +5,12 @@
 #include "dvh_validate.h"
 
 namespace {
-
 constexpr int kChunkWindows = 262144;
-
-dvh::Opts make_opts(const dvh_options& p) {
+}
+
+namespace dvh {
+
+Opts make_opts(const dvh_options& p) {
   dvh::Opts o;
   o.eps = p.eps;
   o.eps_obj = p.eps_obj;
@@ -29,10 +31,34 @@
   return o;
 }
 
-dvh::Batch make_batch(const dvh_packed& bt) {
+Batch make_batch(const dvh_packed& bt) {
   return dvh::Batch{bt.desc, bt.indptr, bt.indices, bt.data, bt.c, bt.c0, bt.q, bt.l, bt.u,
                     bt.x, bt.y, bt.stats, bt.istats};
 }
+
+std::string check_descriptors(const dvh_packed& bt, const std::vector<int64_t>& desc) {
+  for (int k = 0; k < bt.count; ++k) {
+    const int64_t* d = &desc[8 * (size_t)k];
+    if (d[0] <= 0 || d[1] < 0 || d[2] < 0 || d[2] > d[1] || d[3] < 0 || d[4] < 0 || d[5] < 0 || d[6] < 0 || d[7] < 0 ||
+        d[4] + d[1] + 1 > bt.total_rows || d[5] + d[3] > bt.total_nnz || d[6] + d[0] > bt.total_n ||
+        d[7] + d[1] > bt.total_m)
+      return "packed descriptor " + std::to_string(k) + " out of range";
+    if (k > 0) {
+      const int64_t* p = &desc[8 * (size_t)(k - 1)];
+      if (d[5] < p[5] || d[6] < p[6] || d[7] < p[7]) return "packed descriptors must have non-decreasing offsets";
+    }
+  }
+  return std::string();
+}
+
+}
+
+namespace {
+
+using dvh::BatchPlan;
+using dvh::ChunkPlan;
+using dvh::make_batch;
+using dvh::make_opts;
 
 int certify_pass(dvh_handle* h, const dvh_packed* bt, const std::vector<int64_t>& desc, int gate, hipStream_t s) {
   const int count = bt->count;
@@ -72,30 +98,17 @@
   return DVH_OK;
 }
 
+bool is_large(const int64_t* d) { return d[0] > dvh::kSmallMax || d[1] > dvh::kSmallMax; }
+
+}
+
+namespace dvh {
+
 void certify_reset(dvh_handle* h) {
   for (int32_t& v : h->st.cert) v = 0;
   h->st.cert_ms = 0.0;
   h->cert_pending = false;
 }
-
-bool is_large(const int64_t* d) { return d[0] > dvh::kSmallMax || d[1] > dvh::kSmallMax; }
-
-struct ChunkPlan {
-  dvh::Chunk ch;
-  int64_t sn, sm, snz;
-  int mn, mm;
-  int64_t mnz;
-  int nsmall;
-  int nj;
-  std::vector<int32_t> med;
-  int med_T = 0;
-};
-struct BatchPlan {
-  std::vector<ChunkPlan> chunks;
-  std::vector<int> large;
-  int64_t wn = 0, wm = 0, wnz = 0;
-  int wc = 0;
-};
 
 BatchPlan scan_chunks(const std::vector<int64_t>& desc, int count, bool chain_on) {
   auto is_medium = [&](const int64_t* d) {
@@ -188,6 +201,15 @@
   return DVH_OK;
 }
 
+}
+
+namespace {
+
+using dvh::certify_reset;
+using dvh::make_work;
+using dvh::next_chunk_events;
+using dvh::scan_chunks;
+
 int host_list_tiers(dvh_handle* h, const dvh::Batch& b, const dvh::Work& w, const ChunkPlan& c, const dvh::Opts& o,
                     bool fast, const std::vector<int64_t>& desc, hipStream_t s) {
   const size_t I = sizeof(int32_t);
@@ -309,8 +331,9 @@
   return DVH_OK;
 }
 
-int finish_timing(dvh_handle* h, hipStream_t s) {
-  DVH_HIP(h, sync_stream(h, s));
+}
+
+void dvh::collect_timing(dvh_handle* h) {
   SolveStats& st = h->st;
   float t = 0;
   st.timing[0] = st.timing[1] = st.timing[2] = 0;
@@ -327,6 +350,13 @@
   }
   st.timing[1] += st.large_ms[0];
   st.timing[2] += st.large_ms[1];
+}
+
+namespace {
+
+int finish_timing(dvh_handle* h, hipStream_t s) {
+  DVH_HIP(h, sync_stream(h, s));
+  dvh::collect_timing(h);
   return DVH_OK;
 }
 
@@ -511,18 +541,8 @@
   std::vector<int64_t> desc(8 * (size_t)bt->count);
   DVH_HIP(h, hipMemcpyAsync(desc.data(), bt->desc, desc.size() * sizeof(int64_t), hipMemcpyDeviceToHost, s));
   DVH_HIP(h, sync_stream(h, s));
-  for (int k = 0; k < bt->count; ++k) {
-    const int64_t* d = &desc[8 * (size_t)k];
-    if (d[0] <= 0 || d[1] < 0 || d[2] < 0 || d[2] > d[1] || d[3] < 0 || d[4] < 0 || d[5] < 0 || d[6] < 0 || d[7] < 0 ||
-        d[4] + d[1] + 1 > bt->total_rows || d[5] + d[3] > bt->total_nnz || d[6] + d[0] > bt->total_n ||
-        d[7] + d[1] > bt->total_m)
-      return fail(h, DVH_ERR_ARG, "packed descriptor " + std::to_string(k) + " out of range");
-    if (k > 0) {
-      const int64_t* p = &desc[8 * (size_t)(k - 1)];
-      if (d[5] < p[5] || d[6] < p[6] || d[7] < p[7])
-        return fail(h, DVH_ERR_ARG, "packed descriptors must have non-decreasing offsets");
-    }
-  }
+  const std::string bad = dvh::check_descriptors(*bt, desc);
+  if (!bad.empty()) return fail(h, DVH_ERR_ARG, bad);
   int rc = solve_packed(h, bt, desc, s);
   if (rc != DVH_OK) return rc;
   return finish_timing(h, s);
diff --git a/der-vet_amd/csrc/dvh_sweep.hip b/der-vet_amd/csrc/dvh_sweep.hip
--- a/der-vet_amd/csrc/dvh_sweep.hip
+++ b/der-vet_amd/csrc/dvh_sweep.hip
@@ -1,3 +1,7 @@
+#include <cstring>
+
+#include <rocprim/device/device_radix_sort.hpp>
+
 #include "dvh_internal.h"
 
 namespace dvh {
@@ -7,7 +11,9 @@
 
 __global__ __launch_bounds__(kSwB) void warm_transfer_kernel(const int64_t* desc, const double* c, const double* u,
                                                              double* x, double* y, const int32_t* rows,
-                                                             const double* wts, int Q, int32_t* bad) {
+                                                             const double* wts, int Q, int32_t* bad,
+                                                             const int32_t* guard) {
+  if (guard && *guard != 0) return;
   __shared__ double red[(kMaxBlend + 1) * (kSwB / kWave)];
   __shared__ double cps[kMaxBlend], cds[kMaxBlend];
   const int32_t* row = rows + (int64_t)(Q + 2) * blockIdx.x;
@@ -140,14 +146,60 @@
   }
 }
 
+__global__ void seeded_guard_kernel(const int32_t* info, int box, int32_t* queue, int32_t* guard) {
+  if (threadIdx.x != 0 || blockIdx.x != 0) return;
+  const bool go = info[0] == 0 && (!box || info[8] == 0);
+  *queue = go ? 0 : INT32_MAX / 2;
+  *guard = go ? 0 : 1;
+}
+
+__global__ __launch_bounds__(kSwB) void seeded_pred_kernel(const int32_t* rows, const double* wts, int Q, int count,
+                                                           int first, const int32_t* istats, double* keys,
+                                                           int32_t* vals) {
+  const int i = blockIdx.x * kSwB + threadIdx.x;
+  if (i >= count) return;
+  const int32_t* row = rows + (int64_t)(Q + 2) * i;
+  double acc = 0.0;
+  for (int k = 0; k < Q; ++k)
+    acc = __dadd_rn(acc, __dmul_rn(wts[(int64_t)Q * i + k], (double)istats[2 * (int64_t)row[1 + k] + 1]));
+  keys[i] = acc;
+  vals[i] = row[0] - first;
+}
+
 }
 
 hipError_t launch_warm_transfer(const int64_t* desc, const double* c, const double* u, double* x, double* y,
-                                const int32_t* rows, const double* wts, int q, int count, int32_t* bad, hipStream_t s) {
+                                const int32_t* rows, const double* wts, int q, int count, int32_t* bad, hipStream_t s,
+                                const int32_t* guard) {
   if (count <= 0) return hipSuccess;
   if (q < 1 || q > kMaxBlend) return hipErrorInvalidValue;
-  hipLaunchKernelGGL(warm_transfer_kernel, dim3(count), dim3(kSwB), 0, s, desc, c, u, x, y, rows, wts, q, bad);
+  hipLaunchKernelGGL(warm_transfer_kernel, dim3(count), dim3(kSwB), 0, s, desc, c, u, x, y, rows, wts, q, bad, guard);
   return hipGetLastError();
 }
 
-}
+hipError_t launch_seeded_guard(const int32_t* info, int box, int32_t* queue, int32_t* guard, hipStream_t s) {
+  hipLaunchKernelGGL(seeded_guard_kernel, dim3(1), dim3(kWave), 0, s, info, box, queue, guard);
+  return hipGetLastError();
+}
+
+hipError_t seeded_order_temp_bytes(int count, size_t* bytes) {
+  *bytes = 0;
+  if (count <= 0) return hipSuccess;
+  return rocprim::radix_sort_pairs_desc(nullptr, *bytes, (const double*)nullptr, (double*)nullptr,
+                                        (const int32_t*)nullptr, (int32_t*)nullptr, (size_t)count);
+}
+
+hipError_t launch_seeded_order(const int32_t* rows, const double* wts, int q, int count, int first,
+                               const int32_t* istats, double* keys, double* keys_out, int32_t* vals, int32_t* order,
+                               void* temp, size_t temp_bytes, hipStream_t s) {
+  if (count <= 0) return hipSuccess;
+  if (q < 1 || q > kMaxBlend) return hipErrorInvalidValue;
+  hipLaunchKernelGGL(seeded_pred_kernel, dim3((count + kSwB - 1) / kSwB), dim3(kSwB), 0, s, rows, wts, q, count, first,
+                     istats, keys, vals);
+  hipError_t e = hipGetLastError();
+  if (e != hipSuccess) return e;
+  return rocprim::radix_sort_pairs_desc(temp, temp_bytes, (const double*)keys, keys_out, (const int32_t*)vals, order,
+                                        (size_t)count, 0, 64, s);
+}
+
+}
diff --git a/der-vet_amd/dervet_hip/_lib.py b/der-vet_amd/dervet_hip/_lib.py
--- a/der-vet_amd/dervet_hip/_lib.py
+++ b/der-vet_amd/dervet_hip/_lib.py
@@ -164,6 +164,14 @@
     "dvh_warm_transfer": (ctypes.c_int, [ctypes.c_void_p, ctypes.POINTER(Packed), ctypes.c_void_p, ctypes.c_int32]),
     "dvh_warm_transfer_blend": (ctypes.c_int, [ctypes.c_void_p, ctypes.POINTER(Packed), ctypes.c_void_p,
                                                ctypes.c_void_p, ctypes.c_int32, ctypes.c_int32]),
+    "dvh_seeded_plan_create": (ctypes.c_int, [ctypes.c_void_p, ctypes.POINTER(Packed), ctypes.c_int32, ctypes.c_void_p,
+                                              ctypes.c_void_p, ctypes.c_int32, ctypes.c_int32,
+                                              ctypes.POINTER(ctypes.c_void_p)]),
+    "dvh_seeded_plan_destroy": (ctypes.c_int, [ctypes.c_void_p, ctypes.c_void_p]),
+    "dvh_seeded_plan_order": (ctypes.c_int, [ctypes.c_void_p, ctypes.c_void_p, ctypes.c_void_p, ctypes.c_int32,
+                                             c_int32_p]),
+    "dvh_solve_seeded_device": (ctypes.c_int, [ctypes.c_void_p, ctypes.c_void_p, ctypes.POINTER(Packed),
+                                               ctypes.POINTER(Options), ctypes.POINTER(Options), ctypes.c_void_p]),
     "dvh_build_battery_group": (ctypes.c_int, [ctypes.c_void_p, ctypes.POINTER(BatteryGroup), ctypes.POINTER(Packed),
                                                ctypes.c_int32]),
     "dvh_synchronize": (ctypes.c_int, [ctypes.c_void_p]),
diff --git a/der-vet_amd/dervet_hip/build.py b/der-vet_amd/dervet_hip/build.py
--- a/der-vet_amd/dervet_hip/build.py
+++ b/der-vet_amd/dervet_hip/build.py
@@ -10,7 +10,7 @@
 BUILDINFO = os.path.join(HERE, "libdervet_hip.buildinfo.json")
 SOURCES = ["dvh_kernels.hip", "dvh_band.hip", "dvh_band_persist.hip", "dvh_band_persist_ice.hip", "dvh_band_grid.hip", "dvh_chain.hip", "dvh_build.hip", "dvh_sweep.hip", "dvh_series.hip", "dvh_route.hip", "dvh_large.hip", "dvh_outage.hip",
            "dvh_certify.hip", "dvh_sizing.hip", "dvh_degradation.hip", "dvh_valuation.hip", "dvh_value_sizing.hip", "dvh_api.cpp", "dvh_api_outage.cpp", "dvh_api_build.cpp",
-           "dvh_api_valuation.cpp", "dvh_api_value_sizing.cpp", "dvh_solve.cpp",
+           "dvh_api_valuation.cpp", "dvh_api_value_sizing.cpp", "dvh_solve.cpp", "dvh_seeded.cpp",
            "dvh_cascade.cpp", "dvh_validate.cpp", "dvh_comm.cpp", "dvh_sizing.cpp", "dvh_sizing_validate.cpp"]
 EXTRA_FLAGS = {"dvh_band_persist.hip": ["-mllvm", "-disable-machine-licm", "-mllvm", "-amdgpu-use-amdgpu-trackers=1"],
                "dvh_band_persist_ice.hip": ["-mllvm", "-disable-machine-licm"],
diff --git a/der-vet_amd/dervet_hip/solver.py b/der-vet_amd/dervet_hip/solver.py
--- a/der-vet_amd/dervet_hip/solver.py
+++ b/der-vet_amd/dervet_hip/solver.py
@@ -248,6 +248,43 @@
         if sync and stream:
             self._check(self._lib.dvh_synchronize(self._h), "dvh_synchronize")
 
+    def seeded_plan(self, pb, n_seed, rows, weights):
+        rows = np.ascontiguousarray(rows, np.int32)
+        weights = np.ascontiguousarray(weights, np.float64)
+        if rows.ndim != 2 or rows.shape[1] < 3 or weights.shape != (len(rows), rows.shape[1] - 2):
+            raise ValueError(f"rows [R, q + 2] and weights [R, q] expected, got {rows.shape} and {weights.shape}")
+        p = pb.as_ctypes()
+        plan = ctypes.c_void_p()
+        rc = self._lib.dvh_seeded_plan_create(self._h, ctypes.byref(p), int(n_seed),
+                                              rows.ctypes.data_as(ctypes.c_void_p),
+                                              weights.ctypes.data_as(ctypes.c_void_p), len(rows), rows.shape[1] - 2,
+                                              ctypes.byref(plan))
+        if rc == _lib.DVH_ERR_UNSUPPORTED:
+            return None
+        self._check(rc, "dvh_seeded_plan_create")
+        return plan
+
+    def seeded_plan_destroy(self, plan):
+        if plan is not None and getattr(self, "_h", None):
+            self._check(self._lib.dvh_seeded_plan_destroy(self._h, plan), "dvh_seeded_plan_destroy")
+
+    def solve_seeded(self, plan, pb, seed_options, warm_options, stream=None):
+        p = pb.as_ctypes()
+        s = ctypes.c_void_p(stream) if stream else None
+        rc = self._lib.dvh_solve_seeded_device(self._h, plan, ctypes.byref(p), ctypes.byref(seed_options),
+                                               ctypes.byref(warm_options), s)
+        if rc == _lib.DVH_ERR_UNSUPPORTED:
+            return False
+        self._check(rc, "dvh_solve_seeded_device")
+        return True
+
+    def seeded_plan_order(self, plan, n_rest):
+        out = np.zeros(max(int(n_rest), 1), np.int32)
+        ordered = ctypes.c_int32()
+        self._check(self._lib.dvh_seeded_plan_order(self._h, plan, out.ctypes.data_as(ctypes.c_void_p), int(n_rest),
+                                                    ctypes.byref(ordered)), "dvh_seeded_plan_order")
+        return out[:n_rest] if ordered.value else None
+
 
 def version():
     return _lib.load().dvh_version().decode()
diff --git a/der-vet_amd/dervet_hip/sweep.py b/der-vet_amd/dervet_hip/sweep.py
--- a/der-vet_amd/dervet_hip/sweep.py
+++ b/der-vet_amd/dervet_hip/sweep.py
@@ -325,6 +325,7 @@
         self.pairs = transfer_pairs(self.transfers) if bl is None else None
         self.rows = transfer_rows(self.transfers) if bl is not None else None
         self._order_dev = None
+        self._plan = None
         self.n_seed = sum(g.G for g in sg)
         self.tags = [t for g in sg + rg for t in g.tags]
         self.specs = None
@@ -365,6 +366,29 @@
         order = win[torch.argsort(pred, descending=True, stable=True)].to(torch.int32).cpu().numpy()
         solver.set_launch_order(order)
 
+    def _seeded_plan(self, solver, dev):
+        if not dev.x.is_cuda or os.environ.get("DVH_SWEEP_FUSED", "1") == "0" or \
+                os.environ.get("DVH_SWEEP_TORCH_TRANSFER") or os.environ.get("DVH_SWEEP_ORDER", "1") not in ("0", "1") or \
+                not hasattr(solver._lib, "dvh_solve_seeded_device"):
+            return None
+        if self._plan is not None and self._plan[0]() is solver and self._plan[1]() is dev and \
+                self._plan[3] == solver._h.value:
+            return self._plan[2]
+        import weakref
+        old = self._plan[0]() if self._plan is not None and self._plan[2] is not None else None
+        if old is not None and getattr(old, "_h", None) and old._h.value == self._plan[3]:
+            old.seeded_plan_destroy(self._plan[2])
+        self._plan = None
+        n_rest = dev.count - self.n_seed
+        if self.rows is not None:
+            rows, wts = self.rows
+        else:
+            rows = self.pairs if self.pairs is not None else np.zeros((0, 3), np.int32)
+            wts = np.ones((len(rows), 1))
+        plan = solver.seeded_plan(dev, self.n_seed, rows, wts) if len(rows) == n_rest else None
+        self._plan = (weakref.ref(solver), weakref.ref(dev), plan, solver._h.value)
+        return plan
+
     def solve(self, solver, dev, warm_options=None, seed_options=None):
         cnt = dev.count
         o0 = solver.options()
@@ -382,6 +406,17 @@
                 if k.endswith("_windows"):
                     paths[k] = paths.get(k, 0) + v
 
+        plan = self._seeded_plan(solver, dev)
+        if plan is not None:
+            so, wo = solver.options(), solver.options()
+            for k, v in seed_options.items():
+                setattr(so, k, v)
+            for k, v in warm_options.items():
+                setattr(wo, k, v)
+            so.warm_start, wo.warm_start = 0, 1
+            if solver.solve_seeded(plan, dev, so, wo):
+                account()
+                return tm, paths
         solver.set_options(warm_start=0, **seed_options)
         try:
             solver.solve_packed(sub_batch(dev, 0, self.n_seed))
diff --git a/include/dervet_hip.h b/include/dervet_hip.h
--- a/include/dervet_hip.h
+++ b/include/dervet_hip.h
@@ -177,6 +177,14 @@
 int dvh_warm_transfer_blend(dvh_handle* h, const dvh_packed* batch, const int32_t* rows, const double* weights,
                             int32_t count, int32_t q);
 
+typedef struct dvh_seeded_plan dvh_seeded_plan;
+int dvh_seeded_plan_create(dvh_handle* h, const dvh_packed* batch, int32_t n_seed, const int32_t* rows,
+                           const double* weights, int32_t count, int32_t q, dvh_seeded_plan** plan);
+int dvh_seeded_plan_destroy(dvh_handle* h, dvh_seeded_plan* plan);
+int dvh_solve_seeded_device(dvh_handle* h, dvh_seeded_plan* plan, const dvh_packed* batch,
+                            const dvh_options* seed_opts, const dvh_options* warm_opts, void* stream);
+int dvh_seeded_plan_order(dvh_handle* h, const dvh_seeded_plan* plan, int32_t* out, int32_t count, int32_t* ordered);
+
 int dvh_certify_batch(dvh_handle* h, const dvh_lp* lps, int32_t count, dvh_result* out);
 int dvh_last_certify(const dvh_handle* h, int32_t* out5);
 int dvh_last_certify_ms(const dvh_handle* h, double* ms);
```

New measurement: 355,000, median of 6. About the same (+0.4%).
